# sangminwoo/SVOL

Measured on AMD Instinct MI355X. Metric: frames/sec (fwd+matcher+bwd), T=32·P=196·d=256, higher is better.
Workload: dtype bf16

## Files before the change

### include/svol_hip.h

```cpp
#ifndef SVOL_HIP_H
#define SVOL_HIP_H

#include <stdint.h>

#ifdef __cplusplus
extern "C" {
#endif

#define SVOL_F32 0
#define SVOL_BF16 1
#define SVOL_F16 2

#define SVOL_OK 0
#define SVOL_E_INVALID (-1)
#define SVOL_E_UNSUPPORTED (-2)
#define SVOL_E_LAUNCH (-3)

#define SVOL_ACT_NONE 0
#define SVOL_ACT_RELU 1
#define SVOL_ACT_GELU 2
#define SVOL_ACT_SIGMOID 3
#define SVOL_ACT_GELU_D 5
#define SVOL_ACT_RELU_RES 4

// ... 2 lines not shown

int svol_cast(const void* src, int dtype_src, void* dst, int dtype_dst, int64_t n, void* stream);
int svol_cast_transpose(const float* src, void* dst, void* dstT, int dtype, int64_t R, int64_t C, void* stream);
int svol_cast_transpose_multi(const void* descs, int32_t n_desc, int64_t total_tiles, int dtype, void* stream);
int svol_cast_split(const float* src, int64_t ld_src, void* dst_hilo, int64_t R, int64_t C, void* stream);

int svol_adamw_flat(float* p, const float* g, float* m, float* v, int64_t n, float lr, float beta1, float beta2, float eps,
                    float weight_decay, int64_t step, float grad_scale, void* stream);
int svol_adamw_flat_zero(float* p, float* g, float* m, float* v, int64_t n, float lr, float beta1, float beta2, float eps,
                         float weight_decay, int64_t step, float grad_scale, void* stream);
int svol_grad_finite(const float* g, int64_t n, float* scaler_state, void* stream);
int svol_adamw_flat_scaled(float* p, const float* g, float* m, float* v, int64_t n, float lr, float beta1, float beta2, float eps,
                           float weight_decay, float grad_mul, const float* scaler_state, void* stream);
int svol_loss_scaler_update(float* scaler_state, float growth_factor, float backoff_factor, int64_t growth_interval, float min_scale,
                            float max_scale, void* stream);
int svol_sgd_flat(float* p, const float* g, float* buf, int64_t n, float lr, float momentum, float weight_decay, float grad_scale,
                  void* stream);
int svol_sgd_flat_zero(float* p, float* g, float* buf, int64_t n, float lr, float momentum, float weight_decay, float grad_scale,
                       void* stream);
int svol_sgd_flat_scaled(float* p, const float* g, float* buf, int64_t n, float lr, float momentum, float weight_decay, float grad_mul,
                         const float* scaler_state, void* stream);
int svol_adam_flat(float* p, const float* g, float* m, float* v, int64_t n, float lr, float beta1, float beta2, float eps,
                   float weight_decay, int64_t step, float grad_scale, void* stream);
int svol_adam_flat_zero(float* p, float* g, float* m, float* v, int64_t n, float lr, float beta1, float beta2, float eps,
                        float weight_decay, int64_t step, float grad_scale, void* stream);
int svol_adam_flat_scaled(float* p, const float* g, float* m, float* v, int64_t n, float lr, float beta1, float beta2, float eps,
                          float weight_decay, float grad_mul, const float* scaler_state, void* stream);
int64_t svol_grad_sqnorm_ws_bytes(int64_t n);
int svol_grad_sqnorm(const float* g, int64_t n, float* ws, float* out, void* stream);
int svol_grad_clip_state(const float* sq, int32_t nb, float grad_mul, float max_norm, float loss_scale, int64_t steps_taken,
                         float* scaler_state, float* state_out, void* stream);
int svol_sgd_flat_grouped(float* p, float* g, float* buf, int64_t n, const int32_t* seg_end, const int32_t* seg_group, int32_t nseg,
                          const float* hyper, int32_t ngroups, const float* state, float grad_mul, int zero, void* stream);
int svol_adam_flat_grouped(float* p, float* g, float* m, float* v, int64_t n, const int32_t* seg_end, const int32_t* seg_group,
                           int32_t nseg, const float* hyper, int32_t ngroups, const float* state, const float* step_count,
                           float grad_mul, int zero, void* stream);
int svol_adamw_flat_grouped(float* p, float* g, float* m, float* v, int64_t n, const int32_t* seg_end, const int32_t* seg_group,
                            int32_t nseg, const float* hyper, int32_t ngroups, const float* state, const float* step_count,
                            float grad_mul, int zero, void* stream);
int svol_flat_step_advance(float* step_count, const float* state, void* stream);

int svol_gemm_nt(const void* A, int64_t lda, const void* A2, int64_t n_split, const void* B, int64_t ldb,
                 void* C, int64_t ldc, const float* bias, const float* colscale, int act, void* pre_act_out,
                 int64_t ldp, const void* residual, int64_t ldr, int out_f32, int64_t M, int64_t N, int64_t K,
                 int dtype, void* stream);
int svol_gemm_nt_split(const void* A, int64_t lda, const void* W_hilo, int64_t ldw, void* C, int64_t ldc, const float* bias,
                       int64_t M, int64_t N, int64_t K, void* stream);
int svol_gemm_nt_dgelu(const void* A, int64_t lda, const void* B, int64_t ldb, void* C, int64_t ldc,
                       const void* pre, int64_t ldp, float* colsum, int64_t M, int64_t N, int64_t K, int dtype,
                       void* stream);
int svol_gemm_nt_dact(const void* A, int64_t lda, const void* B, int64_t ldb, void* C, int64_t ldc,
                      const void* aux, int64_t ldaux, int act, float* colsum, int64_t M, int64_t N, int64_t K,
                      int dtype, void* stream);

int svol_gemm_tn(const void* A, int64_t lda, const void* B, int64_t ldb, float* C, int64_t ldc, float* colsum,
                 int64_t Mc, int64_t N, int64_t K, int dtype, void* stream);
#define SVOL_TN_GROUP_MAX 6
typedef struct svol_tn_problem {
    const void* A; int64_t lda;
    const void* B; int64_t ldb;
    float* C; int64_t ldc;
    float* colsum;
    int64_t Mc, N, K;
} svol_tn_problem;
int svol_gemm_tn_grouped(const svol_tn_problem* problems, int32_t n, int dtype, void* stream);
int svol_colsum(const void* X, int64_t ldx, float* out, int64_t M, int64_t N, int dtype, void* stream);
int svol_act_bwd(const void* dy, const void* aux, void* dpre, int act, int64_t n, int dtype, void* stream);

int svol_layernorm_fwd(const void* x, int x_f32, const float* gamma, const float* beta, float* y32, void* y,
                       void* ypos, const void* pos, int64_t pos_rows, float* mean, float* rstd, int64_t M, int64_t D,
                       float dropout_p, uint64_t seed, const int64_t* seed_offset_dev, int dtype, void* stream);
int svol_layernorm_bwd(const float* dy32, const void* dy, const void* dy2, const void* x, int x_f32,
                       const float* gamma, const float* mean, const float* rstd, float* dx32, void* dx,
                       float* dgamma, float* dbeta, float* dx_colsum, int64_t M, int64_t D, float dropout_p,
                       uint64_t seed, const int64_t* seed_offset_dev, int dtype, void* stream);

int svol_dropout(const void* x, void* y, int64_t n, int64_t row_len, float p, uint64_t seed, int dtype, void* stream);
int svol_dropout_add(const float* t32, const float* res32, float* out32, int64_t n, int64_t row_len, float p, uint64_t seed, void* stream);

int svol_posenc_sine(const float* mask, void* pos, int64_t B, int64_t L, int64_t D, int dtype, void* stream);

int64_t svol_attn_ws_bytes(int64_t B, int64_t H, int64_t Lq, int64_t Lk, int64_t dh);
int svol_attn_fwd(const void* q, int64_t ldq, const void* k, int64_t ldk, const void* v, int64_t ldv, void* o,
                  int64_t ldo, float* lse2, const float* kbias, int64_t B, int64_t H, int64_t Lq, int64_t Lk,
                  int64_t dh, float scale, float q_premul, void* ws, int64_t ws_bytes, int dtype, void* stream);
int svol_attn_bwd(const void* q, int64_t ldq, const void* k, int64_t ldk, const void* v, int64_t ldv, const void* o,
                  int64_t ldo, const void* d_o, int64_t lddo, const float* lse2, float* delta, const float* kbias,
                  void* dq, int64_t lddq, void* dk, int64_t lddk, void* dv, int64_t lddv, int64_t B, int64_t H,
                  int64_t Lq, int64_t Lk, int64_t dh, float scale, float q_premul, void* ws, int64_t ws_bytes,
                  int dtype, void* stream);

#define SVOL_ATTN_DQ_PREZEROED 1
int64_t svol_attn_bwd_sp_image_bytes(int64_t B, int64_t H, int64_t Lq, int64_t Lk, int64_t dh, int64_t ws_bytes, int dtype);
int svol_attn_bwd_zero_ws(void* ws, int64_t ws_bytes, int64_t B, int64_t H, int64_t Lq, int64_t Lk, int64_t dh, int dtype, void* stream);
int svol_attn_bwd_ex(const void* q, int64_t ldq, const void* k, int64_t ldk, const void* v, int64_t ldv, const void* o,
                     int64_t ldo, const void* d_o, int64_t lddo, const float* lse2, float* delta, const float* kbias,
                     void* dq, int64_t lddq, void* dk, int64_t lddk, void* dv, int64_t lddv, int64_t B, int64_t H,
                     int64_t Lq, int64_t Lk, int64_t dh, float scale, float q_premul, void* ws, int64_t ws_bytes,
                     int dtype, int flags, void* ev_prep, void* stream);

int svol_attn_fwd_dropout(const void* q, int64_t ldq, const void* k, int64_t ldk, const void* v, int64_t ldv, void* o,
                          int64_t ldo, float* lse2, const float* kbias, int64_t B, int64_t H, int64_t Lq, int64_t Lk,
                          int64_t dh, float scale, float q_premul, void* ws, int64_t ws_bytes, float dropout_p, uint64_t seed,
                          int dtype, void* stream);
int svol_attn_bwd_dropout(const void* q, int64_t ldq, const void* k, int64_t ldk, const void* v, int64_t ldv, const void* o,
                          int64_t ldo, const void* d_o, int64_t lddo, const float* lse2, float* delta, const float* kbias,
                          void* dq, int64_t lddq, void* dk, int64_t lddk, void* dv, int64_t lddv, int64_t B, int64_t H,
                          int64_t Lq, int64_t Lk, int64_t dh, float scale, float q_premul, void* ws, int64_t ws_bytes,
                          float dropout_p, uint64_t seed, int dtype, void* stream);

int svol_gate_fwd(const float* x32, const void* pos, const float* u, const float* gamma, const float* beta,
                  float* y32, void* y, void* ypos, float* a, float* mean, float* rstd, float* ws, int64_t B,
                  int64_t L, int64_t D, int64_t H, int dtype, void* stream);
int svol_gate_bwd(const float* dy32, const void* dy, const void* dy2, const float* x32, const void* pos,
                  const float* u, const float* gamma, const float* a, const float* mean, const float* rstd,
                  const float* ws, float* ws2, float* dx32, float* du, float* dgamma, float* dbeta, int64_t B,
                  int64_t L, int64_t D, int64_t H, int dtype, void* stream);

int svol_layernorm_gate_scores_fwd(const float* x32, const float* gamma, const float* beta, float* y32, void* y, void* ypos,
                                   const void* pos, float* mean, float* rstd, const float* u_next, float* scores_next,
                                   int64_t B, int64_t L, int64_t D, int64_t H, int dtype, void* stream);
int svol_gate_fwd_scored(const float* x32, const void* pos, const float* u, const float* gamma, const float* beta,
                         float* y32, void* y, void* ypos, float* a, float* mean, float* rstd, float* ws, int64_t B,
                         int64_t L, int64_t D, int64_t H, int dtype, void* stream);

int svol_gate_vectors_fwd(const float* skch, const float* W_in, const float* b_in, float* q_out, float* u_out, int64_t B, int64_t D,
                          int64_t H, void* stream);
int svol_gate_vectors_bwd(const float* du, const float* skch, const float* W_in, const float* q, float* dq_ws, float* dskch,
                          float* dW_in, float* db_in, int64_t B, int64_t D, int64_t H, void* stream);
#define SVOL_GATE_VEC_MAX_LAYERS 8
int svol_gate_vectors_fwd_multi(const float* skch, const float* const* W_in, const float* const* b_in, float* const* q_out,
                                float* const* u_out, int64_t n_layers, int64_t B, int64_t D, int64_t H, void* stream);
int svol_gate_vectors_bwd_multi(const float* const* du, const float* skch, const float* const* W_in, const float* const* q,
                                float* const* dq_ws, float* const* dskch, float* const* dW_in, float* const* db_in, int64_t n_layers,
                                int64_t B, int64_t D, int64_t H, void* stream);

int svol_match_cost(const float* logits, const float* boxes, const float* tgt_boxes, const int32_t* pred_off,
                    const int32_t* pred_cnt, const int32_t* tgt_off, const int32_t* tgt_cnt,
                    const int64_t* cost_off, float* cost, int32_t n_problems, float w_bbox, float w_giou,
                    float w_class, int32_t* box_status, void* stream);
int svol_lsap_batched(const float* cost, const int64_t* cost_off, const int32_t* pred_off, const int32_t* pred_cnt,
                      const int32_t* tgt_off, const int32_t* tgt_cnt, int32_t* match, int32_t* status,
                      int32_t n_problems, int32_t max_dim, void* stream);
int svol_heads_fwd(const float* hs, const float* Wc, const float* bc, const float* W0, const float* b0, const float* W1, const float* b1,
                   const float* W2, const float* b2, float* logits, float* h1, float* h2, float* boxes, int64_t R, int64_t D, void* stream);
// ... 46 lines not shown
int svol_conv_weight_unpack_add(const float* dwp, float* grad, int64_t Cout, int64_t Cin, int64_t kh, int64_t kw, int64_t Kp, void* stream);
int svol_conv_wgrad_nhwc(const void* dz, const void* x, float* dwp, int64_t N, int64_t H, int64_t W, int64_t C, int64_t Cout, int64_t kh, int64_t kw,
                         int64_t stride, int64_t pad, int64_t Kp, int dtype, void* stream);
int svol_bn_apply(const void* z, const float* scale, const float* shift, const void* residual, int relu, void* y, int64_t M, int64_t C,
                  int dtype, void* stream);
int svol_bn_bwd_reduce(const void* dy, const void* y, const void* z, const float* mean, const float* rstd, float* sum_g, float* sum_gx,
                       int64_t M, int64_t C, int dtype, void* stream);
int svol_bn_bwd_apply(const void* dy, const void* y, const void* z, const float* mean, const float* rstd, const float* gamma,
                      const float* sum_g, const float* sum_gx, void* dz, void* dres, int64_t M, int64_t C, int dtype, void* stream);
int svol_col2im_nhwc(const void* dcols, int64_t ldcols, void* dx, int64_t N, int64_t H, int64_t W, int64_t C, int64_t kh, int64_t kw,
                     int64_t stride, int64_t pad, int dtype, void* stream);
int svol_maxpool_idx_nhwc(const void* x, void* y, uint8_t* idx, int64_t N, int64_t H, int64_t W, int64_t C, int64_t k, int64_t stride,
                          int64_t pad, int dtype, void* stream);
int svol_maxpool_bwd_nhwc(const void* dy, const uint8_t* idx, void* dx, int64_t N, int64_t H, int64_t W, int64_t C, int64_t k,
                          int64_t stride, int64_t pad, int dtype, void* stream);
int svol_attn_weights_mean(const void* q, int64_t ldq, const void* k, int64_t ldk, const float* lse2, const float* kbias,
                           float* att, int64_t B, int64_t H, int64_t Lq, int64_t Lk, int64_t dh, float scale,
                           float q_premul, int dtype, void* stream);
int svol_attn_small_fwd(const void* q, int64_t ldq, const void* k, int64_t ldk, const void* v, int64_t ldv, void* o, int64_t ldo,
                        int64_t n_seq, int64_t H, int64_t L, int64_t dh, float scale, int dtype, void* stream);
int svol_attn_small_fwd_lse(const void* q, int64_t ldq, const void* k, int64_t ldk, const void* v, int64_t ldv, void* o, int64_t ldo,
                            float* lse2, int64_t n_seq, int64_t H, int64_t L, int64_t dh, float scale, int dtype, void* stream);
int svol_attn_small_bwd(const void* q, int64_t ldq, const void* k, int64_t ldk, const void* v, int64_t ldv, const void* o, int64_t ldo,
                        const void* dout, int64_t lddo, const float* lse2, void* dq, int64_t lddq, void* dk, int64_t lddk, void* dv,
                        int64_t lddv, int64_t n_seq, int64_t H, int64_t L, int64_t dh, float scale, int dtype, void* stream);


#define SVOL_DIM_B 0
#define SVOL_DIM_L 1
#define SVOL_DIM_N 2
#define SVOL_DIM_D 3
#define SVOL_DIM_H 4
#define SVOL_DIM_F 5
#define SVOL_DIM_DTYPE 6
#define SVOL_DIM_QDTYPE 7
#define SVOL_DIM_ATTN_WS_BYTES 8
#define SVOL_DIM_COUNT 9

#define SVOL_BLK_VIDEO_HALF 0
#define SVOL_BLK_QUERY_SELF 1
#define SVOL_BLK_QUERY_CROSS 2
const char* svol_block_slot_names(int block);
int svol_block_trace_dump(char* buf, int64_t cap);
int svol_clock_probe(uint64_t* samples, int32_t* count, int32_t max_samples, const int32_t* stop, int64_t period_us,
                     int64_t max_ms, int32_t* wall_khz, void* stream);


#define SVOL_VH_SLOTS(X) \
    X(X32) X(POS) X(U) X(G1) X(BT1) X(G2) X(BT2) X(G3) X(BT3) X(B_IN) X(B_O) X(B_FC1) X(B_FC2) X(QSCALE) \
    X(W_IN) X(WV_HILO) X(W_O) X(W_FC1) X(W_FC2) X(W_IN_T) X(W_O_T) X(W_FC1_T) X(W_FC2_T) \
    X(Y1) X(Y1POS) X(A) X(MEAN1) X(RSTD1) X(GATE_WS) X(GATE_PRE) X(U_NEXT) X(GATE_WS_NEXT) \
    X(QKV) X(O) X(LSE) X(S2) X(Y2) X(MEAN2) X(RSTD2) X(PRE) X(HID) X(S3) \
    X(MEAN3) X(RSTD3) X(M32) X(M) X(MPOS) X(Y1_32) X(Y2_32) X(ATTN_WS) \
    X(DM32) X(DM) X(DMPOS) X(DS32_3) X(DS3) X(DPRE) X(DY2) X(DS32_2) X(G2D) X(DO) X(DQKV) X(DELTA) X(DXQP) X(DXQ) X(GATE_WS2) \
    X(DX32) X(DU) \
    X(DG1) X(DBT1) X(DG2) X(DBT2) X(DG3) X(DBT3) X(DW_IN) X(DB_IN) X(DW_O) X(DB_O) X(DW_FC1) X(DB_FC1) X(DW_FC2) X(DB_FC2) \
    X(EV_A0) X(EV_A1) X(EV_CLEAN_IN) X(EV_PREP) X(ATTN_WS_NEXT) X(ZERO_STREAM) X(EV_CLEAN_OUT)
#define SVOL_QS_SLOTS(X) \
    X(O32) X(O) X(OPOS) X(QPOS) X(B_IN) X(B_O) X(G4) X(BT4) X(QSCALE) X(W_IN) X(WV_HILO) X(W_O) X(W_IN_T) X(W_O_T) \
    X(QKV) X(OA) X(LSE) X(S4) X(MEAN4) X(RSTD4) X(Y32) X(Y) X(YPOS) X(ATTN_WS) \
    X(DY32) X(DY) X(DYPOS) X(G) X(DOA) X(DQKV) X(DELTA) X(DO32) X(DXQ) X(DXQP) X(DQPOS) \
    X(DW_IN) X(DB_IN) X(DW_O) X(DB_O) X(DG4) X(DBT4)
#define SVOL_QC_SLOTS(X) \
    X(O32) X(O) X(OPOS) X(MV) X(MPOS) X(KBIAS) X(QPOS) X(B_IN) X(B_O) X(G5) X(BT5) X(B_FC1) X(B_FC2) X(G6) X(BT6) X(QSCALE) \
    X(W_INQ) X(W_INQ_T) X(W_KV) X(W_KV_T) X(WV_HILO) X(W_O) X(W_O_T) X(W_FC1) X(W_FC1_T) X(W_FC2) X(W_FC2_T) \
    X(Q) X(QC) X(KV) X(OA) X(OAQ) X(LSE) X(S5) X(Y5_32) X(Y5) X(MEAN5) X(RSTD5) X(PRE) X(HID) X(S6) X(MEAN6) X(RSTD6) \
    X(Y32) X(Y) X(YPOS) X(ATTN_WS) \
    X(DY32) X(DY) X(DYPOS) X(DS32_6) X(DS6) X(DPRE) X(DY5) X(DS32_5) X(G5D) X(DOAQ) X(DOA) X(DQC) X(DQ) X(DKV) X(DELTA) \
    X(DO32) X(DXQP) X(DMPOS) X(DMV) X(DQPOS) \
    X(DW_IN) X(DB_IN) X(DW_O) X(DB_O) X(DG5) X(DBT5) X(DW_FC1) X(DB_FC1) X(DW_FC2) X(DB_FC2) X(DG6) X(DBT6)
#define SVOL_SLOT_ENUM_VH(n) SVOL_VH_##n,
#define SVOL_SLOT_ENUM_QS(n) SVOL_QS_##n,
#define SVOL_SLOT_ENUM_QC(n) SVOL_QC_##n,
enum { SVOL_VH_SLOTS(SVOL_SLOT_ENUM_VH) SVOL_VH_COUNT };
enum { SVOL_QS_SLOTS(SVOL_SLOT_ENUM_QS) SVOL_QS_COUNT };
enum { SVOL_QC_SLOTS(SVOL_SLOT_ENUM_QC) SVOL_QC_COUNT };

int svol_video_half_fwd(const int64_t* dims, void* const* slots, void* stream);
int svol_video_half_bwd(const int64_t* dims, void* const* slots, int phase, void* stream);
int svol_video_half_wgrad(const int64_t* dims, void* const* slots, void* stream);
int svol_video_half_wgrad_part(const int64_t* dims, void* const* slots, int part, void* stream);
int svol_query_self_fwd(const int64_t* dims, void* const* slots, void* stream);
int svol_query_self_bwd(const int64_t* dims, void* const* slots, void* stream);
int svol_query_self_wgrad(const int64_t* dims, void* const* slots, void* stream);
int svol_query_cross_fwd(const int64_t* dims, void* const* slots, void* stream);
int svol_query_cross_bwd(const int64_t* dims, void* const* slots, void* stream);
int svol_query_cross_wgrad(const int64_t* dims, void* const* slots, void* stream);

#ifdef __cplusplus
}
#endif
#endif
```

### svol_amd/_lib.py

```python
from __future__ import annotations

import ctypes
import os

_HERE = os.path.dirname(os.path.abspath(__file__))
LIB_PATH = os.path.join(_HERE, 'libsvol_hip.so')

_p = ctypes.c_void_p
_i64 = ctypes.c_int64
_i32 = ctypes.c_int32
_int = ctypes.c_int
_f32 = ctypes.c_float
_u64 = ctypes.c_uint64

SIGNATURES = {
    'svol_block_trace_dump': [ctypes.c_char_p, _i64],
    'svol_lsap_solve': [_p, _i64, _i64, _p, _p],
    'svol_heads_fwd': [_p] * 13 + [_i64, _i64, _p],
    'svol_heads_bwd': [_p] * 17 + [_i64, _i64, _p],
    'svol_set_loss_bwd': [_p] * 6 + [_i64, _i64, _p],
    'svol_weighted_total': [_p, _p, _i64, _p, _p],
    'svol_weighted_total_bwd': [_p, _p, _i64, _p, _p],
    'svol_cast': [_p, _int, _p, _int, _i64, _p],
    'svol_cast_transpose': [_p, _p, _p, _int, _i64, _i64, _p],
    'svol_cast_split': [_p, _i64, _p, _i64, _i64, _p],
    'svol_gemm_nt_split': [_p, _i64, _p, _i64, _p, _i64, _p, _i64, _i64, _i64, _p],
    'svol_gemm_nt': [_p, _i64, _p, _i64, _p, _i64, _p, _i64, _p, _p, _int, _p, _i64, _p, _i64, _int, _i64, _i64, _i64,
                     _int, _p],
    'svol_gemm_nt_dgelu': [_p, _i64, _p, _i64, _p, _i64, _p, _i64, _p, _i64, _i64, _i64, _int, _p],
    'svol_gemm_nt_dact': [_p, _i64, _p, _i64, _p, _i64, _p, _i64, _int, _p, _i64, _i64, _i64, _int, _p],
    'svol_gemm_tn': [_p, _i64, _p, _i64, _p, _i64, _p, _i64, _i64, _i64, _int, _p],
    'svol_gemm_tn_grouped': [_p, _i32, _int, _p],
    'svol_colsum': [_p, _i64, _p, _i64, _i64, _int, _p],
    'svol_act_bwd': [_p, _p, _p, _int, _i64, _int, _p],
    'svol_layernorm_fwd': [_p, _int, _p, _p, _p, _p, _p, _p, _i64, _p, _p, _i64, _i64, _f32, _u64, _p, _int, _p],
    'svol_layernorm_bwd': [_p, _p, _p, _p, _int, _p, _p, _p, _p, _p, _p, _p, _p, _i64, _i64, _f32, _u64, _p, _int, _p],
    'svol_cast_transpose_multi': [_p, _int, _i64, _int, _p],
    'svol_postprocess': [_p, _p, _p, _i64, _i64, _i64, _p],
    'svol_eval_max_iou': [_p, _p, _p, _p, _p, _p, _i64, _int, _p],
    'svol_eval_ap': [_p, _p, _p, _p, _p, _p, _p, _p, _int, _p, _p, _p, _p, _i64, _i64, _i64, _p],
    'svol_patchify': [_p, _p, _i64, _i64, _i64, _i64, _i64, _int, _p],
    'svol_vit_embed': [_p, _p, _p, _p, _p, _i64, _i64, _i64, _int, _p],
    'svol_ingest_resize': [_p, _i64, _i64, _i64, _i64, _i64, _i64, _p, _i64, _p, _i64, _p, _p, _p, _i64, _i64, _i64, _i64, _i64, _i64, _int, _p],
    'svol_adamw_flat': [_p, _p, _p, _p, _i64, _f32, _f32, _f32, _f32, _f32, _i64, _f32, _p],
    'svol_adamw_flat_zero': [_p, _p, _p, _p, _i64, _f32, _f32, _f32, _f32, _f32, _i64, _f32, _p],
    'svol_grad_finite': [_p, _i64, _p, _p],
    'svol_adamw_flat_scaled': [_p, _p, _p, _p, _i64, _f32, _f32, _f32, _f32, _f32, _f32, _p, _p],
    'svol_loss_scaler_update': [_p, _f32, _f32, _i64, _f32, _f32, _p],
    'svol_sgd_flat': [_p, _p, _p, _i64, _f32, _f32, _f32, _f32, _p],
    'svol_sgd_flat_zero': [_p, _p, _p, _i64, _f32, _f32, _f32, _f32, _p],
    'svol_sgd_flat_scaled': [_p, _p, _p, _i64, _f32, _f32, _f32, _f32, _p, _p],
    'svol_adam_flat': [_p, _p, _p, _p, _i64, _f32, _f32, _f32, _f32, _f32, _i64, _f32, _p],
    'svol_adam_flat_zero': [_p, _p, _p, _p, _i64, _f32, _f32, _f32, _f32, _f32, _i64, _f32, _p],
    'svol_adam_flat_scaled': [_p, _p, _p, _p, _i64, _f32, _f32, _f32, _f32, _f32, _f32, _p, _p],
    'svol_grad_sqnorm_ws_bytes': [_i64],
    'svol_grad_sqnorm': [_p, _i64, _p, _p, _p],
    'svol_grad_clip_state': [_p, _i32, _f32, _f32, _f32, _i64, _p, _p, _p],
    'svol_sgd_flat_grouped': [_p, _p, _p, _i64, _p, _p, _i32, _p, _i32, _p, _f32, _int, _p],
    'svol_adam_flat_grouped': [_p, _p, _p, _p, _i64, _p, _p, _i32, _p, _i32, _p, _p, _f32, _int, _p],
    'svol_adamw_flat_grouped': [_p, _p, _p, _p, _i64, _p, _p, _i32, _p, _i32, _p, _p, _f32, _int, _p],
    'svol_flat_step_advance': [_p, _p, _p],
    'svol_conv_nhwc': [_p, _p, _i64, _p, _p, _int, _p, _i64, _i64, _i64, _i64, _i64, _i64, _i64, _i64, _i64, _int, _p],
    'svol_im2col': [_p, _i64, _i64, _i64, _i64, _int, _p, _i64, _i64, _i64, _i64, _i64, _i64, _i64, _i64, _i64, _int, _p],
    'svol_maxpool_nhwc': [_p, _p, _i64, _i64, _i64, _i64, _i64, _i64, _i64, _int, _p],
    'svol_avgpool_nhwc': [_p, _p, _i64, _i64, _i64, _int, _p],
    'svol_bn_colstats': [_p, _p, _f32, _p, _p, _i64, _i64, _int, _p],
    'svol_bn_finalize': [_p, _p, _p, _p, _p, _p, _p, _f32, _f32, _i64, _i64, _p, _p, _p, _p, _p],
    'svol_conv_weight_pack': [_p, _p, _i64, _i64, _i64, _i64, _i64, _int, _int, _p],
    'svol_conv_weight_unpack_add': [_p, _p, _i64, _i64, _i64, _i64, _i64, _p],
    'svol_conv_wgrad_nhwc': [_p, _p, _p, _i64, _i64, _i64, _i64, _i64, _i64, _i64, _i64, _i64, _i64, _int, _p],
    'svol_bn_apply': [_p, _p, _p, _p, _int, _p, _i64, _i64, _int, _p],
    'svol_bn_bwd_reduce': [_p, _p, _p, _p, _p, _p, _p, _i64, _i64, _int, _p],
    'svol_bn_bwd_apply': [_p, _p, _p, _p, _p, _p, _p, _p, _p, _p, _i64, _i64, _int, _p],
    'svol_col2im_nhwc': [_p, _i64, _p, _i64, _i64, _i64, _i64, _i64, _i64, _i64, _i64, _int, _p],
    'svol_maxpool_idx_nhwc': [_p, _p, _p, _i64, _i64, _i64, _i64, _i64, _i64, _i64, _int, _p],
    'svol_maxpool_bwd_nhwc': [_p, _p, _p, _i64, _i64, _i64, _i64, _i64, _i64, _i64, _int, _p],
    'svol_attn_weights_mean': [_p, _i64, _p, _i64, _p, _p, _p, _i64, _i64, _i64, _i64, _i64, _f32, _f32, _int, _p],
    'svol_attn_small_fwd': [_p, _i64, _p, _i64, _p, _i64, _p, _i64, _i64, _i64, _i64, _i64, _f32, _int, _p],
    'svol_attn_small_fwd_lse': [_p, _i64, _p, _i64, _p, _i64, _p, _i64, _p, _i64, _i64, _i64, _i64, _f32, _int, _p],
    'svol_attn_small_bwd': [_p, _i64, _p, _i64, _p, _i64, _p, _i64, _p, _i64, _p, _p, _i64, _p, _i64, _p, _i64, _i64, _i64, _i64,
                            _i64, _f32, _int, _p],
    'svol_posenc_sine': [_p, _p, _i64, _i64, _i64, _int, _p],
    'svol_attn_ws_bytes': [_i64, _i64, _i64, _i64, _i64],
# ... 83 lines not shown
```

### svol_amd/blocks.py

```python
from __future__ import annotations

import ctypes
import math
import os
import weakref

import torch

from . import _lib, ops

WGRAD_SPLIT = os.environ.get('SVOL_WGRAD_SPLIT') is not None
ENABLED = os.environ.get('SVOL_NO_BLOCKS') is None
GATE_SCORES_FUSE = os.environ.get('SVOL_GATE_SCORES_FUSE') is not None
VH, QS, QC = 0, 1, 2
_F32, _BF16 = 0, 1
_ESZ = {torch.float32: 4, torch.bfloat16: 2, torch.float16: 2}
_SLOTS = {}


def _slots(block):
    m = _SLOTS.get(block)
    if m is None:
        names = _lib.lib().svol_block_slot_names(block).decode().rstrip(',').split(',')
        m = _SLOTS[block] = {n: i for i, n in enumerate(names)}
# ... 293 lines not shown
    e0, e1 = torch.cuda.Event(enable_timing=True), torch.cuda.Event(enable_timing=True)
    e0.record()
    e1.record()
    tm.records.setdefault((name, meta), []).append((e0, e1))
    return e0, e1


DQ_PREZERO = os.environ.get('SVOL_DQ_PREZERO') is not None and os.environ.get('SVOL_NO_DQ_PREZERO') is None
_DQ_PREZERO = {}


class _DqPrezero:
    __slots__ = ('bufs', 'side', 'ev_prep', 'clean_ev', 'clean', 'nxt')

    def __init__(self, dev, wsb):
        self.bufs = [torch.empty((_align(wsb, 1 << 20),), dtype=torch.uint8, device=dev) for _ in range(2)]
        self.side = torch.cuda.Stream(device=dev)
        self.ev_prep = torch.cuda.Event()
        self.clean_ev = [torch.cuda.Event(), torch.cuda.Event()]
        for e_ in [self.ev_prep] + self.clean_ev:
            e_.record()
        self.clean = [False, False]
        self.nxt = 0

    def bind(self, tbl):
        i = self.nxt
        tbl.set('ATTN_WS', self.bufs[i].data_ptr())
        tbl.set('EV_CLEAN_IN', self.clean_ev[i].cuda_event if self.clean[i] else None)
        tbl.set('EV_PREP', self.ev_prep.cuda_event)
        tbl.set('ATTN_WS_NEXT', self.bufs[1 - i].data_ptr())
        tbl.set('ZERO_STREAM', self.side.cuda_stream)
        tbl.set('EV_CLEAN_OUT', self.clean_ev[1 - i].cuda_event)
        self.clean[i] = False

    def advance(self, tbl):
        i = self.nxt
        self.clean[1 - i] = True
        self.nxt = 1 - i
        for n_ in ('EV_CLEAN_IN', 'EV_PREP', 'ATTN_WS_NEXT', 'ZERO_STREAM', 'EV_CLEAN_OUT'):
            tbl.set(n_, None)


def _dq_prezero(dev, B, H, L, dh, dt, wsb):
    if not DQ_PREZERO or dt == torch.float32 or torch.cuda.is_current_stream_capturing():
        return None
    key = (dev, ops._stream(), B, H, L, dh, dt, wsb)
    st = _DQ_PREZERO.get(key)
    if st is None:
        img = _lib.lib().svol_attn_bwd_sp_image_bytes(B, H, L, L, dh, wsb, ops._DT[dt])
        st = _DQ_PREZERO[key] = _DqPrezero(dev, wsb) if img > 0 else False
    return st or None


def _vh_fwd_layout(B, L, D, H, F, e):
    M = B * L
    return [('Y1', M * D * e), ('Y1POS', M * D * e), ('A', M * 4), ('MEAN1', M * 4), ('RSTD1', M * 4), ('GATE_WS', B * H * (L + 2) * 4),
            ('QKV', M * 3 * D * e), ('O', M * D * e), ('LSE', B * H * L * 4), ('S2', M * D * 4), ('Y2', M * D * e), ('MEAN2', M * 4),
            ('RSTD2', M * 4), ('PRE', M * F * e), ('HID', M * F * e), ('S3', M * D * 4), ('MEAN3', M * 4), ('RSTD3', M * 4),
            ('M32', M * D * 4), ('M', M * D * e), ('MPOS', M * D * e)]


def _vh_bwd_layout(B, L, D, H, F, e):
    M = B * L
    return [('DS32_3', M * D * 4), ('DS3', M * D * e), ('DPRE', M * F * e), ('DY2', M * D * e), ('DS32_2', M * D * 4), ('G2D', M * D * e),
            ('DO', M * D * e), ('DQKV', M * 3 * D * e), ('DELTA', 3 * B * H * L * 4), ('DXQP', M * D * e), ('DXQ', M * D * e),
            ('GATE_WS2', (B * L + B * H) * 4), ('DX32', M * D * 4)]


class VideoHalfFn(torch.autograd.Function):

    @staticmethod
    def forward(ctx, pl, x32, pos, u, u_next, sc_in, *params):
        ctx.set_materialize_grads(False)
        B, L, D = x32.shape
        layer = pl.layer()
        H, F = layer.nhead, layer.mlp1.fc1.weight.shape[0]
        dt = pl.dt
        e = _ESZ[dt]
        dev = x32.device
        M = B * L
        x2 = x32.reshape(M, D)
        x2 = x2 if x2.is_contiguous() else x2.contiguous()
        pos2 = pos.reshape(M, D)
        pos2 = pos2 if pos2.is_contiguous() else pos2.contiguous()
        u = u.contiguous()
        assert x2.dtype == torch.float32 and pos2.dtype == dt and u.dtype == torch.float32
        wsb = _attn_ws_bytes(B, H, L, L, D // H, dt)
        key = (VH, B, L, D, H, F, dt)
        lay = _layout(('f',) + key, lambda: _vh_fwd_layout(B, L, D, H, F, e))
        slay = _layout(('s',) + key, lambda: [('Y1_32', M * D * 4), ('Y2_32', M * D * 4), ('ATTN_WS', max(wsb, 16))])
        arena = torch.empty((lay.total,), dtype=torch.uint8, device=dev)
        scr = _scratch(dev, slay.total)
        tbl = _Table(VH, pl.tpl)
        lay.fill(tbl, arena.data_ptr())
        slay.fill(tbl, scr.data_ptr())
        tbl.set('X32', x2.data_ptr())
        tbl.set('POS', pos2.data_ptr())
        tbl.set('U', u.data_ptr())
        if sc_in is not None:
            assert sc_in.dtype == torch.float32 and sc_in.numel() == B * H * (L + 2) and sc_in.is_contiguous()
            tbl.set('GATE_WS', sc_in.data_ptr())
            tbl.set('GATE_PRE', sc_in.data_ptr())
        if u_next is not None:
            u_next = u_next.contiguous()
            assert u_next.dtype == torch.float32 and u_next.shape == u.shape and L % 4 == 0
            sc_next = torch.empty((B * H * (L + 2),), dtype=torch.float32, device=dev)
            tbl.set('U_NEXT', u_next.data_ptr())
            tbl.set('GATE_WS_NEXT', sc_next.data_ptr())
        else:
            sc_next = torch.empty((0,), dtype=torch.float32, device=dev)
        dims = _dims(B, L, 0, D, H, F, dt, dt, wsb)
        big = B * H * L * L >= ops._WGRAD_FLUSH_MIN_SCORES
        if big:
            ops._BIG_ATTN['left'] += 1
        ev = _maybe_events('attn_fwd', (B, H, L, L, D // H))
        if ev:
            tbl.set('EV_A0', ev[0].cuda_event)
            tbl.set('EV_A1', ev[1].cuda_event)
# ... 2 lines not shown
        tbl.set('EV_A1', None)
        tbl.set('U_NEXT', None)
        tbl.set('GATE_WS_NEXT', None)
        ctx.pl, ctx.tbl, ctx.dims, ctx.arena, ctx.shape, ctx.big = pl, tbl, dims, arena, (B, L, D, H, F), big
        ctx.n_par = len(params)
        ctx.sc_in = sc_in
        ctx.save_for_backward(x2, pos2, u)
        ctx.mark_non_differentiable(sc_next)
        return (lay.view(arena, 'M32', torch.float32, (B, L, D)), lay.view(arena, 'M', dt, (B, L, D)),
                lay.view(arena, 'MPOS', dt, (B, L, D)), sc_next)

    @staticmethod
    def backward(ctx, dm32, dm, dmpos, _dsc=None):
        pl, tbl, dims = ctx.pl, ctx.tbl, ctx.dims
        B, L, D, H, F = ctx.shape
        x2, pos2, u = ctx.saved_tensors
        n_par = ctx.n_par
        if dm32 is None and dm is None and dmpos is None:
            pl.done(n_par > 0)
            return (None,) * (6 + n_par)
        dt = pl.dt
        e = _ESZ[dt]
        dev = x2.device
        M = B * L
        cont = lambda t_: None if t_ is None else (t_.reshape(M, D) if t_.is_contiguous() else t_.reshape(M, D).contiguous())
        dm32, dm, dmpos = cont(dm32), cont(dm), cont(dmpos)
        lay = _layout(('b', VH, B, L, D, H, F, dt), lambda: _vh_bwd_layout(B, L, D, H, F, e))
        tmp = torch.empty((lay.total,), dtype=torch.uint8, device=dev)
        lay.fill(tbl, tmp.data_ptr())
        du = torch.zeros((B, H, D), dtype=torch.float32, device=dev)
        tbl.set('DU', du.data_ptr())
        tbl.set_t('DM32', dm32)
        tbl.set_t('DM', dm)
        tbl.set_t('DMPOS', dmpos)
        slay = _layout(('s', VH, B, L, D, H, F, dt), None)
        scr = _scratch(dev, slay.total)
        slay.fill(tbl, scr.data_ptr())
        bufs = pl.grad_buffers(tbl, dev)
        L_ = _lib.lib()
        s = ops._stream()
        _lib.check(L_.svol_video_half_bwd(dims, tbl.arr, 1, s), 'svol_video_half_bwd')
        keep = [t_ for t_ in (ctx.arena, tmp, dm32, dm, dmpos) if t_ is not None]
        split = bufs is None and ctx.big and WGRAD_SPLIT
        if ctx.big:
            ops._BIG_ATTN['left'] -= 1
            if split:
                _issue_wgrad('svol_video_half_wgrad_part', dims, tbl, keep, dev, part=1)
            ops.flush_wgrad(gate=True)
        ev = _maybe_events('attn_bwd', (B, H, L, L, D // H))
        if ev:
            tbl.set('EV_A0', ev[0].cuda_event)
            tbl.set('EV_A1', ev[1].cuda_event)
        pz = _dq_prezero(dev, B, H, L, D // H, dt, dims[8]) if ctx.big else None
        if pz is not None:
            pz.bind(tbl)
        _lib.check(L_.svol_video_half_bwd(dims, tbl.arr, 2, s), 'svol_video_half_bwd')
        if pz is not None:
            pz.advance(tbl)
        tbl.set('EV_A0', None)
        tbl.set('EV_A1', None)
        if split:
            _issue_wgrad('svol_video_half_wgrad_part', dims, tbl, keep, dev, part=2)
        elif bufs is None:
            _issue_wgrad('svol_video_half_wgrad', dims, tbl, keep, dev)
        else:
            _lib.check(L_.svol_video_half_wgrad(dims, tbl.arr, s), 'svol_video_half_wgrad')
        pl.done(n_par > 0)
        dx32 = lay.view(tmp, 'DX32', torch.float32, (B, L, D))
        needs = ctx.needs_input_grad
        return (None, dx32, None, du if needs[3] else None, None, None) + tuple(pl.grads_out(bufs, needs[6:], n_par > 0))


def gate_scores_fusable(L, D, H):
    return GATE_SCORES_FUSE and L % 4 == 0 and D % 4 == 0 and D <= 256 and H <= 8


def video_half(layer, x32, pos, u, dt, u_next=None, sc_in=None):
    pl = plan(layer, VH, dt, dt)
    if u_next is not None and not gate_scores_fusable(x32.shape[1], x32.shape[2], layer.nhead):
        u_next = None
    m32, m, mpos, sc = VideoHalfFn.apply(pl, x32, pos, u, u_next, sc_in, *pl.inputs(x32, u))
    return m32, m, mpos, (sc if u_next is not None else None)


def _qpos_target(pl, qpos, tbl, dev, N, D):
    if not qpos.requires_grad:
        tbl.set('DQPOS', None)
        return None, False
    s = ops._claim(qpos, True) if (qpos.is_leaf and qpos.dtype == torch.float32) else None
    if s is not None:
        tbl.set_t('DQPOS', s.view)
        return None, True
    g = torch.zeros((N, D), dtype=torch.float32, device=dev)
    tbl.set('DQPOS', g.data_ptr())
    return g, False


class QuerySelfFn(torch.autograd.Function):

    @staticmethod
    def forward(ctx, pl, o32, o, opos, qpos, *params):
        ctx.set_materialize_grads(False)
        B, N, D = o.shape
        layer = pl.layer()
        H = layer.nhead
        qdt = pl.qdt
        e = _ESZ[qdt]
        dev = o.device
        R = B * N
        c = lambda t_: t_ if t_.is_contiguous() else t_.contiguous()
        o32_, o_, opos_, qpos_ = c(o32), c(o), c(opos), c(qpos)
# ... 30 lines not shown
            pl.done(n_par > 0)
            return (None,) * (5 + n_par)
        qdt = pl.qdt
        e = _ESZ[qdt]
        dev = o_.device
        R = B * N
        cont = lambda t_: None if t_ is None else (t_ if t_.is_contiguous() else t_.contiguous())
        dy32, dy, dypos = cont(dy32), cont(dy), cont(dypos)
        lay = _layout(('b', QS, B, N, D, H, qdt), lambda: [('G', R * D * e), ('DOA', R * D * e), ('DQKV', R * 3 * D * e),
                                                            ('DELTA', 3 * B * H * N * 4), ('DO32', R * D * 4), ('DXQ', R * D * e),
                                                            ('DXQP', R * D * e)])
        tmp = torch.empty((lay.total,), dtype=torch.uint8, device=dev)
        lay.fill(tbl, tmp.data_ptr())
        tbl.set_t('DY32', dy32)
        tbl.set_t('DY', dy)
        tbl.set_t('DYPOS', dypos)
        slay = _layout(('s', QS, B, N, D, H, qdt), None)
        scr = _scratch(dev, slay.total)
        slay.fill(tbl, scr.data_ptr())
        needs = ctx.needs_input_grad
        gq, _ = _qpos_target(pl, qpos, tbl, dev, N, D) if needs[4] else (None, False)
        if not needs[4]:
            tbl.set('DQPOS', None)
        bufs = pl.grad_buffers(tbl, dev)
        L_ = _lib.lib()
        s = ops._stream()
        _lib.check(L_.svol_query_self_bwd(dims, tbl.arr, s), 'svol_query_self_bwd')
        keep = (ctx.arena, tmp, o_, opos_)
        if bufs is None:
            _issue_wgrad('svol_query_self_wgrad', dims, tbl, list(keep), dev)
        else:
            _lib.check(L_.svol_query_self_wgrad(dims, tbl.arr, s), 'svol_query_self_wgrad')
        pl.done(n_par > 0)
        if gq is not None and qdt != torch.float32:
            gq = ops.cast(gq, qdt)
        v = lambda n_, dt_: lay.view(tmp, n_, dt_, (B, N, D))
        return (None, v('DO32', torch.float32), v('DXQ', qdt), v('DXQP', qdt), gq) + tuple(pl.grads_out(bufs, needs[5:], n_par > 0))


def query_self(layer, out, qpos, dt, qdt):
    pl = plan(layer, QS, dt, qdt)
    o32, o, opos = out
    return QuerySelfFn.apply(pl, o32, o, opos, qpos, *pl.inputs(o32, o, opos))


def _qc_fwd_layout(B, N, L, D, H, F, e, qe):
    R, M = B * N, B * L
    return [('Q', R * D * qe), ('QC', R * D * e), ('KV', M * 2 * D * e), ('OA', R * D * e), ('OAQ', R * D * qe), ('LSE', B * H * N * 4),
            ('S5', R * D * 4), ('Y5_32', R * D * 4), ('Y5', R * D * qe), ('MEAN5', R * 4), ('RSTD5', R * 4), ('PRE', R * F * qe),
            ('HID', R * F * qe), ('S6', R * D * 4), ('MEAN6', R * 4), ('RSTD6', R * 4), ('Y32', R * D * 4), ('Y', R * D * qe),
            ('YPOS', R * D * qe)]


def _qc_bwd_layout(B, N, L, D, H, F, e, qe):
    R, M = B * N, B * L
    return [('DS32_6', R * D * 4), ('DS6', R * D * qe), ('DPRE', R * F * qe), ('DY5', R * D * qe), ('G5D', R * D * qe), ('DOAQ', R * D * qe),
            ('DOA', R * D * e), ('DQC', R * D * e), ('DQ', R * D * qe), ('DKV', M * 2 * D * e), ('DELTA', 3 * B * H * N * 4),
            ('DO32', R * D * 4), ('DXQP', R * D * qe), ('DMPOS', M * D * e), ('DMV', M * D * e)]


class QueryCrossFn(torch.autograd.Function):

    @staticmethod
    def forward(ctx, pl, o32, o, opos, mv, mpos, kbias, qpos, *params):
        ctx.set_materialize_grads(False)
        B, N, D = o.shape
        L = mv.shape[1]
        layer = pl.layer()
        H, F = layer.nhead, layer.mlp2.fc1.weight.shape[0]
        dt, qdt = pl.dt, pl.qdt
        e, qe = _ESZ[dt], _ESZ[qdt]
        dev = o.device
        c = lambda t_: t_ if t_.is_contiguous() else t_.contiguous()
        o32_, o_, opos_, mv_, mpos_, kb_, qpos_ = c(o32), c(o), c(opos), c(mv), c(mpos), c(kbias), c(qpos)
        assert o32_.dtype == torch.float32 and o_.dtype == qdt and opos_.dtype == qdt and qpos_.dtype == qdt
        assert mv_.dtype == dt and mpos_.dtype == dt and kb_.dtype == torch.float32
        wsb = _attn_ws_bytes(B, H, N, L, D // H, dt)
        key = (QC, B, N, L, D, H, F, dt, qdt)
        lay = _layout(('f',) + key, lambda: _qc_fwd_layout(B, N, L, D, H, F, e, qe))
        slay = _layout(('s',) + key, lambda: [('ATTN_WS', max(wsb, 16))])
        arena = torch.empty((lay.total,), dtype=torch.uint8, device=dev)
        scr = _scratch(dev, slay.total)
        tbl = _Table(QC, pl.tpl)
        lay.fill(tbl, arena.data_ptr())
        slay.fill(tbl, scr.data_ptr())
        for n_, t_ in (('O32', o32_), ('O', o_), ('OPOS', opos_), ('MV', mv_), ('MPOS', mpos_), ('KBIAS', kb_), ('QPOS', qpos_)):
            tbl.set(n_, t_.data_ptr())
        dims = _dims(B, L, N, D, H, F, dt, qdt, wsb)
        _lib.check(_lib.lib().svol_query_cross_fwd(dims, tbl.arr, ops._stream()), 'svol_query_cross_fwd')
        ctx.pl, ctx.tbl, ctx.dims, ctx.arena, ctx.shape = pl, tbl, dims, arena, (B, N, L, D, H, F)
        ctx.n_par = len(params)
        ctx.save_for_backward(o32_, o_, opos_, mv_, mpos_, kb_, qpos)
        return (lay.view(arena, 'Y32', torch.float32, (B, N, D)), lay.view(arena, 'Y', qdt, (B, N, D)),
                lay.view(arena, 'YPOS', qdt, (B, N, D)))

    @staticmethod
    def backward(ctx, dy32, dy, dypos):
        pl, tbl, dims = ctx.pl, ctx.tbl, ctx.dims
        B, N, L, D, H, F = ctx.shape
        o32_, o_, opos_, mv_, mpos_, kb_, qpos = ctx.saved_tensors
        n_par = ctx.n_par
        if dy32 is None and dy is None and dypos is None:
            pl.done(n_par > 0)
            return (None,) * (8 + n_par)
        dt, qdt = pl.dt, pl.qdt
        e, qe = _ESZ[dt], _ESZ[qdt]
        dev = o_.device
        cont = lambda t_: None if t_ is None else (t_ if t_.is_contiguous() else t_.contiguous())
        dy32, dy, dypos = cont(dy32), cont(dy), cont(dypos)
        lay = _layout(('b', QC, B, N, L, D, H, F, dt, qdt), lambda: _qc_bwd_layout(B, N, L, D, H, F, e, qe))
        tmp = torch.empty((lay.total,), dtype=torch.uint8, device=dev)
        lay.fill(tbl, tmp.data_ptr())
        tbl.set_t('DY32', dy32)
        tbl.set_t('DY', dy)
        tbl.set_t('DYPOS', dypos)
        slay = _layout(('s', QC, B, N, L, D, H, F, dt, qdt), None)
        scr = _scratch(dev, slay.total)
        slay.fill(tbl, scr.data_ptr())
        needs = ctx.needs_input_grad
        gq = None
        if needs[7]:
            gq, _ = _qpos_target(pl, qpos, tbl, dev, N, D)
        else:
            tbl.set('DQPOS', None)
        bufs = pl.grad_buffers(tbl, dev)
        L_ = _lib.lib()
        s = ops._stream()
        _lib.check(L_.svol_query_cross_bwd(dims, tbl.arr, s), 'svol_query_cross_bwd')
        keep = (ctx.arena, tmp, opos_, mv_, mpos_)
        if bufs is None:
            _issue_wgrad('svol_query_cross_wgrad', dims, tbl, list(keep), dev)
        else:
            _lib.check(L_.svol_query_cross_wgrad(dims, tbl.arr, s), 'svol_query_cross_wgrad')
        pl.done(n_par > 0)
        if gq is not None and qdt != torch.float32:
            gq = ops.cast(gq, qdt)
        vq = lambda n_, dt_: lay.view(tmp, n_, dt_, (B, N, D))
        vm = lambda n_: lay.view(tmp, n_, dt, (B, L, D))
        return (None, vq('DO32', torch.float32), None, vq('DXQP', qdt), vm('DMV'), vm('DMPOS'), None, gq) + \
            tuple(pl.grads_out(bufs, needs[8:], n_par > 0))


def query_cross(layer, out, mv, mpos, kbias, qpos, dt, qdt):
    pl = plan(layer, QC, dt, qdt)
    o32, o, opos = out
    return QueryCrossFn.apply(pl, o32, o, opos, mv, mpos, kbias, qpos, *pl.inputs(o32, opos, mv, mpos))


def trace_dump() -> str:
    buf = ctypes.create_string_buffer(1 << 20)
    _lib.check(_lib.lib().svol_block_trace_dump(buf, len(buf)), 'svol_block_trace_dump')
    return buf.value.decode()
```

### svol_amd/csrc/attention.hip

```cpp
#include "attn_call.h"

namespace {

constexpr float LOG2E = 1.4426950408889634f;

template <typename T> struct AT;
template <> struct AT<float> {
    static constexpr int EPC = 4, NA = 4, CPR = 8, NAT_ROW = 128, TR_STRIDE = 64 * 4 + 16;
};

template <typename T>
__device__ __forceinline__ int nat_off(int row, int ch) {
    if constexpr (sizeof(T) == 2) return row * 64 + ((ch ^ ((row >> 2) & 3)) << 4);
    else return row * 128 + ((ch ^ (row & 7)) << 4);
}

template <typename T>
__device__ __forceinline__ void stage_tile(char* nat, char* tr, const T* g, int64_t ld, int row0, int limit, int dh,
                                           int tid) {
    constexpr int EPC = AT<T>::EPC, CPR = AT<T>::CPR, ST = AT<T>::TR_STRIDE;
    for (int c = tid; c < 64 * CPR; c += 256) {
        const int row = c / CPR, ch = c % CPR;
        const int d0 = ch * EPC;
        uint4 v = make_uint4(0, 0, 0, 0);
// ... 462 lines not shown
    AttnArgs p{};
    attn_fill(p, c);
    dim3 grid((unsigned)((Lq + 127) / 128), (unsigned)H, (unsigned)B);
    hipLaunchKernelGGL(attn_fwd_kernel<float>, grid, dim3(256), 0, c.stream, p);
    SVOL_CHECK_LAUNCH();
    return SVOL_OK;
}
int svol_attn_fwd(const void* q, int64_t ldq, const void* k, int64_t ldk, const void* v, int64_t ldv, void* o,
                  int64_t ldo, float* lse2, const float* kbias, int64_t B, int64_t H, int64_t Lq, int64_t Lk, int64_t dh,
                  float scale, float q_premul, void* ws, int64_t ws_bytes, int dtype, void* stream) {
    return svol_attn_fwd_dropout(q, ldq, k, ldk, v, ldv, o, ldo, lse2, kbias, B, H, Lq, Lk, dh, scale, q_premul, ws, ws_bytes, 0.f, 0,
                                 dtype, stream);
}

static int attn_bwd_impl(const void* q, int64_t ldq, const void* k, int64_t ldk, const void* v, int64_t ldv, const void* o,
                         int64_t ldo, const void* d_o, int64_t lddo, const float* lse2, float* delta, const float* kbias, void* dq,
                         int64_t lddq, void* dk, int64_t lddk, void* dv, int64_t lddv, int64_t B, int64_t H, int64_t Lq, int64_t Lk,
                         int64_t dh, float scale, float q_premul, void* ws, int64_t ws_bytes, float drop_p, uint64_t drop_seed,
                         int dtype, void* stream, int flags = 0, void* ev_prep = nullptr) {
    AttnCall c{};
    c.q = q; c.k = k; c.v = v; c.o = o; c.d_o = d_o; c.lse2 = const_cast<float*>(lse2); c.delta = delta; c.kbias = kbias;
    c.dq = dq; c.dk = dk; c.dv = dv;
    c.ldq = ldq; c.ldk = ldk; c.ldv = ldv; c.ldo = ldo; c.lddo = lddo; c.lddq = lddq; c.lddk = lddk; c.lddv = lddv;
    c.scale = scale; c.premul = q_premul; c.ws = static_cast<float*>(ws); c.ws_bytes = ws_bytes;
    c.drop_p = drop_p; c.drop_seed = drop_seed; c.flags = flags; c.ev_prep = ev_prep; c.stream = reinterpret_cast<hipStream_t>(stream);
    if (const int rc = check_call(c, true, B, H, Lq, Lk, dh, dtype)) return rc;
    if (svol_is16(dtype)) return (dtype == SVOL_BF16 ? svol_attn_bwd_bf16_launch : svol_attn_bwd_f16_launch)(c);
    AttnArgs p{};
    attn_fill(p, c);
    const int64_t total = B * Lq * H;
    dim3 gd((unsigned)((total + 255) / 256));
    dim3 gq((unsigned)((Lq + 127) / 128), (unsigned)H, (unsigned)B);
    dim3 gk((unsigned)((Lk + 127) / 128), (unsigned)H, (unsigned)B);
    hipLaunchKernelGGL(attn_delta_kernel<float>, gd, dim3(256), 0, c.stream, p);
    hipLaunchKernelGGL(attn_bwd_dq_kernel<float>, gq, dim3(256), 0, c.stream, p);
    hipLaunchKernelGGL(attn_bwd_dkdv_kernel<float>, gk, dim3(256), 0, c.stream, p);
    if (ev_prep) (void)hipEventRecord(static_cast<hipEvent_t>(ev_prep), c.stream);
    SVOL_CHECK_LAUNCH();
    return SVOL_OK;
}

int svol_attn_bwd(const void* q, int64_t ldq, const void* k, int64_t ldk, const void* v, int64_t ldv, const void* o,
                  int64_t ldo, const void* d_o, int64_t lddo, const float* lse2, float* delta, const float* kbias, void* dq,
                  int64_t lddq, void* dk, int64_t lddk, void* dv, int64_t lddv, int64_t B, int64_t H, int64_t Lq, int64_t Lk,
                  int64_t dh, float scale, float q_premul, void* ws, int64_t ws_bytes, int dtype, void* stream) {
    return attn_bwd_impl(q, ldq, k, ldk, v, ldv, o, ldo, d_o, lddo, lse2, delta, kbias, dq, lddq, dk, lddk, dv, lddv, B, H, Lq, Lk, dh,
                         scale, q_premul, ws, ws_bytes, 0.f, 0, dtype, stream);
}
int svol_attn_bwd_ex(const void* q, int64_t ldq, const void* k, int64_t ldk, const void* v, int64_t ldv, const void* o,
                     int64_t ldo, const void* d_o, int64_t lddo, const float* lse2, float* delta, const float* kbias, void* dq,
                     int64_t lddq, void* dk, int64_t lddk, void* dv, int64_t lddv, int64_t B, int64_t H, int64_t Lq, int64_t Lk,
                     int64_t dh, float scale, float q_premul, void* ws, int64_t ws_bytes, int dtype, int flags, void* ev_prep,
                     void* stream) {
    if (flags & ~SVOL_ATTN_DQ_PREZEROED) return SVOL_E_INVALID;
    return attn_bwd_impl(q, ldq, k, ldk, v, ldv, o, ldo, d_o, lddo, lse2, delta, kbias, dq, lddq, dk, lddk, dv, lddv, B, H, Lq, Lk, dh,
                         scale, q_premul, ws, ws_bytes, 0.f, 0, dtype, stream, flags, ev_prep);
}
int64_t svol_attn_bwd_sp_image_bytes(int64_t B, int64_t H, int64_t Lq, int64_t Lk, int64_t dh, int64_t ws_bytes, int dtype) {
    if (!svol_is16(dtype) || check_common(B, H, Lq, Lk, dh, dtype)) return 0;
    return (dtype == SVOL_BF16 ? svol_attn_sp_image_bytes_bf16 : svol_attn_sp_image_bytes_f16)((int)B, (int)H, (int)Lq, (int)Lk, (int)dh,
                                                                                              ws_bytes);
}
int svol_attn_bwd_zero_ws(void* ws, int64_t ws_bytes, int64_t B, int64_t H, int64_t Lq, int64_t Lk, int64_t dh, int dtype, void* stream) {
    if (!ws || !aligned16(ws)) return SVOL_E_INVALID;
    if (!svol_is16(dtype)) return SVOL_E_UNSUPPORTED;
    const int rc = check_common(B, H, Lq, Lk, dh, dtype);
    if (rc) return rc;
    return (dtype == SVOL_BF16 ? svol_attn_sp_zero_bf16_launch : svol_attn_sp_zero_f16_launch)(
        static_cast<float*>(ws), ws_bytes, (int)B, (int)H, (int)Lq, (int)Lk, (int)dh, reinterpret_cast<hipStream_t>(stream));
}
int svol_attn_bwd_dropout(const void* q, int64_t ldq, const void* k, int64_t ldk, const void* v, int64_t ldv, const void* o,
                          int64_t ldo, const void* d_o, int64_t lddo, const float* lse2, float* delta, const float* kbias, void* dq,
                          int64_t lddq, void* dk, int64_t lddk, void* dv, int64_t lddv, int64_t B, int64_t H, int64_t Lq, int64_t Lk,
                          int64_t dh, float scale, float q_premul, void* ws, int64_t ws_bytes, float dropout_p, uint64_t seed,
                          int dtype, void* stream) {
    return attn_bwd_impl(q, ldq, k, ldk, v, ldv, o, ldo, d_o, lddo, lse2, delta, kbias, dq, lddq, dk, lddk, dv, lddv, B, H, Lq, Lk, dh,
                         scale, q_premul, ws, ws_bytes, dropout_p, seed, dtype, stream);
}

}
```

### svol_amd/csrc/attention_bf16.hip

```cpp
#include <cstdint>
#include <cstdlib>

#include "attn_call.h"

namespace {

constexpr float LOG2E = 1.4426950408889634f;
constexpr int KT = 128;
constexpr int IMG = KT * 64;
constexpr float LAZY_THR = 4.0f;

struct Args {
    const void *q, *k, *v, *o, *d_o;
    void *out_o, *dq, *dk, *dv;
    const float* kbias;
    float *lse2, *delta;
    int64_t ldq, ldk, ldv, ldo, lddo, lddq, lddk, lddv;
    int B, H, Lq, Lk, dh;
    float scale;
    float premul;
    int ksplit, tiles_per_split;
    float *ws_o, *ws_ml, *ws_dq;
    const int* tile_flags;
    int head_xcd, nxt;
// ... 1502 lines not shown
        {
            const int row = tid >> 3, d0 = (tid & 7) * 4;
            f32x4 v = *reinterpret_cast<const f32x4*>(sRed + row * 32 + d0);
#pragma unroll
            for (int w = 1; w < 4; ++w) {
                const f32x4 u = *reinterpret_cast<const f32x4*>(sRed + (w * 32 + row) * 32 + d0);
#pragma unroll
                for (int e = 0; e < 4; ++e) v[e] += u[e];
            }
            const int q = sub * 32 + row;
            if (q < p.Lq) {
                float* z = p.ws_dq + ((int64_t)b * p.Lq + q) * (p.H * 32) + hh * 32 + d0;
#pragma unroll
                for (int e = 0; e < 4; ++e) unsafeAtomicAdd(z + e, v[e]);
            }
        }
        __syncthreads();
    }
}

template <bool ZERO>
__global__ __launch_bounds__(256) void attn_bwd_sp_prep_bf16(Args p) {
    __shared__ float s_lse[8][33], s_dl[8][33];
    const int tid = threadIdx.x;
    const int64_t row0 = (int64_t)blockIdx.x * 32;
    const int b = (int)(row0 / p.Lq), q0 = (int)(row0 % p.Lq);
    {
        const int hh = tid >> 5, rl = tid & 31;
        if (hh < p.H) s_lse[hh][rl] = p.lse2[((int64_t)b * p.H + hh) * p.Lq + q0 + rl];
    }
    const int rl = tid >> 3, hh = tid & 7;
    float dl = 0.f;
    if (hh < p.H) {
        const int64_t row = row0 + rl;
        const h16_t* o = reinterpret_cast<const h16_t*>(p.o) + row * p.ldo + hh * 32;
        const h16_t* d = reinterpret_cast<const h16_t*>(p.d_o) + row * p.lddo + hh * 32;
#pragma unroll
        for (int i = 0; i < 32; i += 8) {
            const h16x8 a = *reinterpret_cast<const h16x8*>(o + i), c = *reinterpret_cast<const h16x8*>(d + i);
#pragma unroll
            for (int e = 0; e < 8; ++e) dl += (float)a[e] * (float)c[e];
        }
        if constexpr (ZERO) {
            float* z = p.ws_dq + row * (p.H * 32) + hh * 32;
#pragma unroll
            for (int i = 0; i < 32; i += 4) *reinterpret_cast<f32x4*>(z + i) = f32x4{0.f, 0.f, 0.f, 0.f};
        }
        s_dl[hh][rl] = dl;
    }
    __syncthreads();
    {
        const int h2 = tid >> 5, r2 = tid & 31;
        if (h2 < p.H) {
            const int64_t si = ((int64_t)b * p.H + h2) * p.Lq + q0 + r2;
            reinterpret_cast<float*>(p.nl2)[si] = -s_lse[h2][r2];
            reinterpret_cast<float*>(p.nd2)[si] = -s_dl[h2][r2];
            p.delta[si] = s_dl[h2][r2];
        }
    }
}
__global__ __launch_bounds__(256) void attn_dq_round_bf16(Args p) {
    const int64_t i = ((int64_t)blockIdx.x * blockDim.x + threadIdx.x) * 8;
    const int64_t W = (int64_t)p.H * 32, total = (int64_t)p.B * p.Lq * W;
    if (i >= total) {
        const int tk = p.Lk % (4 * 128);
        const int64_t j = i - ((total + 2047) / 2048) * 2048;
        if (tk == 0 || j < 0 || j >= (int64_t)p.B * p.H * 2 * tk * 32) return;
        const int64_t per = (int64_t)2 * tk * 32;
        const int bh = (int)(j / per), rem = (int)(j % per), kv = rem / (tk * 32), key = (rem / 32) % tk, d0 = rem % 32;
        const float* src = p.ws_dq + total + (int64_t)bh * 4 * per + rem;
        f32x4 a = {0.f, 0.f, 0.f, 0.f}, c = a;
#pragma unroll
        for (int part = 0; part < 4; ++part) { a += *reinterpret_cast<const f32x4*>(src + part * per); c += *reinterpret_cast<const f32x4*>(src + part * per + 4); }
        const float mul = kv == 0 ? p.scale / p.premul : 1.f;
        h16x8 v;
#pragma unroll
        for (int e = 0; e < 4; ++e) { v[e] = (h16_t)(a[e] * mul); v[4 + e] = (h16_t)(c[e] * mul); }
        const int b_ = bh / p.H, hh_ = bh % p.H;
        const int64_t row = (int64_t)b_ * p.Lk + (p.Lk - tk) + key;
        h16_t* o = kv == 0 ? reinterpret_cast<h16_t*>(p.dk) + row * p.lddk : reinterpret_cast<h16_t*>(p.dv) + row * p.lddv;
        *reinterpret_cast<h16x8*>(o + hh_ * 32 + d0) = v;
        return;
    }
    const int64_t row = i / W, c = i % W;
    const f32x4 a = *reinterpret_cast<const f32x4*>(p.ws_dq + i), b = *reinterpret_cast<const f32x4*>(p.ws_dq + i + 4);
    h16x8 v;
#pragma unroll
    for (int e = 0; e < 4; ++e) { v[e] = (h16_t)(a[e] * p.scale); v[4 + e] = (h16_t)(b[e] * p.scale); }
    *reinterpret_cast<h16x8*>(reinterpret_cast<h16_t*>(p.dq) + row * p.lddq + c) = v;
}

__global__ __launch_bounds__(256) void attn_sp_zero_image(float* __restrict__ z, int64_t n4) {
    const int64_t stride = (int64_t)gridDim.x * 256;
    for (int64_t i = (int64_t)blockIdx.x * 256 + threadIdx.x; i < n4; i += stride)
        reinterpret_cast<f32x4*>(z)[i] = f32x4{0.f, 0.f, 0.f, 0.f};
}

typedef __attribute__((ext_vector_type(4))) unsigned u32x4;
__device__ __forceinline__ u32x4 to_acc(u32x4 r) {
    asm volatile("; operand -> AGPR" : "+a"(r));
    return r;
}
__device__ __forceinline__ u32x4 as_u32x4(const uint4& v) { return u32x4{v.x, v.y, v.z, v.w}; }
#define SP_FENCE() __builtin_amdgcn_sched_barrier(0)
__device__ __forceinline__ void sp_mfma_c(f32x16& d, const uint4& a, const u32x4& b, const f32x16& c) {
    asm volatile("v_mfma_f32_32x32x16_" SVOL_H16_ASM " %0, %1, %2, %3" : "=&v"(d) : "v"(as_u32x4(a)), "a"(b), "v"(c));
}
__device__ __forceinline__ void sp_mfma_z(f32x16& d, const uint4& a, const u32x4& b) {
    asm volatile("v_mfma_f32_32x32x16_" SVOL_H16_ASM " %0, %1, %2, 0" : "=&v"(d) : "v"(as_u32x4(a)), "a"(b));
}
__device__ __forceinline__ void sp_mfma_v(f32x16& d, const uint4& a, const u32x4& b) {
    asm volatile("v_mfma_f32_32x32x16_" SVOL_H16_ASM " %0, %1, %2, %0" : "+v"(d) : "v"(as_u32x4(a)), "a"(b));
}
__device__ __forceinline__ void sp_mfma_a(f32x16& acc, const uint4& a, const u32x4& b) {
    asm volatile("v_mfma_f32_32x32x16_" SVOL_H16_ASM " %0, %1, %2, %0" : "+a"(acc) : "v"(as_u32x4(a)), "v"(b));
}
__device__ __forceinline__ unsigned cvt_pk_u32(float a, float b) { return __builtin_bit_cast(unsigned, cvt_pk_h16(a, b)); }

struct SpStep {
    uint4 qa[2], doa[2];
    f32x16 Cl, Cd;
};
constexpr int SP_OFF_Q = 4 * KT * 4 + 512;
constexpr int SP_OFF_T = SP_OFF_Q + 4 * IMG;
constexpr int SP_OFF_P = SP_OFF_Q + 8 * IMG;

template <int NKB>
__device__ __forceinline__ void attn_bwd_sp_body(const Args& p, char* smem, int hh, int b, int kbase, int t_begin, int t_end, float* tail_out) {
    float* sL = reinterpret_cast<float*>(smem);
    float* sD = sL + 2 * KT;
    float* sNeg = sL + 4 * KT;
    char* sQ = smem + SP_OFF_Q;
    char* sPart = smem + SP_OFF_P;
    const int tid = threadIdx.x, lane = tid & 63, wave = __builtin_amdgcn_readfirstlane(tid >> 6);
    const int r = lane & 31, h = lane >> 5;
    constexpr int dqw = 8 * 32;
    const h16_t* Q = reinterpret_cast<const h16_t*>(p.q) + (int64_t)b * p.Lq * p.ldq + hh * 32;
    const h16_t* dO = reinterpret_cast<const h16_t*>(p.d_o) + (int64_t)b * p.Lq * p.lddo + hh * 32;
// ... 820 lines not shown
constexpr int SP_ZERO_WGS = 64;
int svol_attn_sp_zero_bf16_launch(float* ws, int64_t ws_bytes, int B, int H, int Lq, int Lk, int dh, hipStream_t s) {
    if (!sp_planned(B, H, Lq, Lk, dh, ws != nullptr, ws_bytes)) return SVOL_E_UNSUPPORTED;
    const int64_t n4 = (int64_t)B * Lq * H * 32 / 4;
    const int64_t want = (n4 + 255) / 256;
    hipLaunchKernelGGL(attn_sp_zero_image, dim3((unsigned)(want < SP_ZERO_WGS ? want : SP_ZERO_WGS)), dim3(256), 0, s, ws, n4);
    return hipGetLastError() == hipSuccess ? SVOL_OK : SVOL_E_LAUNCH;
}
static Args make_args(const AttnCall& c, int ksplit, int tiles_per_split, const Grid& g) {
    Args p{};
    attn_fill(p, c);
    p.ksplit = ksplit; p.tiles_per_split = tiles_per_split;
    if (ksplit > 1) {
        p.ws_o = c.ws;
        p.ws_ml = p.ws_o + (int64_t)p.ksplit * p.B * p.Lq * p.H * p.dh;
        p.ws_dq = p.ws_ml + (int64_t)p.ksplit * p.B * p.H * p.Lq * 2;
    }
    p.head_xcd = g.head_xcd; p.nxt = g.nxt; p.tail_last = g.tail_last;
    return p;
}

int svol_attn_fwd_bf16_launch(const AttnCall& c) {
    const Plan pl = attn_plan(c);
    Args p = make_args(c, pl.fwd_ksplit, pl.fwd_tps, pl.gf);
    const dim3 grid = pl.gf.dim, wg(256);
    hipStream_t s = c.stream;
    switch (pl.fwd) {
    case Fwd::pre_masked:
        p.tile_flags = reinterpret_cast<const int*>(c.ws);
        hipLaunchKernelGGL(attn_tile_flags_bf16, dim3((unsigned)pl.ntk, (unsigned)c.B), dim3(64), 0, s, c.kbias, c.Lk, pl.ntk, reinterpret_cast<int*>(c.ws));
        hipLaunchKernelGGL(attn_fwd_bf16_pre_masked, grid, wg, 0, s, p);
        break;
    case Fwd::fast2_redo:
        p.redo = reinterpret_cast<int*>(c.ws);
        hipLaunchKernelGGL(attn_fwd_bf16_fast2, grid, wg, 0, s, p);
        [[fallthrough]];
    case Fwd::pre_all: hipLaunchKernelGGL(attn_fwd_bf16_pre, grid, wg, 0, s, p); break;
    case Fwd::general_m:
    case Fwd::ksplit_m: hipLaunchKernelGGL(attn_fwd_bf16<true>, grid, wg, 0, s, p); break;
    case Fwd::general_u:
    case Fwd::ksplit_u: hipLaunchKernelGGL(attn_fwd_bf16<false>, grid, wg, 0, s, p); break;
    }
    const int64_t total = (int64_t)c.B * c.Lq * c.H;
    if (pl.fwd_ksplit > 1) hipLaunchKernelGGL(attn_combine_bf16, dim3((unsigned)((total + 127) / 128)), dim3(128), 0, s, p);
    return hipGetLastError() == hipSuccess ? SVOL_OK : SVOL_E_LAUNCH;
}

int svol_attn_bwd_bf16_launch(const AttnCall& c) {
    const Plan pl = attn_plan(c);
    Args pq = make_args(c, pl.bwd_ksplit, pl.bwd_tps, pl.gq), pk = make_args(c, pl.bwd_ksplit, pl.bwd_tps, pl.gk);
    const int64_t total = (int64_t)c.B * c.Lq * c.H;
    const dim3 gd((unsigned)((total + 255) / 256)), wg(256);
    hipStream_t s = c.stream;
    auto bind_rows = [&](Args& a) { a.nl2 = reinterpret_cast<unsigned*>(c.delta + total); a.nd2 = reinterpret_cast<unsigned*>(c.delta + 2 * total); };
    void (*dq)(Args) = nullptr, (*dkdv)(Args) = nullptr;
    if (!pl.pre) hipLaunchKernelGGL(attn_delta_bf16, gd, wg, 0, s, pq);
    switch (pl.bwd) {
    case Bwd::bwd_pre_masked:
        pq.tile_flags = pk.tile_flags = reinterpret_cast<const int*>(c.ws);
        hipLaunchKernelGGL(attn_tile_flags_bf16, dim3((unsigned)pl.ntk, (unsigned)c.B), dim3(64), 0, s, c.kbias, c.Lk, pl.ntk, reinterpret_cast<int*>(c.ws));
        dq = attn_bwd_dq_bf16_pre_masked, dkdv = attn_bwd_dkdv_bf16_pre_masked;
        break;
    case Bwd::bwd_sp:
        pq.ws_dq = c.ws;
        bind_rows(pq);
        hipLaunchKernelGGL((c.flags & SVOL_ATTN_DQ_PREZEROED) ? attn_bwd_sp_prep_bf16<false> : attn_bwd_sp_prep_bf16<true>,
                           dim3((unsigned)((int64_t)c.B * c.Lq / 32)), wg, 0, s, pq);
        break;
    case Bwd::bwd_rot_dma:
        bind_rows(pq), bind_rows(pk);
        dq = attn_bwd_dq_bf16_rot, dkdv = attn_bwd_dkdv_bf16_pre_dma;
        break;
    case Bwd::bwd_rot: dq = attn_bwd_dq_bf16_rot, dkdv = attn_bwd_dkdv_bf16_pre; break;
    case Bwd::bwd_pre: dq = attn_bwd_dq_bf16_pre, dkdv = attn_bwd_dkdv_bf16_pre; break;
    case Bwd::fq_m:
    case Bwd::fq_u: {
        Args pf = pq;
        pf.tiles_per_split = pl.fq_tps;
        hipLaunchKernelGGL(pl.bwd == Bwd::fq_m ? attn_bwd_fq_bf16<true> : attn_bwd_fq_bf16<false>, pl.fq_grid, wg, 0, s, pf);
        hipLaunchKernelGGL(attn_dq_finish_bf16, gd, wg, 0, s, pq);
        break;
    }
    case Bwd::two_pass_m: dq = attn_bwd_dq_bf16<true>, dkdv = attn_bwd_dkdv_bf16<true>; break;
    case Bwd::two_pass_u: dq = attn_bwd_dq_bf16<false>, dkdv = attn_bwd_dkdv_bf16<false>; break;
    }
    if (dq) {
        hipLaunchKernelGGL(dq, pl.gq.dim, wg, 0, s, pq);
        if (pl.bwd_ksplit > 1) hipLaunchKernelGGL(attn_dq_finish_bf16, gd, wg, 0, s, pq);
        hipLaunchKernelGGL(dkdv, pl.gk.dim, wg, 0, s, pk);
    }
    if (c.ev_prep) (void)hipEventRecord(static_cast<hipEvent_t>(c.ev_prep), s);
    if (pl.bwd == Bwd::bwd_sp) {
        hipLaunchKernelGGL(attn_bwd_sp_bf16, dim3(sp_grid(c.B, c.H, c.Lk)), wg, 0, s, pq);
        hipLaunchKernelGGL(attn_dq_round_bf16, dim3(sp_round_grid(c.B, c.H, c.Lq, c.Lk)), wg, 0, s, pq);
    }
    return hipGetLastError() == hipSuccess ? SVOL_OK : SVOL_E_LAUNCH;
}
```

### svol_amd/csrc/attn_call.h

```cpp
#pragma once
#include "common.h"

struct AttnCall {
    const void *q, *k, *v, *o, *d_o;
    void *out_o, *dq, *dk, *dv;
    const float* kbias;
    float *lse2, *delta;
    int64_t ldq, ldk, ldv, ldo, lddo, lddq, lddk, lddv;
    int B, H, Lq, Lk, dh;
    float scale, premul, drop_p;
    uint64_t drop_seed;
    float* ws;
    int64_t ws_bytes;
    int flags;
    void* ev_prep;
    hipStream_t stream;
};

template <typename A> static inline void attn_fill(A& p, const AttnCall& c) {
    p.q = c.q; p.k = c.k; p.v = c.v; p.o = c.o; p.d_o = c.d_o; p.out_o = c.out_o; p.dq = c.dq; p.dk = c.dk; p.dv = c.dv;
    p.kbias = c.kbias; p.lse2 = c.lse2; p.delta = c.delta;
    p.ldq = c.ldq; p.ldk = c.ldk; p.ldv = c.ldv; p.ldo = c.ldo; p.lddo = c.lddo; p.lddq = c.lddq; p.lddk = c.lddk; p.lddv = c.lddv;
    p.B = c.B; p.H = c.H; p.Lq = c.Lq; p.Lk = c.Lk; p.dh = c.dh; p.scale = c.scale; p.premul = c.premul;
    p.drop_p = c.drop_p; p.drop_inv = c.drop_p > 0.f ? 1.f / (1.f - c.drop_p) : 1.f; p.drop_seed = c.drop_seed;
}

#define SVOL_ATTN_H16_ENTRIES(T)                                                                                      \
    int svol_attn_fwd_##T##_launch(const AttnCall& c);                                                                \
    int svol_attn_bwd_##T##_launch(const AttnCall& c);                                                                \
    int64_t svol_attn_ws_floats_##T(int B, int H, int Lq, int Lk, int dh);                                            \
    int64_t svol_attn_sp_image_bytes_##T(int B, int H, int Lq, int Lk, int dh, int64_t ws_bytes);                     \
    int svol_attn_sp_zero_##T##_launch(float* ws, int64_t ws_bytes, int B, int H, int Lq, int Lk, int dh, hipStream_t s);
SVOL_ATTN_H16_ENTRIES(bf16)
SVOL_ATTN_H16_ENTRIES(f16)
#undef SVOL_ATTN_H16_ENTRIES
```

### svol_amd/csrc/blocks.hip

```cpp
#include <math.h>
#include <stdio.h>
#include <stdlib.h>
#include <string.h>

#include <map>
#include <mutex>
#include <string>
#include <vector>

#include "common.h"

namespace {

const bool kTrace = getenv("SVOL_BLOCK_TRACE") != nullptr;
struct TraceRec { const char* prog; const char* site; hipEvent_t e0, e1; };
std::mutex g_trace_mu;
std::vector<TraceRec> g_trace_log;
struct Trace {
    const char* prog;
    hipStream_t s;
    hipEvent_t last = nullptr;
    Trace* prev;
    static thread_local Trace* cur;
    Trace(const char* prog_, void* s_) : prog(prog_), s(static_cast<hipStream_t>(s_)), prev(cur) {
        cur = this;
        if (kTrace && hipEventCreate(&last) == hipSuccess) (void)hipEventRecord(last, s);
    }
    ~Trace() { cur = prev; }
    void mark(const char* site) {
        if (!kTrace || !last) return;
        hipEvent_t e;
        if (hipEventCreate(&e) != hipSuccess) return;
        (void)hipEventRecord(e, s);
        std::lock_guard<std::mutex> lk(g_trace_mu);
        g_trace_log.push_back({prog, site, last, e});
        last = e;
    }
};
thread_local Trace* Trace::cur = nullptr;

struct Dims {
    int64_t B, L, N, D, H, F, ws_bytes;
    int dt, qdt;
    explicit Dims(const int64_t* d)
        : B(d[SVOL_DIM_B]), L(d[SVOL_DIM_L]), N(d[SVOL_DIM_N]), D(d[SVOL_DIM_D]), H(d[SVOL_DIM_H]), F(d[SVOL_DIM_F]),
          ws_bytes(d[SVOL_DIM_ATTN_WS_BYTES]), dt((int)d[SVOL_DIM_DTYPE]), qdt((int)d[SVOL_DIM_QDTYPE]) {}
    bool ok() const {
        return B > 0 && D > 0 && H > 0 && D % H == 0 && (dt == SVOL_F32 || svol_is16(dt)) && (qdt == SVOL_F32 || svol_is16(qdt));
    }
};

inline int esz(int dtype) { return svol_is16(dtype) ? 2 : 4; }
inline void* at(void* p, int64_t elems, int dtype) { return p ? static_cast<char*>(p) + elems * esz(dtype) : nullptr; }
inline const void* at(const void* p, int64_t elems, int dtype) { return p ? static_cast<const char*>(p) + elems * esz(dtype) : nullptr; }
inline float* f32(void* p) { return static_cast<float*>(p); }

inline float attn_scale(int64_t dh) { return (float)(1.0 / sqrt((double)dh)); }
inline float attn_premul(int64_t dh, int dtype) { return svol_is16(dtype) ? (float)(1.4426950408889634 / sqrt((double)dh)) : 0.f; }

inline int nt(const void* A, int64_t lda, const void* W, int64_t ldw, void* C, int64_t ldc, const void* bias, const void* colscale,
              int64_t M, int64_t N, int64_t K, int dtype, void* s) {
    return svol_gemm_nt(A, lda, nullptr, 0, W, ldw, C, ldc, static_cast<const float*>(bias), static_cast<const float*>(colscale),
                        SVOL_ACT_NONE, nullptr, 0, nullptr, 0, 0, M, N, K, dtype, s);
}
inline int nt_res(const void* A, int64_t lda, const void* W, int64_t ldw, void* C32, const void* bias, const void* res32, int64_t M,
                  int64_t N, int64_t K, int dtype, void* s) {
    return svol_gemm_nt(A, lda, nullptr, 0, W, ldw, C32, N, static_cast<const float*>(bias), nullptr, SVOL_ACT_NONE, nullptr, 0, res32, N,
                        1, M, N, K, dtype, s);
}

#define RUN(expr)                                 \
    do {                                          \
        const int rc_ = (expr);                   \
        if (rc_) return rc_;                      \
        if (kTrace && Trace::cur) Trace::cur->mark(#expr); \
    } while (0)

#define SLOT_NAME(n) #n ","
const char* const kVhNames = SVOL_VH_SLOTS(SLOT_NAME);
const char* const kQsNames = SVOL_QS_SLOTS(SLOT_NAME);
const char* const kQcNames = SVOL_QC_SLOTS(SLOT_NAME);

inline void record(void* ev, void* stream) {
    if (ev) (void)hipEventRecord(static_cast<hipEvent_t>(ev), static_cast<hipStream_t>(stream));
}

}


extern "C" {

int svol_block_trace_dump(char* buf, int64_t cap) {
    if (!buf || cap <= 0) return SVOL_E_INVALID;
    buf[0] = 0;
    if (!kTrace) return SVOL_OK;
    if (hipDeviceSynchronize() != hipSuccess) return SVOL_E_LAUNCH;
    std::lock_guard<std::mutex> lk(g_trace_mu);
    static const bool timeline = getenv("SVOL_BLOCK_TRACE") && atoi(getenv("SVOL_BLOCK_TRACE")) == 2;
    if (timeline && !g_trace_log.empty()) {
        std::string out;
        char line[256];
        const hipEvent_t ref = g_trace_log.front().e0;
        for (const TraceRec& r : g_trace_log) {
            float t0 = 0.f, t1 = 0.f;
            if (hipEventElapsedTime(&t0, ref, r.e0) != hipSuccess || hipEventElapsedTime(&t1, ref, r.e1) != hipSuccess) continue;
            std::string site(r.site);
            const size_t c = site.find(',');
            if (c != std::string::npos) site.resize(c);
            snprintf(line, sizeof line, "%9.3f %9.3f  %-20s %s\n", t0, t1, r.prog, site.c_str());
            out += line;
        }
        std::map<hipEvent_t, int> seen_;
        for (const TraceRec& r : g_trace_log) { seen_[r.e0] = 1; seen_[r.e1] = 1; }
        for (auto& kv : seen_) (void)hipEventDestroy(kv.first);
        g_trace_log.clear();
        strncpy(buf, out.c_str(), (size_t)cap - 1);
        buf[cap - 1] = 0;
        return SVOL_OK;
    }
    std::map<std::string, std::pair<double, int>> acc;
    std::vector<std::string> order;
    std::map<hipEvent_t, int> seen;
    for (const TraceRec& r : g_trace_log) {
        float ms = 0.f;
        if (hipEventElapsedTime(&ms, r.e0, r.e1) != hipSuccess) continue;
        std::string site(r.site);
        const size_t c = site.find(',');
        if (c != std::string::npos) site.resize(c);
        const std::string key = std::string(r.prog) + " | " + site;
// ... 26 lines not shown
}

int svol_video_half_fwd(const int64_t* dims, void* const* p, void* s) {
    if (!dims || !p) return SVOL_E_INVALID;
    Trace tr_("video_half_fwd", s);
    const Dims d(dims);
    if (!d.ok() || d.L <= 0 || d.F <= 0) return SVOL_E_INVALID;
    const int64_t M = d.B * d.L, D = d.D, F = d.F, dh = D / d.H;
    const int dt = d.dt, xf = dt != SVOL_F32;
#define P(n) p[SVOL_VH_##n]
    if (P(GATE_PRE))
        RUN(svol_gate_fwd_scored(f32(P(X32)), P(POS), f32(P(U)), f32(P(G1)), f32(P(BT1)), f32(P(Y1_32)), P(Y1), P(Y1POS), f32(P(A)),
                                 f32(P(MEAN1)), f32(P(RSTD1)), f32(P(GATE_WS)), d.B, d.L, D, d.H, dt, s));
    else
        RUN(svol_gate_fwd(f32(P(X32)), P(POS), f32(P(U)), f32(P(G1)), f32(P(BT1)), f32(P(Y1_32)), P(Y1), P(Y1POS), f32(P(A)), f32(P(MEAN1)),
                          f32(P(RSTD1)), f32(P(GATE_WS)), d.B, d.L, D, d.H, dt, s));
    RUN(nt(P(Y1POS), D, P(W_IN), D, P(QKV), 3 * D, P(B_IN), P(QSCALE), M, 2 * D, D, dt, s));
    if (P(WV_HILO))
        RUN(svol_gemm_nt_split(P(Y1), D, P(WV_HILO), 2 * D, at(P(QKV), 2 * D, dt), 3 * D, f32(P(B_IN)) + 2 * D, M, D, D, s));
    else
        RUN(nt(P(Y1), D, at(P(W_IN), 2 * D * D, dt), D, at(P(QKV), 2 * D, dt), 3 * D, f32(P(B_IN)) + 2 * D, nullptr, M, D, D, dt, s));
    record(P(EV_A0), s);
    RUN(svol_attn_fwd(P(QKV), 3 * D, at(P(QKV), D, dt), 3 * D, at(P(QKV), 2 * D, dt), 3 * D, P(O), D, f32(P(LSE)), nullptr, d.B, d.H, d.L,
                      d.L, dh, attn_scale(dh), attn_premul(dh, dt), P(ATTN_WS), d.ws_bytes, dt, s));
    record(P(EV_A1), s);
    RUN(nt_res(P(O), D, P(W_O), D, P(S2), P(B_O), P(Y1_32), M, D, D, dt, s));
    RUN(svol_layernorm_fwd(P(S2), xf, f32(P(G2)), f32(P(BT2)), f32(P(Y2_32)), P(Y2), nullptr, nullptr, 0, f32(P(MEAN2)), f32(P(RSTD2)), M,
                           D, 0.f, 0, nullptr, dt, s));
    RUN(svol_gemm_nt(P(Y2), D, nullptr, 0, P(W_FC1), D, P(HID), F, f32(P(B_FC1)), nullptr, SVOL_ACT_GELU_D, P(PRE), F, nullptr, 0, 0, M, F, D, dt, s));
    RUN(nt_res(P(HID), F, P(W_FC2), F, P(S3), P(B_FC2), P(Y2_32), M, D, F, dt, s));
    if (P(U_NEXT) && P(GATE_WS_NEXT))
        RUN(svol_layernorm_gate_scores_fwd(f32(P(S3)), f32(P(G3)), f32(P(BT3)), f32(P(M32)), P(M), P(MPOS), P(POS), f32(P(MEAN3)),
                                           f32(P(RSTD3)), f32(P(U_NEXT)), f32(P(GATE_WS_NEXT)), d.B, d.L, D, d.H, dt, s));
    else
        RUN(svol_layernorm_fwd(P(S3), xf, f32(P(G3)), f32(P(BT3)), f32(P(M32)), P(M), P(MPOS), P(POS), M, f32(P(MEAN3)), f32(P(RSTD3)), M, D,
                               0.f, 0, nullptr, dt, s));
    return SVOL_OK;
}

int svol_video_half_bwd(const int64_t* dims, void* const* p, int phase, void* s) {
    if (!dims || !p || phase < 0 || phase > 2) return SVOL_E_INVALID;
    Trace tr_(phase == 2 ? "video_half_bwd.2" : "video_half_bwd.1", s);
    const Dims d(dims);
    if (!d.ok() || d.L <= 0 || d.F <= 0) return SVOL_E_INVALID;
    const int64_t M = d.B * d.L, D = d.D, F = d.F, dh = D / d.H;
    const int dt = d.dt, xf = dt != SVOL_F32;
    if (phase != 2) {
        RUN(svol_layernorm_bwd(f32(P(DM32)), P(DM), P(DMPOS), P(S3), xf, f32(P(G3)), f32(P(MEAN3)), f32(P(RSTD3)), f32(P(DS32_3)), P(DS3),
                               f32(P(DG3)), f32(P(DBT3)), f32(P(DB_FC2)), M, D, 0.f, 0, nullptr, dt, s));
        RUN(svol_gemm_nt_dact(P(DS3), D, P(W_FC2_T), D, P(DPRE), F, P(PRE), F, SVOL_ACT_GELU_D, f32(P(DB_FC1)), M, F, D, dt, s));
        RUN(nt(P(DPRE), F, P(W_FC1_T), F, P(DY2), D, nullptr, nullptr, M, D, F, dt, s));
        RUN(svol_layernorm_bwd(f32(P(DS32_3)), P(DY2), nullptr, P(S2), xf, f32(P(G2)), f32(P(MEAN2)), f32(P(RSTD2)), f32(P(DS32_2)), P(G2D),
                               f32(P(DG2)), f32(P(DBT2)), f32(P(DB_O)), M, D, 0.f, 0, nullptr, dt, s));
        RUN(nt(P(G2D), D, P(W_O_T), D, P(DO), D, nullptr, nullptr, M, D, D, dt, s));
    }
    if (phase != 1) {
        int aflags = 0;
        if (P(EV_CLEAN_IN)) {
            if (hipStreamWaitEvent(static_cast<hipStream_t>(s), static_cast<hipEvent_t>(P(EV_CLEAN_IN)), 0) != hipSuccess) return SVOL_E_LAUNCH;
            aflags = SVOL_ATTN_DQ_PREZEROED;
        }
        record(P(EV_A0), s);
        RUN(svol_attn_bwd_ex(P(QKV), 3 * D, at(P(QKV), D, dt), 3 * D, at(P(QKV), 2 * D, dt), 3 * D, P(O), D, P(DO), D, f32(P(LSE)),
                             f32(P(DELTA)), nullptr, P(DQKV), 3 * D, at(P(DQKV), D, dt), 3 * D, at(P(DQKV), 2 * D, dt), 3 * D, d.B, d.H, d.L,
                             d.L, dh, attn_scale(dh), attn_premul(dh, dt), P(ATTN_WS), d.ws_bytes, dt, aflags, P(EV_PREP), s));
        record(P(EV_A1), s);
        if (P(ATTN_WS_NEXT) && P(ZERO_STREAM) && P(EV_PREP) && P(EV_CLEAN_OUT)) {
            hipStream_t zs = static_cast<hipStream_t>(P(ZERO_STREAM));
            if (hipStreamWaitEvent(zs, static_cast<hipEvent_t>(P(EV_PREP)), 0) != hipSuccess) return SVOL_E_LAUNCH;
            const int zrc = svol_attn_bwd_zero_ws(P(ATTN_WS_NEXT), d.ws_bytes, d.B, d.H, d.L, d.L, dh, dt, zs);
            if (zrc) return zrc;
            record(P(EV_CLEAN_OUT), zs);
        }
        RUN(nt(P(DQKV), 3 * D, P(W_IN_T), 3 * D, P(DXQP), D, nullptr, nullptr, M, D, 2 * D, dt, s));
        RUN(nt(at(P(DQKV), 2 * D, dt), 3 * D, at(P(W_IN_T), 2 * D, dt), 3 * D, P(DXQ), D, nullptr, nullptr, M, D, D, dt, s));
        RUN(svol_gate_bwd(f32(P(DS32_2)), P(DXQ), P(DXQP), f32(P(X32)), P(POS), f32(P(U)), f32(P(G1)), f32(P(A)), f32(P(MEAN1)),
                          f32(P(RSTD1)), f32(P(GATE_WS)), f32(P(GATE_WS2)), f32(P(DX32)), f32(P(DU)), f32(P(DG1)), f32(P(DBT1)), d.B, d.L,
                          D, d.H, dt, s));
    }
    return SVOL_OK;
}

int svol_video_half_wgrad_part(const int64_t* dims, void* const* p, int part, void* s) {
    if (!dims || !p || part < 0 || part > 2) return SVOL_E_INVALID;
    Trace tr_(part == 1 ? "video_half_wgrad.1" : part == 2 ? "video_half_wgrad.2" : "video_half_wgrad", s);
    const Dims d(dims);
    if (!d.ok()) return SVOL_E_INVALID;
    const int64_t M = d.B * d.L, D = d.D, F = d.F;
    const int dt = d.dt;
    const svol_tn_problem pr[5] = {
        {P(DS3), D, P(HID), F, f32(P(DW_FC2)), F, nullptr, M, D, F},
        {P(DPRE), F, P(Y2), D, f32(P(DW_FC1)), D, nullptr, M, F, D},
        {P(G2D), D, P(O), D, f32(P(DW_O)), D, nullptr, M, D, D},
        {P(DQKV), 3 * D, P(Y1POS), D, f32(P(DW_IN)), D, f32(P(DB_IN)), M, 2 * D, D},
        {at(P(DQKV), 2 * D, dt), 3 * D, P(Y1), D, f32(P(DW_IN)) + 2 * D * D, D, f32(P(DB_IN)) + 2 * D, M, D, D}};
    if (part == 1) RUN(svol_gemm_tn_grouped(pr, 3, dt, s));
    else if (part == 2) RUN(svol_gemm_tn_grouped(pr + 3, 2, dt, s));
    else RUN(svol_gemm_tn_grouped(pr, 5, dt, s));
    return SVOL_OK;
}

int svol_video_half_wgrad(const int64_t* dims, void* const* p, void* s) { return svol_video_half_wgrad_part(dims, p, 0, s); }
#undef P

int svol_query_self_fwd(const int64_t* dims, void* const* p, void* s) {
    if (!dims || !p) return SVOL_E_INVALID;
    Trace tr_("query_self_fwd", s);
    const Dims d(dims);
    if (!d.ok() || d.N <= 0) return SVOL_E_INVALID;
    const int64_t R = d.B * d.N, D = d.D, dh = D / d.H;
    const int qdt = d.qdt, xf = qdt != SVOL_F32;
#define P(n) p[SVOL_QS_##n]
    RUN(nt(P(OPOS), D, P(W_IN), D, P(QKV), 3 * D, P(B_IN), P(QSCALE), R, 2 * D, D, qdt, s));
    if (P(WV_HILO))
        RUN(svol_gemm_nt_split(P(O), D, P(WV_HILO), 2 * D, at(P(QKV), 2 * D, qdt), 3 * D, f32(P(B_IN)) + 2 * D, R, D, D, s));
    else
        RUN(nt(P(O), D, at(P(W_IN), 2 * D * D, qdt), D, at(P(QKV), 2 * D, qdt), 3 * D, f32(P(B_IN)) + 2 * D, nullptr, R, D, D, qdt, s));
    RUN(svol_attn_fwd(P(QKV), 3 * D, at(P(QKV), D, qdt), 3 * D, at(P(QKV), 2 * D, qdt), 3 * D, P(OA), D, f32(P(LSE)), nullptr, d.B, d.H,
                      d.N, d.N, dh, attn_scale(dh), attn_premul(dh, qdt), P(ATTN_WS), d.ws_bytes, qdt, s));
    RUN(nt_res(P(OA), D, P(W_O), D, P(S4), P(B_O), P(O32), R, D, D, qdt, s));
    RUN(svol_layernorm_fwd(P(S4), xf, f32(P(G4)), f32(P(BT4)), f32(P(Y32)), P(Y), P(YPOS), P(QPOS), d.N, f32(P(MEAN4)), f32(P(RSTD4)), R, D,
                           0.f, 0, nullptr, qdt, s));
    return SVOL_OK;
}

int svol_query_self_bwd(const int64_t* dims, void* const* p, void* s) {
    if (!dims || !p) return SVOL_E_INVALID;
    Trace tr_("query_self_bwd", s);
    const Dims d(dims);
// ... 41 lines not shown
    if (mixed) {
        RUN(nt(P(OPOS), D, P(W_INQ), D, P(Q), D, P(B_IN), P(QSCALE), R, D, D, qdt, s));
        RUN(svol_cast(P(Q), qdt, P(QC), dt, R * D, s));
    } else {
        RUN(nt(P(OPOS), D, P(W_KV), D, P(QC), D, P(B_IN), P(QSCALE), R, D, D, dt, s));
    }
    RUN(nt(P(MPOS), D, at(P(W_KV), D * D, dt), D, P(KV), 2 * D, f32(P(B_IN)) + D, nullptr, M, D, D, dt, s));
    if (P(WV_HILO))
        RUN(svol_gemm_nt_split(P(MV), D, P(WV_HILO), 2 * D, at(P(KV), D, dt), 2 * D, f32(P(B_IN)) + 2 * D, M, D, D, s));
    else
        RUN(nt(P(MV), D, at(P(W_KV), 2 * D * D, dt), D, at(P(KV), D, dt), 2 * D, f32(P(B_IN)) + 2 * D, nullptr, M, D, D, dt, s));
    RUN(svol_attn_fwd(P(QC), D, P(KV), 2 * D, at(P(KV), D, dt), 2 * D, P(OA), D, f32(P(LSE)), f32(P(KBIAS)), d.B, d.H, d.N, d.L, dh,
                      attn_scale(dh), attn_premul(dh, dt), P(ATTN_WS), d.ws_bytes, dt, s));
    const void* oq = P(OA);
    if (mixed) {
        RUN(svol_cast(P(OA), dt, P(OAQ), qdt, R * D, s));
        oq = P(OAQ);
    }
    RUN(nt_res(oq, D, P(W_O), D, P(S5), P(B_O), P(O32), R, D, D, qdt, s));
    RUN(svol_layernorm_fwd(P(S5), xf, f32(P(G5)), f32(P(BT5)), f32(P(Y5_32)), P(Y5), nullptr, nullptr, 0, f32(P(MEAN5)), f32(P(RSTD5)), R,
                           D, 0.f, 0, nullptr, qdt, s));
    RUN(svol_gemm_nt(P(Y5), D, nullptr, 0, P(W_FC1), D, P(HID), F, f32(P(B_FC1)), nullptr, SVOL_ACT_GELU, P(PRE), F, nullptr, 0, 0, R, F, D,
                     qdt, s));
    RUN(nt_res(P(HID), F, P(W_FC2), F, P(S6), P(B_FC2), P(Y5_32), R, D, F, qdt, s));
    RUN(svol_layernorm_fwd(P(S6), xf, f32(P(G6)), f32(P(BT6)), f32(P(Y32)), P(Y), P(YPOS), P(QPOS), d.N, f32(P(MEAN6)), f32(P(RSTD6)), R, D,
                           0.f, 0, nullptr, qdt, s));
    return SVOL_OK;
}

int svol_query_cross_bwd(const int64_t* dims, void* const* p, void* s) {
    if (!dims || !p) return SVOL_E_INVALID;
    Trace tr_("query_cross_bwd", s);
    const Dims d(dims);
    if (!d.ok() || d.N <= 0 || d.L <= 0 || d.F <= 0) return SVOL_E_INVALID;
    const int64_t R = d.B * d.N, M = d.B * d.L, D = d.D, F = d.F, dh = D / d.H;
    const int dt = d.dt, qdt = d.qdt, xf = qdt != SVOL_F32;
    const bool mixed = qdt != dt;
    RUN(svol_layernorm_bwd(f32(P(DY32)), P(DY), P(DYPOS), P(S6), xf, f32(P(G6)), f32(P(MEAN6)), f32(P(RSTD6)), f32(P(DS32_6)), P(DS6),
                           f32(P(DG6)), f32(P(DBT6)), f32(P(DB_FC2)), R, D, 0.f, 0, nullptr, qdt, s));
    if (P(DQPOS) && P(DYPOS)) RUN(svol_colsum(P(DYPOS), d.N * D, f32(P(DQPOS)), d.B, d.N * D, qdt, s));
    RUN(svol_gemm_nt_dact(P(DS6), D, P(W_FC2_T), D, P(DPRE), F, P(PRE), F, SVOL_ACT_GELU, f32(P(DB_FC1)), R, F, D, qdt, s));
    RUN(nt(P(DPRE), F, P(W_FC1_T), F, P(DY5), D, nullptr, nullptr, R, D, F, qdt, s));
    RUN(svol_layernorm_bwd(f32(P(DS32_6)), P(DY5), nullptr, P(S5), xf, f32(P(G5)), f32(P(MEAN5)), f32(P(RSTD5)), f32(P(DO32)), P(G5D),
                           f32(P(DG5)), f32(P(DBT5)), f32(P(DB_O)), R, D, 0.f, 0, nullptr, qdt, s));
    RUN(nt(P(G5D), D, P(W_O_T), D, P(DOAQ), D, nullptr, nullptr, R, D, D, qdt, s));
    const void* d_o = P(DOAQ);
    if (mixed) {
        RUN(svol_cast(P(DOAQ), qdt, P(DOA), dt, R * D, s));
        d_o = P(DOA);
    }
    RUN(svol_attn_bwd(P(QC), D, P(KV), 2 * D, at(P(KV), D, dt), 2 * D, P(OA), D, d_o, D, f32(P(LSE)), f32(P(DELTA)), f32(P(KBIAS)), P(DQC), D,
                      P(DKV), 2 * D, at(P(DKV), D, dt), 2 * D, d.B, d.H, d.N, d.L, dh, attn_scale(dh), attn_premul(dh, dt), P(ATTN_WS),
                      d.ws_bytes, dt, s));
    RUN(nt(P(DKV), 2 * D, at(P(W_KV_T), D, dt), 3 * D, P(DMPOS), D, nullptr, nullptr, M, D, D, dt, s));
    RUN(nt(at(P(DKV), D, dt), 2 * D, at(P(W_KV_T), 2 * D, dt), 3 * D, P(DMV), D, nullptr, nullptr, M, D, D, dt, s));
    const void* dq = P(DQC);
    if (mixed) {
        RUN(svol_cast(P(DQC), dt, P(DQ), qdt, R * D, s));
        dq = P(DQ);
    }
    RUN(nt(dq, D, mixed ? P(W_INQ_T) : P(W_KV_T), 3 * D, P(DXQP), D, nullptr, nullptr, R, D, D, qdt, s));
    return SVOL_OK;
}

int svol_query_cross_wgrad(const int64_t* dims, void* const* p, void* s) {
    if (!dims || !p) return SVOL_E_INVALID;
    Trace tr_("query_cross_wgrad", s);
    const Dims d(dims);
    if (!d.ok()) return SVOL_E_INVALID;
    const int64_t R = d.B * d.N, M = d.B * d.L, D = d.D, F = d.F;
    const int dt = d.dt, qdt = d.qdt;
    const bool mixed = qdt != dt;
    const svol_tn_problem pv[2] = {
        {P(DKV), 2 * D, P(MPOS), D, f32(P(DW_IN)) + D * D, D, f32(P(DB_IN)) + D, M, D, D},
        {at(P(DKV), D, dt), 2 * D, P(MV), D, f32(P(DW_IN)) + 2 * D * D, D, f32(P(DB_IN)) + 2 * D, M, D, D}};
    RUN(svol_gemm_tn_grouped(pv, 2, dt, s));
    const svol_tn_problem pq[4] = {
        {P(DS6), D, P(HID), F, f32(P(DW_FC2)), F, nullptr, R, D, F},
        {P(DPRE), F, P(Y5), D, f32(P(DW_FC1)), D, nullptr, R, F, D},
        {P(G5D), D, mixed ? P(OAQ) : P(OA), D, f32(P(DW_O)), D, nullptr, R, D, D},
        {mixed ? P(DQ) : P(DQC), D, P(OPOS), D, f32(P(DW_IN)), D, f32(P(DB_IN)), R, D, D}};
    RUN(svol_gemm_tn_grouped(pq, 4, qdt, s));
    return SVOL_OK;
#undef P
}

}
```

### svol_amd/csrc/common.h

```cpp
#pragma once
#include <hip/hip_runtime.h>
#include <stdint.h>

#include "../../include/svol_hip.h"

typedef __bf16 bf16_t;
typedef __attribute__((ext_vector_type(8))) __bf16 bf16x8;
typedef __attribute__((ext_vector_type(4))) __bf16 bf16x4;
typedef __attribute__((ext_vector_type(2))) __bf16 bf16x2;
typedef _Float16 f16_t;
typedef __attribute__((ext_vector_type(8))) _Float16 f16x8;
typedef __attribute__((ext_vector_type(4))) _Float16 f16x4;
typedef __attribute__((ext_vector_type(2))) _Float16 f16x2;
typedef __attribute__((ext_vector_type(4))) float f32x4;
typedef __attribute__((ext_vector_type(16))) float f32x16;

#ifdef SVOL_H16_FP16
typedef f16_t h16_t;
typedef f16x8 h16x8;
typedef f16x4 h16x4;
typedef f16x2 h16x2;
#define SVOL_MFMA_16x16x32_H16 __builtin_amdgcn_mfma_f32_16x16x32_f16
#define SVOL_MFMA_32x32x16_H16 __builtin_amdgcn_mfma_f32_32x32x16_f16
#define SVOL_DS_READ_TR16_H16 svol_ds_read_tr16_f16
#define SVOL_H16_ASM "f16"
#define SVOL_H16_ONE2 0x3C003C00u
#define SVOL_H16_NINF_LO 0x0000FC00u
#define SVOL_H16_DTYPE SVOL_F16
#define SVOL_H16_NEG_BIG (-6.0e4f)
#define SVOL_H16_PSUM_MAX 6.5e4f
#define svol_gemm_nt_bf16_fast svol_gemm_nt_f16_fast
#define svol_gemm_tn_bf16_fast svol_gemm_tn_f16_fast
#define svol_gemm_tn_bf16_grouped svol_gemm_tn_f16_grouped
#define svol_conv_wgrad_bf16_fast svol_conv_wgrad_f16_fast
#define svol_gemm_ws_bf16 svol_gemm_ws_f16
#define svol_gemm_n256_bf16 svol_gemm_n256_f16
#define svol_attn_fwd_bf16_launch svol_attn_fwd_f16_launch
#define svol_attn_bwd_bf16_launch svol_attn_bwd_f16_launch
#define svol_attn_ws_floats_bf16 svol_attn_ws_floats_f16
#define svol_attn_sp_image_bytes_bf16 svol_attn_sp_image_bytes_f16
#define svol_attn_sp_zero_bf16_launch svol_attn_sp_zero_f16_launch
#else
typedef bf16_t h16_t;
typedef bf16x8 h16x8;
typedef bf16x4 h16x4;
typedef bf16x2 h16x2;
#define SVOL_MFMA_16x16x32_H16 __builtin_amdgcn_mfma_f32_16x16x32_bf16
#define SVOL_MFMA_32x32x16_H16 __builtin_amdgcn_mfma_f32_32x32x16_bf16
#define SVOL_DS_READ_TR16_H16 __builtin_amdgcn_ds_read_tr16_b64_v4bf16
#define SVOL_H16_ASM "bf16"
#define SVOL_H16_ONE2 0x3F803F80u
#define SVOL_H16_NINF_LO 0x0000FF80u
#define SVOL_H16_DTYPE SVOL_BF16
#define SVOL_H16_NEG_BIG (-3.0e38f)
#define SVOL_H16_PSUM_MAX 1.0e30f
#endif
typedef __attribute__((ext_vector_type(4))) short i16x4;
__device__ __forceinline__ f16x4 svol_ds_read_tr16_f16(__attribute__((address_space(3))) f16x4* p) {
    return __builtin_bit_cast(f16x4, __builtin_amdgcn_ds_read_tr16_b64_v4i16((__attribute__((address_space(3))) i16x4*)p));
}
typedef __attribute__((ext_vector_type(2))) float f32x2;
__device__ __forceinline__ h16x2 cvt_pk_h16(float a, float b) {
#ifdef SVOL_H16_FP16
    return __builtin_convertvector((f32x2){a, b}, f16x2);
#else
    return h16x2{(bf16_t)a, (bf16_t)b};
#endif
}
static inline bool svol_is16(int dtype) { return dtype == SVOL_BF16 || dtype == SVOL_F16; }

template <typename T> struct H16;
template <> struct H16<bf16_t> {
    typedef bf16x8 v8;
    typedef bf16x4 v4;
    typedef __attribute__((address_space(3))) bf16x4* lds_v4_ptr;
    static __device__ __forceinline__ f32x4 mfma16(v8 a, v8 b, f32x4 c) { return __builtin_amdgcn_mfma_f32_16x16x32_bf16(a, b, c, 0, 0, 0); }
    static __device__ __forceinline__ f32x16 mfma32(v8 a, v8 b, f32x16 c) { return __builtin_amdgcn_mfma_f32_32x32x16_bf16(a, b, c, 0, 0, 0); }
    static __device__ __forceinline__ v4 read_tr(lds_v4_ptr p) { return __builtin_amdgcn_ds_read_tr16_b64_v4bf16(p); }
};
template <> struct H16<f16_t> {
    typedef f16x8 v8;
    typedef f16x4 v4;
    typedef __attribute__((address_space(3))) f16x4* lds_v4_ptr;
    static __device__ __forceinline__ f32x4 mfma16(v8 a, v8 b, f32x4 c) { return __builtin_amdgcn_mfma_f32_16x16x32_f16(a, b, c, 0, 0, 0); }
    static __device__ __forceinline__ f32x16 mfma32(v8 a, v8 b, f32x16 c) { return __builtin_amdgcn_mfma_f32_32x32x16_f16(a, b, c, 0, 0, 0); }
    static __device__ __forceinline__ v4 read_tr(lds_v4_ptr p) { return svol_ds_read_tr16_f16(p); }
};

#define SVOL_CHECK_LAUNCH()                                   \
    do {                                                      \
        if (hipGetLastError() != hipSuccess) return SVOL_E_LAUNCH; \
    } while (0)

static inline bool aligned16(const void* p) { return (reinterpret_cast<uintptr_t>(p) & 15u) == 0; }
__device__ __forceinline__ bool nonfinite(float x) { return !(fabsf(x) <= 3.0e38f); }

#include <cstdlib>
static inline bool svol_deterministic() {
    static const bool det = getenv("SVOL_DETERMINISTIC") != nullptr;
    return det;
}

struct DetScratch {
    float* p = nullptr;
    hipStream_t s;
    DetScratch(size_t floats, hipStream_t s_, bool zero = false) : s(s_) {
        if (floats == 0) return;
        hipStreamCaptureStatus cap = hipStreamCaptureStatusNone;
        if (hipStreamIsCapturing(s, &cap) != hipSuccess || cap != hipStreamCaptureStatusNone) return;
        if (hipMallocAsync(reinterpret_cast<void**>(&p), floats * sizeof(float), s) != hipSuccess) p = nullptr;
        if (p && zero && hipMemsetAsync(p, 0, floats * sizeof(float), s) != hipSuccess) { (void)hipFreeAsync(p, s); p = nullptr; }
    }
    ~DetScratch() { if (p) (void)hipFreeAsync(p, s); }
    DetScratch(const DetScratch&) = delete;
    DetScratch& operator=(const DetScratch&) = delete;
};
#ifdef __HIPCC__
namespace {
__global__ __launch_bounds__(256) void det_fold_kernel(const float* __restrict__ part, int parts, int64_t pstride, float* __restrict__ dst,
                                                       int64_t n, int64_t bpart, int64_t bdst) {
    const int64_t j = (int64_t)blockIdx.x * 256 + threadIdx.x;
    if (j >= n) return;
// ... 148 lines not shown
```

### svol_amd/csrc/gemm.hip

```cpp
#include <cstdlib>

#include "common.h"

namespace {

template <typename T> struct Tr;
template <> struct Tr<bf16_t> { static constexpr int EPC = 8; };
template <> struct Tr<f16_t> { static constexpr int EPC = 8; };
template <> struct Tr<float> { static constexpr int EPC = 4; };

__device__ __forceinline__ void mma_chunk(f32x4& acc, const uint4& a, const uint4& b, bf16_t) {
    acc = __builtin_amdgcn_mfma_f32_16x16x32_bf16(__builtin_bit_cast(bf16x8, a), __builtin_bit_cast(bf16x8, b), acc,
                                                  0, 0, 0);
}
__device__ __forceinline__ void mma_chunk(f32x4& acc, const uint4& a, const uint4& b, f16_t) {
    acc = __builtin_amdgcn_mfma_f32_16x16x32_f16(__builtin_bit_cast(f16x8, a), __builtin_bit_cast(f16x8, b), acc, 0, 0, 0);
}
__device__ __forceinline__ void mma_chunk(f32x4& acc, const uint4& a, const uint4& b, float) {
    f32x4 af = __builtin_bit_cast(f32x4, a), bf = __builtin_bit_cast(f32x4, b);
#pragma unroll
    for (int e = 0; e < 4; ++e) acc = __builtin_amdgcn_mfma_f32_16x16x4f32(af[e], bf[e], acc, 0, 0, 0);
}

struct NtArgs {
// ... 473 lines not shown
        }
    } else {
        if (mv) {
            const f32x4 x = *reinterpret_cast<const f32x4*>(p.aux + (int64_t)m * p.ldaux + n0);
#pragma unroll
            for (int e = 0; e < 4; ++e) v[e] *= p.act == SVOL_ACT_RELU ? (x[e] > 0.f ? 1.f : 0.f) : (p.act == SVOL_ACT_GELU_D ? x[e] : dgelu_f(x[e]));
        } else {
            v = f32x4{0.f, 0.f, 0.f, 0.f};
        }
        if (p.colsum) {
            __syncthreads();
            *reinterpret_cast<f32x4*>(&red[0][row][c0]) = v;
            __syncthreads();
            if (tid < SKF_T) {
                float sacc = 0.f;
#pragma unroll 8
                for (int i = 0; i < SKF_T; ++i) sacc += red[0][i][tid];
                atomicAdd(p.colsum + bn + tid, sacc);
            }
        }
    }
    if (mv) *reinterpret_cast<f32x4*>(p.C + (int64_t)m * p.ldc + n0) = v;
}

inline bool skinny_f32_ok(int64_t M, int64_t N, int64_t K, int64_t lda, int64_t ldb, int64_t ldc, const void* A, const void* B,
                          const void* C) {
    constexpr int64_t max_m = 2048;
    return M <= max_m && K % 128 == 0 && N % 32 == 0 && lda % 4 == 0 && ldb % 4 == 0 && ldc % 4 == 0 && aligned16(A) &&
           aligned16(B) && aligned16(C) && (M + 31) / 32 <= 65535;
}

inline int grid_1d(int64_t n, int block) {
    int64_t g = (n + block - 1) / block;
    return (int)(g > 4096 ? 4096 : (g < 1 ? 1 : g));
}

}

int svol_gemm_tn_bf16_fast(const void* A, int64_t lda, const void* B, int64_t ldb, float* C, int64_t ldc, float* colsum,
                           int64_t Mc, int64_t N, int64_t K, hipStream_t s);
int svol_gemm_nt_bf16_fast(const void* A, int64_t lda, const void* B, int64_t ldb, void* C, int64_t ldc, const float* bias,
                           int act, void* pre, int64_t ldp, const void* res, int64_t ldr, int out_f32, const void* aux,
                           int64_t ldaux, float* colsum, int epi, const float* colscale, int64_t M, int64_t N, int64_t K,
                           int64_t kwrap, hipStream_t s);

int svol_gemm_tn_f16_fast(const void* A, int64_t lda, const void* B, int64_t ldb, float* C, int64_t ldc, float* colsum,
                          int64_t Mc, int64_t N, int64_t K, hipStream_t s);
int svol_gemm_tn_bf16_grouped(const svol_tn_problem* pr, int n, hipStream_t s);
int svol_gemm_tn_f16_grouped(const svol_tn_problem* pr, int n, hipStream_t s);
int svol_gemm_nt_f16_fast(const void* A, int64_t lda, const void* B, int64_t ldb, void* C, int64_t ldc, const float* bias,
                          int act, void* pre, int64_t ldp, const void* res, int64_t ldr, int out_f32, const void* aux,
                          int64_t ldaux, float* colsum, int epi, const float* colscale, int64_t M, int64_t N, int64_t K,
                          int64_t kwrap, hipStream_t s);

static int tn_generic_plan(const void* A, int64_t lda, const void* B, int64_t ldb, float* C, int64_t ldc, float* colsum, int64_t Mc,
                           int64_t N, int64_t K, int dtype, TnArgs& out, int64_t& wgs) {
    const int epc = svol_is16(dtype) ? 8 : 4;
    if (N % epc || K % epc || lda % epc || ldb % epc) return SVOL_E_UNSUPPORTED;
    if (!aligned16(A) || !aligned16(B)) return SVOL_E_INVALID;
    if (Mc > (1 << 30) || N > (1 << 30) || K > (1 << 30)) return SVOL_E_UNSUPPORTED;
    const int ct = svol_is16(dtype) ? 64 : 32;
    const int64_t tiles = ((N + 127) / 128) * ((K + 127) / 128);
    constexpr int small_wgs = 64;
    const int target_wgs = (dtype == SVOL_F32 && Mc <= 4096) ? small_wgs : (tiles <= 8 ? 256 : 512);
    int64_t want = (target_wgs + tiles - 1) / tiles;
    if (svol_deterministic()) want = 1;
    int64_t chunk = (Mc + want - 1) / want;
    chunk = ((chunk + ct - 1) / ct) * ct;
    const int64_t floor_rows = (dtype == SVOL_F32 && Mc <= 4096) ? ct : 4 * ct;
    if (chunk < floor_rows) chunk = floor_rows;
    int64_t splits = (Mc + chunk - 1) / chunk;
    if (splits > 8 && splits % 8) {
        const int64_t s8 = (splits + 7) / 8 * 8;
        int64_t c8 = (Mc + s8 - 1) / s8;
        c8 = ((c8 + ct - 1) / ct) * ct;
        if (c8 >= floor_rows && (Mc + c8 - 1) / c8 == s8) { chunk = c8; splits = s8; }
    }
    const int64_t ktiles = (K + 127) / 128;
    if (splits * tiles > (1ll << 30)) return SVOL_E_UNSUPPORTED;
    out = TnArgs{A, B, C, colsum, lda, ldb, ldc, (int)Mc, (int)N, (int)K, (int)chunk, (int)ktiles, (int)splits};
    wgs = splits * tiles;
    return SVOL_OK;
}

extern "C" {

int svol_abi_version(void) { return 7; }

const char* svol_strerror(int code) {
    switch (code) {
        case SVOL_OK: return "ok";
        case SVOL_E_INVALID: return "invalid argument (null pointer, bad size or misaligned buffer)";
        case SVOL_E_UNSUPPORTED: return "shape not supported by the gfx950 kernels";
        case SVOL_E_LAUNCH: return "kernel launch failed";
        default: return "unknown error";
    }
}

static int gemm_nt_impl(const void* A, int64_t lda, const void* A2, int64_t n_split, const void* B, int64_t ldb, void* C,
                        int64_t ldc, const float* bias, const float* colscale, int act, void* pre_act_out, int64_t ldp,
                        const void* residual, int64_t ldr, int out_f32, int64_t M, int64_t N, int64_t K, int64_t kwrap, int dtype,
                        void* stream) {
    if (!A || !B || !C || M < 0 || N < 0 || K <= 0) return SVOL_E_INVALID;
    if (act == SVOL_ACT_GELU_D && !pre_act_out) return SVOL_E_INVALID;
    if (M == 0 || N == 0) return SVOL_OK;
    const int epc = svol_is16(dtype) ? 8 : 4;
// ... 30 lines not shown
    } else if (small) {
        hipLaunchKernelGGL((gemm_nt_kernel<float, float, 64>), g64, dim3(256), 0, s, p);
    } else {
        hipLaunchKernelGGL((gemm_nt_kernel<float, float>), grid, dim3(256), 0, s, p);
    }
    SVOL_CHECK_LAUNCH();
    return SVOL_OK;
}

int svol_gemm_nt(const void* A, int64_t lda, const void* A2, int64_t n_split, const void* B, int64_t ldb, void* C,
                 int64_t ldc, const float* bias, const float* colscale, int act, void* pre_act_out, int64_t ldp,
                 const void* residual, int64_t ldr, int out_f32, int64_t M, int64_t N, int64_t K, int dtype, void* stream) {
    return gemm_nt_impl(A, lda, A2, n_split, B, ldb, C, ldc, bias, colscale, act, pre_act_out, ldp, residual, ldr, out_f32, M, N, K, K,
                        dtype, stream);
}

int svol_gemm_nt_split(const void* A, int64_t lda, const void* W_hilo, int64_t ldw, void* C, int64_t ldc, const float* bias,
                       int64_t M, int64_t N, int64_t K, void* stream) {
    if (K <= 0 || K % 8) return SVOL_E_UNSUPPORTED;
    return gemm_nt_impl(A, lda, nullptr, 0, W_hilo, ldw, C, ldc, bias, nullptr, SVOL_ACT_NONE, nullptr, 0, nullptr, 0, 0, M, N, 2 * K, K,
                        SVOL_BF16, stream);
}

int svol_gemm_nt_dact(const void* A, int64_t lda, const void* B, int64_t ldb, void* C, int64_t ldc, const void* aux,
                      int64_t ldaux, int act, float* colsum, int64_t M, int64_t N, int64_t K, int dtype, void* stream) {
    if (!A || !B || !C || !aux || M < 0 || N < 0 || K <= 0) return SVOL_E_INVALID;
    if (act != SVOL_ACT_GELU && act != SVOL_ACT_RELU && act != SVOL_ACT_GELU_D) return SVOL_E_INVALID;
    if (M == 0 || N == 0) return SVOL_OK;
    if (colsum && svol_deterministic()) {
        const int rc = svol_gemm_nt_dact(A, lda, B, ldb, C, ldc, aux, ldaux, act, nullptr, M, N, K, dtype, stream);
        return rc ? rc : svol_colsum(C, ldc, colsum, M, N, dtype, stream);
    }
    hipStream_t s = reinterpret_cast<hipStream_t>(stream);
    if (svol_is16(dtype)) {
        const int rc = (dtype == SVOL_BF16 ? svol_gemm_nt_bf16_fast : svol_gemm_nt_f16_fast)(
            A, lda, B, ldb, C, ldc, nullptr, act, nullptr, 0, nullptr, 0, 0, aux, ldaux, colsum, 1, nullptr, M, N, K, K, s);
        if (rc != SVOL_E_UNSUPPORTED) return rc;
    }
    if (dtype == SVOL_F32 && skinny_f32_ok(M, N, K, lda, ldb, ldc, A, B, C) && ldaux % 4 == 0 && aligned16(aux)) {
        SkArgs q{(const float*)A, (const float*)B, (float*)C, nullptr, nullptr, nullptr, nullptr, (const float*)aux, colsum,
                 lda, ldb, ldc, 0, 0, ldaux, (int)M, (int)N, (int)K, act, 1};
        hipLaunchKernelGGL(gemm_nt_f32_skinny, dim3((unsigned)(N / 32), (unsigned)((M + 31) / 32)), dim3(256), 0, s, q);
        SVOL_CHECK_LAUNCH();
        return SVOL_OK;
    }
    if (ldc != N || ldaux != N) return SVOL_E_UNSUPPORTED;
    int rc = svol_gemm_nt(A, lda, nullptr, 0, B, ldb, C, ldc, nullptr, nullptr, SVOL_ACT_NONE, nullptr, 0, nullptr, 0, 0, M, N, K,
                          dtype, stream);
    if (rc) return rc;
    rc = svol_act_bwd(C, aux, C, act, M * N, dtype, stream);
    if (rc) return rc;
    if (colsum) rc = svol_colsum(C, ldc, colsum, M, N, dtype, stream);
    return rc;
}

int svol_gemm_nt_dgelu(const void* A, int64_t lda, const void* B, int64_t ldb, void* C, int64_t ldc, const void* pre,
                       int64_t ldp, float* colsum, int64_t M, int64_t N, int64_t K, int dtype, void* stream) {
    return svol_gemm_nt_dact(A, lda, B, ldb, C, ldc, pre, ldp, SVOL_ACT_GELU, colsum, M, N, K, dtype, stream);
}

int svol_gemm_tn(const void* A, int64_t lda, const void* B, int64_t ldb, float* C, int64_t ldc, float* colsum, int64_t Mc,
                 int64_t N, int64_t K, int dtype, void* stream) {
    if (!A || !B || !C || Mc < 0 || N <= 0 || K <= 0) return SVOL_E_INVALID;
    if (Mc == 0) return SVOL_OK;
    if (!svol_is16(dtype) && dtype != SVOL_F32) return SVOL_E_INVALID;
    if (svol_is16(dtype)) {
        const int rc = (dtype == SVOL_BF16 ? svol_gemm_tn_bf16_fast : svol_gemm_tn_f16_fast)(A, lda, B, ldb, C, ldc, colsum, Mc, N, K,
                                                                                              reinterpret_cast<hipStream_t>(stream));
        if (rc != SVOL_E_UNSUPPORTED) return rc;
    }
    TnArgs p{};
    int64_t wgs = 0;
    const int prc = tn_generic_plan(A, lda, B, ldb, C, ldc, colsum, Mc, N, K, dtype, p, wgs);
    if (prc) return prc;
    const int64_t splits = 1, tiles = wgs;
    dim3 grid((unsigned)(splits * tiles));
    hipStream_t s = reinterpret_cast<hipStream_t>(stream);
    if (dtype == SVOL_BF16) hipLaunchKernelGGL(gemm_tn_kernel<bf16_t>, grid, dim3(256), 0, s, p);
    else if (dtype == SVOL_F16) hipLaunchKernelGGL(gemm_tn_kernel<f16_t>, grid, dim3(256), 0, s, p);
    else hipLaunchKernelGGL(gemm_tn_kernel<float>, grid, dim3(256), 0, s, p);
    SVOL_CHECK_LAUNCH();
    return SVOL_OK;
}

int svol_gemm_tn_grouped(const svol_tn_problem* pr, int32_t n, int dtype, void* stream) {
    if (!pr || n < 0) return SVOL_E_INVALID;
    if (!svol_is16(dtype) && dtype != SVOL_F32) return SVOL_E_INVALID;
    hipStream_t s = reinterpret_cast<hipStream_t>(stream);
    for (int32_t i0 = 0; i0 < n; i0 += SVOL_TN_GROUP_MAX) {
        const int m = (int)((n - i0 < SVOL_TN_GROUP_MAX) ? n - i0 : SVOL_TN_GROUP_MAX);
        int rc = SVOL_E_UNSUPPORTED;
        bool ok = m > 1;
        for (int i = 0; ok && i < m; ++i) ok = pr[i0 + i].A && pr[i0 + i].B && pr[i0 + i].C && pr[i0 + i].Mc > 0 && pr[i0 + i].N > 0 && pr[i0 + i].K > 0;
        if (ok && svol_is16(dtype)) {
            rc = (dtype == SVOL_BF16 ? svol_gemm_tn_bf16_grouped : svol_gemm_tn_f16_grouped)(pr + i0, m, s);
        } else if (ok) {
            TnGroupArgsG g{};
            g.n = m;
            int64_t tot = 0;
            rc = SVOL_OK;
            for (int i = 0; i < m && rc == SVOL_OK; ++i) {
                int64_t wgs = 0;
                const svol_tn_problem& q = pr[i0 + i];
                rc = tn_generic_plan(q.A, q.lda, q.B, q.ldb, q.C, q.ldc, q.colsum, q.Mc, q.N, q.K, dtype, g.a[i], wgs);
                g.begin[i] = (int)tot;
                tot += wgs;
// ... 135 lines not shown
```

### svol_amd/csrc/gemm_ws_bf16.hip

```cpp
#include <cstdlib>

#include "common.h"

namespace {

struct WsArgs {
    const h16_t* A; const h16_t* W; void* C;
    const float* bias; const float* colscale; h16_t* pre; const void* res; const h16_t* aux; float* colsum;
    int64_t lda, ldw, ldc, ldp, ldr, ldaux;
    int M, N, act, tiles_per_wg, nchunk;
};

typedef __attribute__((address_space(3))) void* lds_void_ptr;

constexpr int WS_K = 256;
constexpr int TR = 16;
constexpr int A_PLANE = TR * WS_K * 2;

typedef unsigned u32x4_t __attribute__((ext_vector_type(4)));

template <int N> __device__ __forceinline__ void ws_wait_vm() { asm volatile("s_waitcnt vmcnt(%0)" ::"n"(N) : "memory"); }
__device__ __forceinline__ void ws_wait_vm_dyn(int n) {
    switch (n) {
#define C_(x) case x: ws_wait_vm<x>(); break;
        C_(0) C_(1) C_(2) C_(3) C_(4) C_(5) C_(6) C_(7) C_(8) C_(9) C_(10) C_(11) C_(12) C_(13) C_(14) C_(15) C_(16)
        C_(17) C_(18) C_(19) C_(20) C_(21) C_(22) C_(23) C_(24) C_(25) C_(26) C_(27) C_(28) C_(29) C_(30) C_(31) C_(32)
#undef C_
        default: ws_wait_vm<32>(); break;
    }
}

__device__ __forceinline__ int ws_col(int t, int i) { return (t >> 1) * 32 + (i >> 2) * 8 + (t & 1) * 4 + (i & 3); }

template <int MODE> struct WsCfg;
template <> struct WsCfg<0> { static constexpr int SLOT = A_PLANE, STG = 4, ND = 2; };
template <> struct WsCfg<1> { static constexpr int SLOT = A_PLANE + TR * 256 * 4, STG = 3, ND = 6; };
template <> struct WsCfg<2> { static constexpr int SLOT = 2 * A_PLANE, STG = 4, ND = 4; };

template <int MODE>
__device__ __forceinline__ void gemm_ws_body(const WsArgs& p) {
    constexpr int SLOT = WsCfg<MODE>::SLOT, STG = WsCfg<MODE>::STG, ND = WsCfg<MODE>::ND;
    __shared__ __attribute__((aligned(1024))) char smem[STG * SLOT];
    const int tid = threadIdx.x, lane = tid & 63;
    const int wave = __builtin_amdgcn_readfirstlane(tid >> 6);
    const int fr = lane & 15, fq = lane >> 4;
    const int chunk_id = blockIdx.x % p.nchunk, cg = blockIdx.x / p.nchunk;
    const int cg0 = cg * 256;
    const int c0 = cg0 + wave * 64;
    const bool active = c0 < p.N;
    const int tile0 = chunk_id * p.tiles_per_wg;
    const int row_base = tile0 * TR;
    const int rows_here = min(p.tiles_per_wg * TR, p.M - row_base);
    const int ntile = (rows_here + TR - 1) / TR;
    const int ns = !active ? 0 : (MODE == 0 ? (p.pre ? 4 : 2) : (MODE == 1 ? 4 : 2));

    const __amdgpu_buffer_rsrc_t rA = __builtin_amdgcn_make_buffer_rsrc(
        (void*)(p.A + (int64_t)row_base * p.lda), 0, (int)((((int64_t)rows_here - 1) * p.lda + WS_K) * 2), 0x00020000);
    int voffA[2];
#pragma unroll
    for (int j = 0; j < 2; ++j) {
        const int row = (wave * 2 + j) * 2 + (lane >> 5), s = lane & 31;
        voffA[j] = (int)(((int64_t)row * p.lda + ((s ^ row) & 31) * 8) * 2);
    }
    __amdgpu_buffer_rsrc_t rX = rA;
    int voffX[4] = {0, 0, 0, 0};
    if constexpr (MODE == 1) {
        const float* R = reinterpret_cast<const float*>(p.res) + (int64_t)row_base * p.ldr + cg0;
        const int cols = min(256, p.N - cg0);
        rX = __builtin_amdgcn_make_buffer_rsrc((void*)R, 0, (int)((((int64_t)rows_here - 1) * p.ldr + cols) * 4), 0x00020000);
#pragma unroll
        for (int j = 0; j < 4; ++j) {
            const int row = wave * 4 + j, s = lane;
            voffX[j] = (int)(((int64_t)row * p.ldr + (((s & 48) | ((s ^ row) & 15))) * 4) * 4);
        }
    } else if constexpr (MODE == 2) {
        const h16_t* X = p.aux + (int64_t)row_base * p.ldaux + cg0;
        const int cols = min(256, p.N - cg0);
        rX = __builtin_amdgcn_make_buffer_rsrc((void*)X, 0, (int)((((int64_t)rows_here - 1) * p.ldaux + cols) * 2), 0x00020000);
#pragma unroll
        for (int j = 0; j < 2; ++j) {
            const int row = (wave * 2 + j) * 2 + (lane >> 5), s = lane & 31;
            voffX[j] = (int)(((int64_t)row * p.ldaux + ((s ^ row) & 31) * 8) * 2);
        }
    }
    auto issue = [&](int slot, int tile) {
        char* sl = smem + slot * SLOT;
        const int soA = (int)((int64_t)tile * TR * p.lda * 2);
#pragma unroll
        for (int j = 0; j < 2; ++j)
            __builtin_amdgcn_raw_ptr_buffer_load_lds(rA, (lds_void_ptr)(sl + (wave * 2 + j) * 1024), 16, voffA[j], soA, 0, 0);
// ... 146 lines not shown
                const unsigned xb = sl + A_PLANE + (unsigned)(fr * 512);
                const unsigned q0 = (unsigned)(((wave * 8 + fq) ^ fr) & 31), q1 = (unsigned)(((wave * 8 + 4 + fq) ^ fr) & 31);
                asm volatile(
                    "ds_read_b128 %0, %2\n\t"
                    "ds_read_b128 %1, %3\n\t"
                    "s_waitcnt lgkmcnt(0)"
                    : "=&v"(ax[0]), "=&v"(ax[1])
                    : "v"(xb + q0 * 16), "v"(xb + q1 * 16)
                    : "memory");
            }
            const bool ok = active && m < p.M;
#pragma unroll
            for (int hf = 0; hf < 2; ++hf) {
                const h16x8 a8 = __builtin_bit_cast(h16x8, ax[hf]);
                h16x8 o;
#pragma unroll
                for (int e = 0; e < 8; ++e) {
                    float d = v[hf][e] * dact_fast((float)a8[e], p.act);
                    d = ok ? d : 0.f;
                    csum[hf][e] += d;
                    o[e] = (h16_t)d;
                }
                if (ok) *reinterpret_cast<h16x8*>(reinterpret_cast<h16_t*>(p.C) + (int64_t)m * p.ldc + c0 + hf * 32 + fq * 8) = o;
            }
        }
    }
    if constexpr (MODE == 2) {
        if (p.colsum) {
#pragma unroll
            for (int hf = 0; hf < 2; ++hf)
#pragma unroll
                for (int e = 0; e < 8; ++e) {
                    float s = csum[hf][e];
                    s += __shfl_xor(s, 1, 64);
                    s += __shfl_xor(s, 2, 64);
                    s += __shfl_xor(s, 4, 64);
                    s += __shfl_xor(s, 8, 64);
                    if (fr == 0 && active) atomicAdd(p.colsum + c0 + hf * 32 + fq * 8 + e, s);
                }
        }
    }
}

__global__ __launch_bounds__(256, 2) void gemm_ws_bf16_m0(WsArgs p) { gemm_ws_body<0>(p); }
__global__ __launch_bounds__(256, 2) void gemm_ws_bf16_m1(WsArgs p) { gemm_ws_body<1>(p); }
__global__ __launch_bounds__(256, 2) void gemm_ws_bf16_m2(WsArgs p) { gemm_ws_body<2>(p); }


__device__ __forceinline__ void store_b128_guarded(u32x4_t v, __amdgpu_buffer_rsrc_t rsrc, int voffset, int soffset) {
    __builtin_amdgcn_raw_buffer_store_b128(v, rsrc, voffset, soffset, 0);
    asm volatile("s_nop 1" ::"v"(v));
}

template <int MODE, int ACT, bool PRE, bool SCALE, int VPM>
__device__ __forceinline__ void gemm_wsp_body(const WsArgs& p) {
    static_assert(MODE == 0 || MODE == 2, "bf16 outputs only");
    constexpr int SLOT = WsCfg<MODE>::SLOT, STG = 4, ND = WsCfg<MODE>::ND;
    constexpr int NS = MODE == 0 ? (PRE ? 4 : 2) : 2;
    __shared__ __attribute__((aligned(1024))) char smem[STG * SLOT];
    const int tid = threadIdx.x, lane = tid & 63;
    const int wave = __builtin_amdgcn_readfirstlane(tid >> 6);
    const int fr = lane & 15, fq = lane >> 4;
    const int chunk_id = blockIdx.x % p.nchunk, cg = blockIdx.x / p.nchunk;
    const int cg0 = cg * 256;
    const int c0 = cg0 + wave * 64;
    const bool active = c0 < p.N;
    const int tile0 = chunk_id * p.tiles_per_wg;
    const int row_base = tile0 * TR;
    const int rows_here = min(p.tiles_per_wg * TR, p.M - row_base);
    const int ntile = (rows_here + TR - 1) / TR;

    const __amdgpu_buffer_rsrc_t rA = __builtin_amdgcn_make_buffer_rsrc(
        (void*)(p.A + (int64_t)row_base * p.lda), 0, (int)((((int64_t)rows_here - 1) * p.lda + WS_K) * 2), 0x00020000);
    int voffA[2];
#pragma unroll
    for (int j = 0; j < 2; ++j) {
        const int row = (wave * 2 + j) * 2 + (lane >> 5), s = lane & 31;
        voffA[j] = (int)(((int64_t)row * p.lda + ((s ^ row) & 31) * 8) * 2);
    }
    __amdgpu_buffer_rsrc_t rX = rA;
    int voffX[2] = {0, 0};
    if constexpr (MODE == 2) {
        const h16_t* X = p.aux + (int64_t)row_base * p.ldaux + cg0;
        const int cols = min(256, p.N - cg0);
        rX = __builtin_amdgcn_make_buffer_rsrc((void*)X, 0, (int)((((int64_t)rows_here - 1) * p.ldaux + cols) * 2), 0x00020000);
#pragma unroll
        for (int j = 0; j < 2; ++j) {
            const int row = (wave * 2 + j) * 2 + (lane >> 5), s = lane & 31;
            voffX[j] = (int)(((int64_t)row * p.ldaux + ((s ^ row) & 31) * 8) * 2);
        }
    }
    auto issue = [&](int slot, int tile) {
        char* sl = smem + slot * SLOT;
        const int soA = (int)((int64_t)tile * TR * p.lda * 2);
#pragma unroll
        for (int j = 0; j < 2; ++j)
            __builtin_amdgcn_raw_ptr_buffer_load_lds(rA, (lds_void_ptr)(sl + (wave * 2 + j) * 1024), 16, voffA[j], soA, 0, 0);
        if constexpr (MODE == 2) {
            const int so = (int)((int64_t)tile * TR * p.ldaux * 2);
#pragma unroll
            for (int j = 0; j < 2; ++j)
                __builtin_amdgcn_raw_ptr_buffer_load_lds(rX, (lds_void_ptr)(sl + A_PLANE + (wave * 2 + j) * 1024), 16, voffX[j], so, 0, 0);
        }
    };

    uint4 wf[4][8];
#pragma unroll
    for (int t = 0; t < 4; ++t) {
        const h16_t* wrow = p.W + (int64_t)(c0 + ws_col(t, fr)) * p.ldw + fq * 8;
#pragma unroll
        for (int ks = 0; ks < 8; ++ks) wf[t][ks] = active ? *reinterpret_cast<const uint4*>(wrow + ks * 32) : make_uint4(0, 0, 0, 0);
    }
    float bias8[2][8], scale8[2][8];
#pragma unroll
    for (int hf = 0; hf < 2; ++hf)
#pragma unroll
        for (int e = 0; e < 8; ++e) {
            const int n = c0 + hf * 32 + fq * 8 + e;
            bias8[hf][e] = (MODE == 0 && active && p.bias) ? p.bias[n] : 0.f;
            scale8[hf][e] = (MODE == 0 && SCALE && active && p.colscale) ? p.colscale[n] : 1.f;
        }
    float csum[2][8];
#pragma unroll
    for (int hf = 0; hf < 2; ++hf)
#pragma unroll
        for (int e = 0; e < 8; ++e) csum[hf][e] = 0.f;

    const unsigned lds0 = (unsigned)(size_t)(lds_void_ptr)smem;
    const unsigned aoff = (unsigned)(fr * 512 + ((fq ^ fr) & 3) * 16);
    const unsigned ax_x = (unsigned)((fr & 12) * 16);
    const unsigned xq0 = (unsigned)(A_PLANE + fr * 512 + (((wave * 8 + fq) ^ fr) & 31) * 16);
    const unsigned xq1 = (unsigned)(A_PLANE + fr * 512 + (((wave * 8 + 4 + fq) ^ fr) & 31) * 16);
    const __amdgpu_buffer_rsrc_t rC = __builtin_amdgcn_make_buffer_rsrc(
        (void*)(reinterpret_cast<h16_t*>(p.C) + (int64_t)row_base * p.ldc), 0,
        active ? (int)((((int64_t)rows_here - 1) * p.ldc + p.N) * 2) : 0, 0x00020000);
    const __amdgpu_buffer_rsrc_t rP = __builtin_amdgcn_make_buffer_rsrc(
        (void*)(PRE ? p.pre + (int64_t)row_base * p.ldp : nullptr), 0,
        (PRE && active) ? (int)((((int64_t)rows_here - 1) * p.ldp + p.N) * 2) : 0, 0x00020000);
    const int voffC = (int)(((int64_t)fr * p.ldc + c0 + fq * 8) * 2), voffP = (int)(((int64_t)fr * p.ldp + c0 + fq * 8) * 2);
    const int cstep = (int)(TR * p.ldc * 2), pstep = (int)(TR * p.ldp * 2);

    u32x4_t af[8], ax[2] = {u32x4_t{0, 0, 0, 0}, u32x4_t{0, 0, 0, 0}};
    auto read_frags = [&](int slot) {
        const unsigned sl = lds0 + (unsigned)(slot * SLOT);
        const unsigned b = sl + aoff;
        asm volatile(
            "ds_read_b128 %0, %8\n\t"
            "ds_read_b128 %1, %9\n\t"
            "ds_read_b128 %2, %10\n\t"
            "ds_read_b128 %3, %11\n\t"
            "ds_read_b128 %4, %8 offset:256\n\t"
            "ds_read_b128 %5, %9 offset:256\n\t"
            "ds_read_b128 %6, %10 offset:256\n\t"
            "ds_read_b128 %7, %11 offset:256"
            : "=&v"(af[0]), "=&v"(af[1]), "=&v"(af[2]), "=&v"(af[3]), "=&v"(af[4]), "=&v"(af[5]), "=&v"(af[6]), "=&v"(af[7])
            : "v"(b + ((0u * 64) ^ ax_x)), "v"(b + ((1u * 64) ^ ax_x)), "v"(b + ((2u * 64) ^ ax_x)), "v"(b + ((3u * 64) ^ ax_x))
            : "memory");
        if constexpr (MODE == 2) {
            asm volatile(
                "ds_read_b128 %0, %2\n\t"
                "ds_read_b128 %1, %3"
                : "=&v"(ax[0]), "=&v"(ax[1])
                : "v"(sl + xq0), "v"(sl + xq1)
                : "memory");
        }
    };
    auto wait_frags = [&]() {
        asm volatile("s_waitcnt lgkmcnt(0)"
                     : "+v"(af[0]), "+v"(af[1]), "+v"(af[2]), "+v"(af[3]), "+v"(af[4]), "+v"(af[5]), "+v"(af[6]), "+v"(af[7]),
                       "+v"(ax[0]), "+v"(ax[1]));
    };
    auto mfma_slab = [&](f32x4 (&acc)[4]) {
#pragma unroll
        for (int t = 0; t < 4; ++t) acc[t] = f32x4{0.f, 0.f, 0.f, 0.f};
#pragma unroll
        for (int ks = 0; ks < 8; ++ks)
#pragma unroll
            for (int t = 0; t < 4; ++t)
                acc[t] = SVOL_MFMA_16x16x32_H16(__builtin_bit_cast(h16x8, wf[t][ks]),
                                                                 __builtin_bit_cast(h16x8, af[ks]), acc[t], 0, 0, 0);
    };
    auto epilogue = [&](int j, const f32x4 (&acc)[4], const u32x4_t (&axj)[2]) {
        float v[2][8];
#pragma unroll
        for (int hf = 0; hf < 2; ++hf)
#pragma unroll
            for (int e = 0; e < 8; ++e) v[hf][e] = acc[2 * hf + (e >> 2)][e & 3];
        if constexpr (MODE == 0) {
#pragma unroll
            for (int hf = 0; hf < 2; ++hf)
#pragma unroll
                for (int e = 0; e < 8; ++e) {
                    v[hf][e] += bias8[hf][e];
                    if constexpr (SCALE) v[hf][e] *= scale8[hf][e];
                }
            if constexpr (PRE) {
                h16x8 o[2];
#pragma unroll
                for (int hf = 0; hf < 2; ++hf)
#pragma unroll
                    for (int e = 0; e < 8; ++e) o[hf][e] = (h16_t)pre_save_fast(v[hf][e], ACT);
                store_b128_guarded(__builtin_bit_cast(u32x4_t, o[0]), rP, voffP, j * pstep);
                store_b128_guarded(__builtin_bit_cast(u32x4_t, o[1]), rP, voffP + 64, j * pstep);
            }
            h16x8 o[2];
#pragma unroll
            for (int hf = 0; hf < 2; ++hf)
#pragma unroll
                for (int e = 0; e < 8; ++e) {
                    float y = v[hf][e];
                    if constexpr (ACT == SVOL_ACT_GELU || ACT == SVOL_ACT_GELU_D) y = gelu_fast(y);
                    if constexpr (ACT == SVOL_ACT_RELU) y = fmaxf(y, 0.f);
                    o[hf][e] = (h16_t)y;
                }
            store_b128_guarded(__builtin_bit_cast(u32x4_t, o[0]), rC, voffC, j * cstep);
            store_b128_guarded(__builtin_bit_cast(u32x4_t, o[1]), rC, voffC + 64, j * cstep);
        } else {
            h16x8 o[2];
#pragma unroll
            for (int hf = 0; hf < 2; ++hf) {
                const h16x8 a8 = __builtin_bit_cast(h16x8, axj[hf]);
#pragma unroll
                for (int e = 0; e < 8; ++e) {
                    const float d = v[hf][e] * dact_fast((float)a8[e], ACT);
                    csum[hf][e] += d;
                    o[hf][e] = (h16_t)d;
                }
            }
            store_b128_guarded(__builtin_bit_cast(u32x4_t, o[0]), rC, voffC, j * cstep);
            store_b128_guarded(__builtin_bit_cast(u32x4_t, o[1]), rC, voffC + 64, j * cstep);
        }
    };

#pragma unroll
    for (int s = 0; s < STG; ++s)
        if (s < ntile) issue(s, s);
    ws_wait_vm_dyn(ND * min(STG - 1, ntile - 1));
    __builtin_amdgcn_s_barrier();
    read_frags(0);
    wait_frags();
    f32x4 acc[4];
    mfma_slab(acc);
    for (int j = 0; j + 1 < ntile; ++j) {
        const int nd = min(STG - 2, ntile - 2 - j), nst = min(j, STG - 1);
        if (nd == STG - 2 && nst == STG - 1) ws_wait_vm<ND * (STG - 2) + NS * (STG - 1)>();
        else ws_wait_vm_dyn(ND * nd + NS * nst);
        __builtin_amdgcn_s_barrier();
        if (j + STG < ntile) issue(j % STG, j + STG);
        f32x4 accp[4];
        u32x4_t axp[2];
#pragma unroll
        for (int t = 0; t < 4; ++t) accp[t] = acc[t];
        axp[0] = ax[0];
        axp[1] = ax[1];
        read_frags((j + 1) % STG);
        wait_frags();
        mfma_slab(acc);
        epilogue(j, accp, axp);
#pragma unroll
        for (int i = 0; i < 32; ++i) {
            __builtin_amdgcn_sched_group_barrier(0x008, 1, 0);
            __builtin_amdgcn_sched_group_barrier(0x002, VPM, 0);
        }
    }
    {
        u32x4_t axp[2] = {ax[0], ax[1]};
        epilogue(ntile - 1, acc, axp);
    }
    if constexpr (MODE == 2) {
        if (p.colsum) {
#pragma unroll
            for (int hf = 0; hf < 2; ++hf)
#pragma unroll
                for (int e = 0; e < 8; ++e) {
                    float s = csum[hf][e];
                    s += __shfl_xor(s, 1, 64);
                    s += __shfl_xor(s, 2, 64);
                    s += __shfl_xor(s, 4, 64);
                    s += __shfl_xor(s, 8, 64);
                    if (fr == 0 && active) atomicAdd(p.colsum + c0 + hf * 32 + fq * 8 + e, s);
                }
        }
    }
}

#define WSP_KERNEL(name, MODE, ACT, PRE, SCALE, VPM) \
    __global__ __launch_bounds__(256, 2) void name(WsArgs p) { gemm_wsp_body<MODE, ACT, PRE, SCALE, VPM>(p); }
WSP_KERNEL(gemm_wsp_bf16_none, 0, SVOL_ACT_NONE, false, false, 2)
WSP_KERNEL(gemm_wsp_bf16_none_scale, 0, SVOL_ACT_NONE, false, true, 2)
WSP_KERNEL(gemm_wsp_bf16_gelu, 0, SVOL_ACT_GELU, false, false, 7)
WSP_KERNEL(gemm_wsp_bf16_gelu_pre, 0, SVOL_ACT_GELU, true, false, 8)
WSP_KERNEL(gemm_wsp_bf16_gelu_dpre, 0, SVOL_ACT_GELU_D, true, false, 9)
WSP_KERNEL(gemm_wsp_bf16_relu, 0, SVOL_ACT_RELU, false, false, 2)
WSP_KERNEL(gemm_wsp_bf16_dgelu, 2, SVOL_ACT_GELU, false, false, 9)
WSP_KERNEL(gemm_wsp_bf16_dmul, 2, SVOL_ACT_GELU_D, false, false, 3)
WSP_KERNEL(gemm_wsp_bf16_drelu, 2, SVOL_ACT_RELU, false, false, 3)
#undef WSP_KERNEL

}

int svol_gemm_ws_bf16(const void* A, int64_t lda, const void* W, int64_t ldw, void* C, int64_t ldc, const float* bias, int act,
                      void* pre, int64_t ldp, const void* res, int64_t ldr, int out_f32, const void* aux, int64_t ldaux,
                      float* colsum, int epi, const float* colscale, int64_t M, int64_t N, int64_t K, hipStream_t s) {
    if (K != WS_K || N % 64 || M < 4096) return SVOL_E_UNSUPPORTED;
    int mode;
    if (epi == 1) {
        if (!aux || out_f32) return SVOL_E_UNSUPPORTED;
        mode = 2;
    } else if (out_f32) {
        if (!res || act != SVOL_ACT_NONE || pre || colscale) return SVOL_E_UNSUPPORTED;
        mode = 1;
    } else {
        if (res || (act != SVOL_ACT_NONE && act != SVOL_ACT_GELU && act != SVOL_ACT_RELU && act != SVOL_ACT_GELU_D)) return SVOL_E_UNSUPPORTED;
        if (act == SVOL_ACT_GELU_D && !pre) return SVOL_E_INVALID;
        mode = 0;
    }
    auto al16 = [](const void* p_) { return (reinterpret_cast<uintptr_t>(p_) & 15) == 0; };
    if (lda % 8 || ldw % 8 || !al16(A) || !al16(W) || !al16(C)) return SVOL_E_UNSUPPORTED;
    if (mode == 1 ? (ldc % 4 || ldr % 4 || !al16(res)) : (ldc % 8 != 0)) return SVOL_E_UNSUPPORTED;
    if (pre && (ldp % 8 || !al16(pre))) return SVOL_E_UNSUPPORTED;
    if (mode == 2 && (ldaux % 8 || !al16(aux))) return SVOL_E_UNSUPPORTED;
    const int64_t ntile = (M + TR - 1) / TR;
    const int64_t ncg = (N + 255) / 256;
    int64_t tpw = (ntile * ncg + (ncg <= 2 ? 255 : 511)) / (ncg <= 2 ? 256 : 512);
    if (tpw < 4) tpw = 4;
    if (tpw > 64) tpw = 64;
    const int64_t ldmax = lda > ldr * 2 ? lda : ldr * 2;
    int64_t ldbig = ldmax > ldaux ? ldmax : ldaux;
    if (ldc > ldbig) ldbig = ldc;
    if (pre && ldp > ldbig) ldbig = ldp;
    if (tpw * TR * ldbig * 2 >= (1ll << 31)) return SVOL_E_UNSUPPORTED;
    int64_t nchunk = (ntile + tpw - 1) / tpw;
    if (ncg > 1 && nchunk > 8 && nchunk % 8) {
        const int64_t n8 = (nchunk + 7) / 8 * 8;
        const int64_t t8 = (ntile + n8 - 1) / n8;
        if (t8 >= 1 && (ntile + t8 - 1) / t8 == n8) { tpw = t8; nchunk = n8; }
    }
    if (nchunk * ncg > (1ll << 30)) return SVOL_E_UNSUPPORTED;
    WsArgs p{(const h16_t*)A, (const h16_t*)W, C, bias, colscale, (h16_t*)pre, res, (const h16_t*)aux, colsum,
             lda, ldw, ldc, ldp, ldr, ldaux, (int)M, (int)N, act, (int)tpw, (int)nchunk};
    dim3 grid((unsigned)(ncg * nchunk));
    void (*kp)(WsArgs) = nullptr;
    if (mode == 0) {
        if (act == SVOL_ACT_NONE && !pre) kp = colscale ? gemm_wsp_bf16_none_scale : gemm_wsp_bf16_none;
        else if (act == SVOL_ACT_GELU && !colscale) kp = pre ? gemm_wsp_bf16_gelu_pre : gemm_wsp_bf16_gelu;
        else if (act == SVOL_ACT_GELU_D && !colscale) kp = gemm_wsp_bf16_gelu_dpre;
        else if (act == SVOL_ACT_RELU && !pre && !colscale) kp = gemm_wsp_bf16_relu;
    } else if (mode == 2) {
        kp = act == SVOL_ACT_RELU ? gemm_wsp_bf16_drelu : (act == SVOL_ACT_GELU_D ? gemm_wsp_bf16_dmul : gemm_wsp_bf16_dgelu);
    }
    if (kp) hipLaunchKernelGGL(kp, grid, dim3(256), 0, s, p);
    else if (mode == 0) hipLaunchKernelGGL(gemm_ws_bf16_m0, grid, dim3(256), 0, s, p);
    else if (mode == 1) hipLaunchKernelGGL(gemm_ws_bf16_m1, grid, dim3(256), 0, s, p);
    else hipLaunchKernelGGL(gemm_ws_bf16_m2, grid, dim3(256), 0, s, p);
    return hipGetLastError() == hipSuccess ? SVOL_OK : SVOL_E_LAUNCH;
}
```

### svol_amd/csrc/norm.hip

```cpp
#include "common.h"

namespace {

constexpr int LN_MAX_PASSES = 4;

template <typename T, typename TX, int NP>
__global__ __launch_bounds__(256) void ln_fwd_kernel(const TX* __restrict__ x, const float* __restrict__ gamma,
                                                     const float* __restrict__ beta, float* __restrict__ y32,
                                                     T* __restrict__ y, T* __restrict__ ypos, const T* __restrict__ pos,
                                                     int64_t pos_rows, float* __restrict__ mean, float* __restrict__ rstd,
                                                     int64_t M, int D, float p, float inv_keep, uint64_t seed0,
                                                     const int64_t* __restrict__ soff) {
    const uint64_t seed = seed0 + (soff ? ((uint64_t)soff[0] << 8) : 0ull);
    const int lane = threadIdx.x & 63;
    const int64_t row = (int64_t)blockIdx.x * 4 + (threadIdx.x >> 6);
    if (row >= M) return;
    const TX* xr = x + row * D;
    float v[NP][4];
    float s = 0.f;
    const T* pr = pos ? pos + (row % pos_rows) * D : nullptr;
    Vec4<TX> t[NP];
    Vec4<T> pv[NP];
    Vec4<float> gv[NP], bv[NP];
#pragma unroll
// ... 235 lines not shown
        int64_t r = i / row_len;
        int64_t k = i - r * row_len;
        uint32_t rm = drop_row(s0, (uint64_t)r);
#pragma unroll
        for (int e = 0; e < 4; ++e) {
            if (i + e >= n) break;
            out[i + e] = res[i + e] + t[i + e] * drop_scale_rk(rm, (uint32_t)k, p, inv_keep);
            if (++k == row_len) { k = 0; ++r; rm = drop_row(s0, (uint64_t)r); }
        }
    }
}
}

extern "C" {

int svol_layernorm_fwd(const void* x, int x_f32, const float* gamma, const float* beta, float* y32, void* y,
                       void* ypos, const void* pos, int64_t pos_rows, float* mean, float* rstd, int64_t M, int64_t D,
                       float dropout_p, uint64_t seed, const int64_t* seed_offset_dev, int dtype, void* stream) {
    if (!x || !gamma || !beta || (!y && !y32) || !mean || !rstd || M < 0 || D <= 0) return SVOL_E_INVALID;
    if (!aligned16(gamma) || !aligned16(beta)) return SVOL_E_INVALID;
    if ((ypos != nullptr) != (pos != nullptr)) return SVOL_E_INVALID;
    if (pos && pos_rows <= 0) return SVOL_E_INVALID;
    if (D % 4 || D > LN_MAX_PASSES * 256) return SVOL_E_UNSUPPORTED;
    if (dropout_p < 0.f || dropout_p >= 1.f) return SVOL_E_INVALID;
    if (!svol_is16(dtype) && dtype != SVOL_F32) return SVOL_E_INVALID;
    if (M == 0) return SVOL_OK;
    const float inv_keep = 1.f / (1.f - dropout_p);
    const unsigned grid = (unsigned)((M + 3) / 4);
    hipStream_t s = reinterpret_cast<hipStream_t>(stream);
#define SVOL_LNF(TT, TXX, NPP)                                                                                              \
    hipLaunchKernelGGL((ln_fwd_kernel<TT, TXX, NPP>), dim3(grid), dim3(256), 0, s, (const TXX*)x, gamma, beta, y32, (TT*)y,      \
                       (TT*)ypos, (const TT*)pos, pos_rows, mean, rstd, M, (int)D, dropout_p, inv_keep, seed, seed_offset_dev)
#define SVOL_LNF_NP(TT, TXX)                     \
    do {                                         \
        if (D <= 256) SVOL_LNF(TT, TXX, 1);      \
        else if (D <= 512) SVOL_LNF(TT, TXX, 2); \
        else SVOL_LNF(TT, TXX, 4);               \
    } while (0)
    if (dtype == SVOL_BF16 && x_f32) SVOL_LNF_NP(bf16_t, float);
    else if (dtype == SVOL_BF16) SVOL_LNF_NP(bf16_t, bf16_t);
    else if (dtype == SVOL_F16 && x_f32) SVOL_LNF_NP(f16_t, float);
    else if (dtype == SVOL_F16) SVOL_LNF_NP(f16_t, f16_t);
    else SVOL_LNF_NP(float, float);
#undef SVOL_LNF_NP
#undef SVOL_LNF
    SVOL_CHECK_LAUNCH();
    return SVOL_OK;
}

int svol_layernorm_bwd(const float* dy32, const void* dy, const void* dy2, const void* x, int x_f32, const float* gamma,
                       const float* mean, const float* rstd, float* dx32, void* dx, float* dgamma, float* dbeta,
                       float* dx_colsum, int64_t M, int64_t D, float dropout_p, uint64_t seed, const int64_t* seed_offset_dev,
                       int dtype, void* stream) {
    if ((!dy32 && !dy && !dy2) || !x || !gamma || !mean || !rstd || (!dx && !dx32) || !dgamma || !dbeta || M < 0 || D <= 0)
        return SVOL_E_INVALID;
    if (D % 4 || D > LN_MAX_PASSES * 256) return SVOL_E_UNSUPPORTED;
    if (dropout_p < 0.f || dropout_p >= 1.f) return SVOL_E_INVALID;
    if (!svol_is16(dtype) && dtype != SVOL_F32) return SVOL_E_INVALID;
    if (M == 0) return SVOL_OK;
    const float inv_keep = 1.f / (1.f - dropout_p);
    int64_t rpw = (M + 2047) / 2048;
    if (rpw < 1) rpw = 1;
    const int64_t waves = (M + rpw - 1) / rpw;
    const unsigned grid = (unsigned)((waves + 3) / 4);
    hipStream_t s = reinterpret_cast<hipStream_t>(stream);
    const bool det_mode = svol_deterministic();
    DetScratch det(det_mode ? (size_t)grid * 3 * (size_t)D : 0, s);
    if (det_mode && !det.p) return SVOL_E_LAUNCH;
#define SVOL_LNB(TT, TXX, NPP)                                                                                                      \
    hipLaunchKernelGGL((ln_bwd_kernel<TT, TXX, NPP>), dim3(grid), dim3(256), 0, s, dy32, (const TT*)dy, (const TT*)dy2, (const TXX*)x, \
                       gamma, mean, rstd, dx32, (TT*)dx, dgamma, dbeta, dx_colsum, M, (int)D, dropout_p, inv_keep, seed,              \
                       seed_offset_dev, (int)rpw, det.p)
#define SVOL_LNB_NP(TT, TXX)                  \
    do {                                      \
        if (D <= 256) SVOL_LNB(TT, TXX, 1);   \
        else if (D <= 512) SVOL_LNB(TT, TXX, 2); \
        else SVOL_LNB(TT, TXX, 4);            \
    } while (0)
    if (dtype == SVOL_BF16 && x_f32) SVOL_LNB_NP(bf16_t, float);
    else if (dtype == SVOL_BF16) SVOL_LNB_NP(bf16_t, bf16_t);
    else if (dtype == SVOL_F16 && x_f32) SVOL_LNB_NP(f16_t, float);
    else if (dtype == SVOL_F16) SVOL_LNB_NP(f16_t, f16_t);
    else SVOL_LNB_NP(float, float);
#undef SVOL_LNB_NP
#undef SVOL_LNB
    if (det_mode) {
        det_fold(det.p, (int)grid, 3 * D, dgamma, D, s);
        det_fold(det.p + D, (int)grid, 3 * D, dbeta, D, s);
        det_fold(det.p + 2 * D, (int)grid, 3 * D, dx_colsum, D, s);
    }
    SVOL_CHECK_LAUNCH();
    return SVOL_OK;
}

int svol_dropout(const void* x, void* y, int64_t n, int64_t row_len, float p, uint64_t seed, int dtype, void* stream) {
    if (!x || !y || n < 0 || row_len <= 0 || row_len > 0xffffffffll || !(p >= 0.f && p < 1.f)) return SVOL_E_INVALID;
    if (n == 0) return SVOL_OK;
    const float inv = 1.f / (1.f - p);
    int64_t g = (n + 1023) / 1024;
    if (g > 8192) g = 8192;
    hipStream_t s = reinterpret_cast<hipStream_t>(stream);
    if (dtype == SVOL_F32) hipLaunchKernelGGL(dropout_kernel<float>, dim3((unsigned)g), dim3(256), 0, s, (const float*)x, (float*)y, n, row_len, p, inv, seed);
    else if (dtype == SVOL_BF16) hipLaunchKernelGGL(dropout_kernel<bf16_t>, dim3((unsigned)g), dim3(256), 0, s, (const bf16_t*)x, (bf16_t*)y, n, row_len, p, inv, seed);
    else if (dtype == SVOL_F16) hipLaunchKernelGGL(dropout_kernel<f16_t>, dim3((unsigned)g), dim3(256), 0, s, (const f16_t*)x, (f16_t*)y, n, row_len, p, inv, seed);
    else return SVOL_E_INVALID;
    SVOL_CHECK_LAUNCH();
    return SVOL_OK;
// ... 32 lines not shown
```

### svol_amd/ops.py

```python
from __future__ import annotations

import ctypes
import math
import os
from typing import Optional

import torch

from . import _lib

ACT_NONE, ACT_RELU, ACT_GELU, ACT_SIGMOID, ACT_RELU_RES, ACT_GELU_D = 0, 1, 2, 3, 4, 5
_DT = {torch.float32: 0, torch.bfloat16: 1, torch.float16: 2}


def _dt(t: torch.Tensor) -> int:
    try:
        return _DT[t.dtype]
    except KeyError:
        raise _lib.SvolHipError(f'unsupported dtype {t.dtype}')


_RAW_STREAM = getattr(torch._C, '_cuda_getCurrentRawStream', None)
_CUR_DEVICE = getattr(torch._C, '_cuda_getDevice', None)

# ... 723 lines not shown
                st['table'] = None
            except TypeError:
                pass
        return e.ws


weights = _WeightCache()


class GradSink:
    __slots__ = ('view', 'owner', 'bucket')

    def __init__(self, view, owner=None, bucket=-1):
        self.view, self.owner, self.bucket = view, owner, bucket


def _claim(p, needed=True):
    s = getattr(p, '_svol_sink', None) if (needed and p is not None) else None
    g = p.grad if s is not None else None
    if g is None or g.data_ptr() != s.view.data_ptr():
        return None
    return s


def _tgt(sink, shape, device):
    return sink.view if sink is not None else torch.zeros(shape, dtype=torch.float32, device=device)


def _pos_grad(dypos, pos_shape, D):
    rows = 1
    for n in pos_shape[:-1]:
        rows *= n
    g = colsum(dypos.reshape(-1, rows * D).contiguous())
    return cast(g.view(pos_shape), dypos.dtype)


class LayerNormFn(torch.autograd.Function):

    @staticmethod
    def forward(ctx, x, gamma, beta, p, seed, seed_dev):
        shp = x.shape
        x2 = x.reshape(-1, shp[-1])
        _, y, _, mean, rstd = layernorm_fwd(x2, gamma, beta, x.dtype, None, p, seed, seed_dev=seed_dev)
        ctx.save_for_backward(x2, gamma, mean, rstd, seed_dev)
        ctx.p, ctx.seed, ctx.shp = p, seed, shp
        ctx.sinks = (_claim(gamma, ctx.needs_input_grad[1]), _claim(beta, ctx.needs_input_grad[2]))
        return y.view(shp)

    @staticmethod
    def backward(ctx, dy):
        x2, gamma, mean, rstd, seed_dev = ctx.saved_tensors
        sg, sb = ctx.sinks
        _, dx, dg, db = layernorm_bwd(None, dy, None, x2, gamma, mean, rstd, x2.dtype, ctx.p, ctx.seed, seed_dev=seed_dev,
                                      dg_out=sg.view if sg else None, db_out=sb.view if sb else None)
        return dx.view(ctx.shp), None if sg else dg, None if sb else db, None, None, None


def layer_norm(x, gamma, beta, p=0.0, seed=0, seed_dev=None):
    return LayerNormFn.apply(x, gamma, beta, p, seed, seed_dev)


class LinearFn(torch.autograd.Function):

    @staticmethod
    def forward(ctx, x, W, b, act, out_f32):
        if act == ACT_GELU:
            raise _lib.SvolHipError('LinearFn: GELU is only available fused in MLPLNFn')
        shp = x.shape
        x2 = x.reshape(-1, shp[-1])
        Wc, WcT = weights.get(W, x.dtype)
        y = gemm_nt(x2, Wc, b, act, out_f32=out_f32)
        ctx.save_for_backward(x2, y if act != ACT_NONE else None)
        ctx.WcT, ctx.act, ctx.shp, ctx.has_b = WcT, act, shp, b is not None
        ctx.need_dx = ctx.needs_input_grad[0]
        epc = 4 if x.dtype == torch.float32 else 8
        ok = W.shape[0] % epc == 0
        ctx.sinks = (_claim(W, ok and ctx.needs_input_grad[1]), _claim(b, ok and ctx.needs_input_grad[2]))
        return y.view(*shp[:-1], W.shape[0])

    @staticmethod
    def backward(ctx, dy):
        x2, y = ctx.saved_tensors
        N = dy.shape[-1]
        d = dy.reshape(-1, N)
        if not d.is_contiguous():
            d = d.contiguous()
        if d.dtype != x2.dtype:
            d = cast(d, x2.dtype)
        if ctx.act != ACT_NONE:
            d = act_bwd(d, y, ctx.act)
        epc = 4 if d.dtype == torch.float32 else 8
        WcT = ctx.WcT
        Np = (N + epc - 1) // epc * epc
        if N % epc:
            dp = torch.zeros((d.shape[0], Np), dtype=d.dtype, device=d.device)
            dp[:, :N] = d
            wp = torch.zeros((WcT.shape[0], Np), dtype=WcT.dtype, device=WcT.device)
            wp[:, :N] = WcT
            d, WcT = dp, wp
        K_ = x2.shape[1]
        sW, sb = ctx.sinks
        if sW is not None and (sb is not None or not ctx.has_b):
            gemm_tn_sink(d, x2, out=sW.view, colsum=sb.view if sb else None)
            dW = db = None
        else:
            buf = torch.zeros((Np * K_ + Np,), dtype=torch.float32, device=d.device)
            dWp, dbp = buf[:Np * K_].view(Np, K_), buf[Np * K_:]
            gemm_tn(d, x2, out=dWp, colsum=dbp if ctx.has_b else None)
# ... 583 lines not shown
```

Baseline: 14850.

## Fuse attention delta/row prep into out-proj GEMM and add several backward work cuts

Adds a GEMM variant that computes dO from the out-projection and, in its epilogue, writes the attention delta, negated LSE and negated delta row planes. This lets the sparse attention backward skip its separate prep kernel. It also keeps a persistent dQ workspace that the dQ-round kernel re-zeroes, which avoids a separate zeroing pass. In addition, it merges the query-cross DMPOS gradient with the video-half path and lets LayerNorm backward skip dx when it is not needed. Together these are several unrelated changes that trade extra code paths and shape gating for fewer kernels and less memory traffic.

```diff
diff --git a/include/svol_hip.h b/include/svol_hip.h
--- a/include/svol_hip.h
+++ b/include/svol_hip.h
@@ -78,6 +78,9 @@
 int svol_gemm_nt_dact(const void* A, int64_t lda, const void* B, int64_t ldb, void* C, int64_t ldc,
                       const void* aux, int64_t ldaux, int act, float* colsum, int64_t M, int64_t N, int64_t K,
                       int dtype, void* stream);
+int svol_gemm_nt_delta(const void* A, int64_t lda, const void* W, int64_t ldw, void* d_o, int64_t lddo, const void* o, int64_t ldo,
+                       const float* lse2, float* rows, int64_t B, int64_t H, int64_t Lq, int64_t N, int64_t K, int dtype,
+                       void* stream);
 
 int svol_gemm_tn(const void* A, int64_t lda, const void* B, int64_t ldb, float* C, int64_t ldc, float* colsum,
                  int64_t Mc, int64_t N, int64_t K, int dtype, void* stream);
@@ -117,6 +120,8 @@
                   int dtype, void* stream);
 
 #define SVOL_ATTN_DQ_PREZEROED 1
+#define SVOL_ATTN_ROWS_READY 4
+#define SVOL_ATTN_DQ_LEAVE_ZERO 8
 int64_t svol_attn_bwd_sp_image_bytes(int64_t B, int64_t H, int64_t Lq, int64_t Lk, int64_t dh, int64_t ws_bytes, int dtype);
 int svol_attn_bwd_zero_ws(void* ws, int64_t ws_bytes, int64_t B, int64_t H, int64_t Lq, int64_t Lk, int64_t dh, int dtype, void* stream);
 int svol_attn_bwd_ex(const void* q, int64_t ldq, const void* k, int64_t ldk, const void* v, int64_t ldv, const void* o,
@@ -269,10 +274,10 @@
     X(Y1) X(Y1POS) X(A) X(MEAN1) X(RSTD1) X(GATE_WS) X(GATE_PRE) X(U_NEXT) X(GATE_WS_NEXT) \
     X(QKV) X(O) X(LSE) X(S2) X(Y2) X(MEAN2) X(RSTD2) X(PRE) X(HID) X(S3) \
     X(MEAN3) X(RSTD3) X(M32) X(M) X(MPOS) X(Y1_32) X(Y2_32) X(ATTN_WS) \
-    X(DM32) X(DM) X(DMPOS) X(DS32_3) X(DS3) X(DPRE) X(DY2) X(DS32_2) X(G2D) X(DO) X(DQKV) X(DELTA) X(DXQP) X(DXQ) X(GATE_WS2) \
+    X(DM32) X(DM) X(DMPOS) X(DS32_3) X(DS3) X(DPRE) X(DY2) X(DS32_2) X(G2D) X(DO) X(DQKV) X(DELTA) X(DXQ) X(GATE_WS2) \
     X(DX32) X(DU) \
     X(DG1) X(DBT1) X(DG2) X(DBT2) X(DG3) X(DBT3) X(DW_IN) X(DB_IN) X(DW_O) X(DB_O) X(DW_FC1) X(DB_FC1) X(DW_FC2) X(DB_FC2) \
-    X(EV_A0) X(EV_A1) X(EV_CLEAN_IN) X(EV_PREP) X(ATTN_WS_NEXT) X(ZERO_STREAM) X(EV_CLEAN_OUT)
+    X(EV_A0) X(EV_A1) X(EV_CLEAN_IN) X(EV_PREP) X(ATTN_WS_NEXT) X(ZERO_STREAM) X(EV_CLEAN_OUT) X(DQ_KEEP) X(DQ_CLEAN)
 #define SVOL_QS_SLOTS(X) \
     X(O32) X(O) X(OPOS) X(QPOS) X(B_IN) X(B_O) X(G4) X(BT4) X(QSCALE) X(W_IN) X(WV_HILO) X(W_O) X(W_IN_T) X(W_O_T) \
     X(QKV) X(OA) X(LSE) X(S4) X(MEAN4) X(RSTD4) X(Y32) X(Y) X(YPOS) X(ATTN_WS) \
diff --git a/svol_amd/_lib.py b/svol_amd/_lib.py
--- a/svol_amd/_lib.py
+++ b/svol_amd/_lib.py
@@ -29,6 +29,7 @@
                      _int, _p],
     'svol_gemm_nt_dgelu': [_p, _i64, _p, _i64, _p, _i64, _p, _i64, _p, _i64, _i64, _i64, _int, _p],
     'svol_gemm_nt_dact': [_p, _i64, _p, _i64, _p, _i64, _p, _i64, _int, _p, _i64, _i64, _i64, _int, _p],
+    'svol_gemm_nt_delta': [_p, _i64, _p, _i64, _p, _i64, _p, _i64, _p, _p, _i64, _i64, _i64, _i64, _i64, _int, _p],
     'svol_gemm_tn': [_p, _i64, _p, _i64, _p, _i64, _p, _i64, _i64, _i64, _int, _p],
     'svol_gemm_tn_grouped': [_p, _i32, _int, _p],
     'svol_colsum': [_p, _i64, _p, _i64, _i64, _int, _p],
diff --git a/svol_amd/blocks.py b/svol_amd/blocks.py
--- a/svol_amd/blocks.py
+++ b/svol_amd/blocks.py
@@ -369,6 +369,39 @@
     return st or None
 
 
+_DQ_KEEP = {}
+
+
+class _DqKeep:
+    __slots__ = ('buf', 'clean')
+
+    def __init__(self, dev, wsb):
+        self.buf = torch.zeros((_align(wsb, 1 << 20),), dtype=torch.uint8, device=dev)
+        self.clean = True
+
+    def bind(self, tbl):
+        tbl.set('ATTN_WS', self.buf.data_ptr())
+        tbl.set('DQ_KEEP', 1)
+        tbl.set('DQ_CLEAN', 1 if self.clean else None)
+        self.clean = False
+
+    def done(self, tbl):
+        self.clean = True
+        tbl.set('DQ_KEEP', None)
+        tbl.set('DQ_CLEAN', None)
+
+
+def _dq_keep(dev, B, H, L, dh, dt, wsb):
+    if dt == torch.float32 or torch.cuda.is_current_stream_capturing():
+        return None
+    key = (dev, ops._stream(), B, H, L, dh, dt, wsb)
+    st = _DQ_KEEP.get(key)
+    if st is None:
+        img = _lib.lib().svol_attn_bwd_sp_image_bytes(B, H, L, L, dh, wsb, ops._DT[dt])
+        st = _DQ_KEEP[key] = _DqKeep(dev, wsb) if img > 0 else False
+    return st or None
+
+
 def _vh_fwd_layout(B, L, D, H, F, e):
     M = B * L
     return [('Y1', M * D * e), ('Y1POS', M * D * e), ('A', M * 4), ('MEAN1', M * 4), ('RSTD1', M * 4), ('GATE_WS', B * H * (L + 2) * 4),
@@ -380,7 +413,7 @@
 def _vh_bwd_layout(B, L, D, H, F, e):
     M = B * L
     return [('DS32_3', M * D * 4), ('DS3', M * D * e), ('DPRE', M * F * e), ('DY2', M * D * e), ('DS32_2', M * D * 4), ('G2D', M * D * e),
-            ('DO', M * D * e), ('DQKV', M * 3 * D * e), ('DELTA', 3 * B * H * L * 4), ('DXQP', M * D * e), ('DXQ', M * D * e),
+            ('DO', M * D * e), ('DQKV', M * 3 * D * e), ('DELTA', 3 * B * H * L * 4), ('DXQ', M * D * e),
             ('GATE_WS2', (B * L + B * H) * 4), ('DX32', M * D * 4)]
 
 
@@ -489,11 +522,16 @@
             tbl.set('EV_A0', ev[0].cuda_event)
             tbl.set('EV_A1', ev[1].cuda_event)
         pz = _dq_prezero(dev, B, H, L, D // H, dt, dims[8]) if ctx.big else None
+        keep_ws = _dq_keep(dev, B, H, L, D // H, dt, dims[8]) if pz is None else None
         if pz is not None:
             pz.bind(tbl)
+        elif keep_ws is not None:
+            keep_ws.bind(tbl)
         _lib.check(L_.svol_video_half_bwd(dims, tbl.arr, 2, s), 'svol_video_half_bwd')
         if pz is not None:
             pz.advance(tbl)
+        elif keep_ws is not None:
+            keep_ws.done(tbl)
         tbl.set('EV_A0', None)
         tbl.set('EV_A1', None)
         if split:
@@ -630,17 +668,18 @@
             ('YPOS', R * D * qe)]
 
 
-def _qc_bwd_layout(B, N, L, D, H, F, e, qe):
+def _qc_bwd_layout(B, N, L, D, H, F, e, qe, merged):
     R, M = B * N, B * L
-    return [('DS32_6', R * D * 4), ('DS6', R * D * qe), ('DPRE', R * F * qe), ('DY5', R * D * qe), ('G5D', R * D * qe), ('DOAQ', R * D * qe),
+    lay = [('DS32_6', R * D * 4), ('DS6', R * D * qe), ('DPRE', R * F * qe), ('DY5', R * D * qe), ('G5D', R * D * qe), ('DOAQ', R * D * qe),
             ('DOA', R * D * e), ('DQC', R * D * e), ('DQ', R * D * qe), ('DKV', M * 2 * D * e), ('DELTA', 3 * B * H * N * 4),
-            ('DO32', R * D * 4), ('DXQP', R * D * qe), ('DMPOS', M * D * e), ('DMV', M * D * e)]
+            ('DO32', R * D * 4), ('DXQP', R * D * qe), ('DMV', M * D * e)]
+    return lay if merged else lay + [('DMPOS', M * D * e)]
 
 
 class QueryCrossFn(torch.autograd.Function):
 
     @staticmethod
-    def forward(ctx, pl, o32, o, opos, mv, mpos, kbias, qpos, *params):
+    def forward(ctx, pl, merged, o32, o, opos, mv, mpos, kbias, qpos, *params):
         ctx.set_materialize_grads(False)
         B, N, D = o.shape
         L = mv.shape[1]
@@ -667,7 +706,7 @@
         dims = _dims(B, L, N, D, H, F, dt, qdt, wsb)
         _lib.check(_lib.lib().svol_query_cross_fwd(dims, tbl.arr, ops._stream()), 'svol_query_cross_fwd')
         ctx.pl, ctx.tbl, ctx.dims, ctx.arena, ctx.shape = pl, tbl, dims, arena, (B, N, L, D, H, F)
-        ctx.n_par = len(params)
+        ctx.n_par, ctx.merged = len(params), bool(merged)
         ctx.save_for_backward(o32_, o_, opos_, mv_, mpos_, kb_, qpos)
         return (lay.view(arena, 'Y32', torch.float32, (B, N, D)), lay.view(arena, 'Y', qdt, (B, N, D)),
                 lay.view(arena, 'YPOS', qdt, (B, N, D)))
@@ -680,15 +719,18 @@
         n_par = ctx.n_par
         if dy32 is None and dy is None and dypos is None:
             pl.done(n_par > 0)
-            return (None,) * (8 + n_par)
+            return (None,) * (9 + n_par)
         dt, qdt = pl.dt, pl.qdt
         e, qe = _ESZ[dt], _ESZ[qdt]
         dev = o_.device
         cont = lambda t_: None if t_ is None else (t_ if t_.is_contiguous() else t_.contiguous())
         dy32, dy, dypos = cont(dy32), cont(dy), cont(dypos)
-        lay = _layout(('b', QC, B, N, L, D, H, F, dt, qdt), lambda: _qc_bwd_layout(B, N, L, D, H, F, e, qe))
+        merged = ctx.merged
+        lay = _layout(('b', QC, B, N, L, D, H, F, dt, qdt, merged), lambda: _qc_bwd_layout(B, N, L, D, H, F, e, qe, merged))
         tmp = torch.empty((lay.total,), dtype=torch.uint8, device=dev)
         lay.fill(tbl, tmp.data_ptr())
+        if merged:
+            tbl.set('DMPOS', None)
         tbl.set_t('DY32', dy32)
         tbl.set_t('DY', dy)
         tbl.set_t('DYPOS', dypos)
@@ -697,7 +739,7 @@
         slay.fill(tbl, scr.data_ptr())
         needs = ctx.needs_input_grad
         gq = None
-        if needs[7]:
+        if needs[8]:
             gq, _ = _qpos_target(pl, qpos, tbl, dev, N, D)
         else:
             tbl.set('DQPOS', None)
@@ -715,14 +757,16 @@
             gq = ops.cast(gq, qdt)
         vq = lambda n_, dt_: lay.view(tmp, n_, dt_, (B, N, D))
         vm = lambda n_: lay.view(tmp, n_, dt, (B, L, D))
-        return (None, vq('DO32', torch.float32), None, vq('DXQP', qdt), vm('DMV'), vm('DMPOS'), None, gq) + \
-            tuple(pl.grads_out(bufs, needs[8:], n_par > 0))
+        return (None, None, vq('DO32', torch.float32), None, vq('DXQP', qdt), vm('DMV'), None if merged else vm('DMPOS'), None, gq) + \
+            tuple(pl.grads_out(bufs, needs[9:], n_par > 0))
 
 
 def query_cross(layer, out, mv, mpos, kbias, qpos, dt, qdt):
     pl = plan(layer, QC, dt, qdt)
     o32, o, opos = out
-    return QueryCrossFn.apply(pl, o32, o, opos, mv, mpos, kbias, qpos, *pl.inputs(o32, opos, mv, mpos))
+    f = mv.grad_fn
+    merged = f is not None and f is mpos.grad_fn and isinstance(f, VideoHalfFn._backward_cls)
+    return QueryCrossFn.apply(pl, merged, o32, o, opos, mv, mpos, kbias, qpos, *pl.inputs(o32, opos, mv, mpos))
 
 
 def trace_dump() -> str:
diff --git a/svol_amd/csrc/attention.hip b/svol_amd/csrc/attention.hip
--- a/svol_amd/csrc/attention.hip
+++ b/svol_amd/csrc/attention.hip
@@ -538,7 +538,7 @@
                      int64_t lddq, void* dk, int64_t lddk, void* dv, int64_t lddv, int64_t B, int64_t H, int64_t Lq, int64_t Lk,
                      int64_t dh, float scale, float q_premul, void* ws, int64_t ws_bytes, int dtype, int flags, void* ev_prep,
                      void* stream) {
-    if (flags & ~SVOL_ATTN_DQ_PREZEROED) return SVOL_E_INVALID;
+    if (flags & ~(SVOL_ATTN_DQ_PREZEROED | SVOL_ATTN_ROWS_READY | SVOL_ATTN_DQ_LEAVE_ZERO)) return SVOL_E_INVALID;
     return attn_bwd_impl(q, ldq, k, ldk, v, ldv, o, ldo, d_o, lddo, lse2, delta, kbias, dq, lddq, dk, lddk, dv, lddv, B, H, Lq, Lk, dh,
                          scale, q_premul, ws, ws_bytes, 0.f, 0, dtype, stream, flags, ev_prep);
 }
diff --git a/svol_amd/csrc/attention_bf16.hip b/svol_amd/csrc/attention_bf16.hip
--- a/svol_amd/csrc/attention_bf16.hip
+++ b/svol_amd/csrc/attention_bf16.hip
@@ -1578,13 +1578,14 @@
     {
         const int h2 = tid >> 5, r2 = tid & 31;
         if (h2 < p.H) {
-            const int64_t si = ((int64_t)b * p.H + h2) * p.Lq + q0 + r2;
+            const int64_t si = attn_rows_index(b, h2, q0 + r2, p.H, p.Lq);
             reinterpret_cast<float*>(p.nl2)[si] = -s_lse[h2][r2];
             reinterpret_cast<float*>(p.nd2)[si] = -s_dl[h2][r2];
             p.delta[si] = s_dl[h2][r2];
         }
     }
 }
+template <bool REZERO>
 __global__ __launch_bounds__(256) void attn_dq_round_bf16(Args p) {
     const int64_t i = ((int64_t)blockIdx.x * blockDim.x + threadIdx.x) * 8;
     const int64_t W = (int64_t)p.H * 32, total = (int64_t)p.B * p.Lq * W;
@@ -1610,6 +1611,10 @@
     }
     const int64_t row = i / W, c = i % W;
     const f32x4 a = *reinterpret_cast<const f32x4*>(p.ws_dq + i), b = *reinterpret_cast<const f32x4*>(p.ws_dq + i + 4);
+    if constexpr (REZERO) {
+        *reinterpret_cast<f32x4*>(p.ws_dq + i) = f32x4{0.f, 0.f, 0.f, 0.f};
+        *reinterpret_cast<f32x4*>(p.ws_dq + i + 4) = f32x4{0.f, 0.f, 0.f, 0.f};
+    }
     h16x8 v;
 #pragma unroll
     for (int e = 0; e < 4; ++e) { v[e] = (h16_t)(a[e] * p.scale); v[4 + e] = (h16_t)(b[e] * p.scale); }
@@ -2536,7 +2541,10 @@
     const int64_t total = (int64_t)c.B * c.Lq * c.H;
     const dim3 gd((unsigned)((total + 255) / 256)), wg(256);
     hipStream_t s = c.stream;
-    auto bind_rows = [&](Args& a) { a.nl2 = reinterpret_cast<unsigned*>(c.delta + total); a.nd2 = reinterpret_cast<unsigned*>(c.delta + 2 * total); };
+    auto bind_rows = [&](Args& a) {
+        a.nl2 = reinterpret_cast<unsigned*>(c.delta + ATTN_ROWS_NL * attn_rows_total(c.B, c.H, c.Lq));
+        a.nd2 = reinterpret_cast<unsigned*>(c.delta + ATTN_ROWS_ND * attn_rows_total(c.B, c.H, c.Lq));
+    };
     void (*dq)(Args) = nullptr, (*dkdv)(Args) = nullptr;
     if (!pl.pre) hipLaunchKernelGGL(attn_delta_bf16, gd, wg, 0, s, pq);
     switch (pl.bwd) {
@@ -2548,8 +2556,13 @@
     case Bwd::bwd_sp:
         pq.ws_dq = c.ws;
         bind_rows(pq);
-        hipLaunchKernelGGL((c.flags & SVOL_ATTN_DQ_PREZEROED) ? attn_bwd_sp_prep_bf16<false> : attn_bwd_sp_prep_bf16<true>,
-                           dim3((unsigned)((int64_t)c.B * c.Lq / 32)), wg, 0, s, pq);
+        if (!(c.flags & SVOL_ATTN_ROWS_READY))
+            hipLaunchKernelGGL((c.flags & SVOL_ATTN_DQ_PREZEROED) ? attn_bwd_sp_prep_bf16<false> : attn_bwd_sp_prep_bf16<true>,
+                               dim3((unsigned)((int64_t)c.B * c.Lq / 32)), wg, 0, s, pq);
+        else if (!(c.flags & SVOL_ATTN_DQ_PREZEROED)) {
+            const int64_t n4 = (int64_t)c.B * c.Lq * c.H * 32 / 4;
+            hipLaunchKernelGGL(attn_sp_zero_image, dim3((unsigned)min((n4 + 255) / 256, (int64_t)2048)), wg, 0, s, c.ws, n4);
+        }
         break;
     case Bwd::bwd_rot_dma:
         bind_rows(pq), bind_rows(pk);
@@ -2576,7 +2589,8 @@
     if (c.ev_prep) (void)hipEventRecord(static_cast<hipEvent_t>(c.ev_prep), s);
     if (pl.bwd == Bwd::bwd_sp) {
         hipLaunchKernelGGL(attn_bwd_sp_bf16, dim3(sp_grid(c.B, c.H, c.Lk)), wg, 0, s, pq);
-        hipLaunchKernelGGL(attn_dq_round_bf16, dim3(sp_round_grid(c.B, c.H, c.Lq, c.Lk)), wg, 0, s, pq);
+        hipLaunchKernelGGL((c.flags & SVOL_ATTN_DQ_LEAVE_ZERO) ? attn_dq_round_bf16<true> : attn_dq_round_bf16<false>,
+                           dim3(sp_round_grid(c.B, c.H, c.Lq, c.Lk)), wg, 0, s, pq);
     }
     return hipGetLastError() == hipSuccess ? SVOL_OK : SVOL_E_LAUNCH;
 }
diff --git a/svol_amd/csrc/attn_call.h b/svol_amd/csrc/attn_call.h
--- a/svol_amd/csrc/attn_call.h
+++ b/svol_amd/csrc/attn_call.h
@@ -17,6 +17,10 @@
     hipStream_t stream;
 };
 
+enum { ATTN_ROWS_DELTA = 0, ATTN_ROWS_NL = 1, ATTN_ROWS_ND = 2, ATTN_ROWS_PLANES = 3 };
+static inline int64_t attn_rows_total(int64_t B, int64_t H, int64_t Lq) { return B * H * Lq; }
+__host__ __device__ static inline int64_t attn_rows_index(int64_t b, int64_t h, int64_t q, int64_t H, int64_t Lq) { return (b * H + h) * Lq + q; }
+
 template <typename A> static inline void attn_fill(A& p, const AttnCall& c) {
     p.q = c.q; p.k = c.k; p.v = c.v; p.o = c.o; p.d_o = c.d_o; p.out_o = c.out_o; p.dq = c.dq; p.dk = c.dk; p.dv = c.dv;
     p.kbias = c.kbias; p.lse2 = c.lse2; p.delta = c.delta;
diff --git a/svol_amd/csrc/blocks.hip b/svol_amd/csrc/blocks.hip
--- a/svol_amd/csrc/blocks.hip
+++ b/svol_amd/csrc/blocks.hip
@@ -75,6 +75,11 @@
         if (rc_) return rc_;                      \
         if (kTrace && Trace::cur) Trace::cur->mark(#expr); \
     } while (0)
+
+inline bool vh_rows_from_gemm(const Dims& d) {
+    return svol_is16(d.dt) && svol_attn_bwd_sp_image_bytes(d.B, d.H, d.L, d.L, d.D / d.H, d.ws_bytes, d.dt) > 0 &&
+           svol_gemm_nt_delta_shape_ok(d.B, d.H, d.L, d.D, d.D);
+}
 
 #define SLOT_NAME(n) #n ","
 const char* const kVhNames = SVOL_VH_SLOTS(SLOT_NAME);
@@ -207,7 +212,10 @@
         RUN(nt(P(DPRE), F, P(W_FC1_T), F, P(DY2), D, nullptr, nullptr, M, D, F, dt, s));
         RUN(svol_layernorm_bwd(f32(P(DS32_3)), P(DY2), nullptr, P(S2), xf, f32(P(G2)), f32(P(MEAN2)), f32(P(RSTD2)), f32(P(DS32_2)), P(G2D),
                                f32(P(DG2)), f32(P(DBT2)), f32(P(DB_O)), M, D, 0.f, 0, nullptr, dt, s));
-        RUN(nt(P(G2D), D, P(W_O_T), D, P(DO), D, nullptr, nullptr, M, D, D, dt, s));
+        if (vh_rows_from_gemm(d))
+            RUN(svol_gemm_nt_delta(P(G2D), D, P(W_O_T), D, P(DO), D, P(O), D, f32(P(LSE)), f32(P(DELTA)), d.B, d.H, d.L, D, D, dt, s));
+        else
+            RUN(nt(P(G2D), D, P(W_O_T), D, P(DO), D, nullptr, nullptr, M, D, D, dt, s));
     }
     if (phase != 1) {
         int aflags = 0;
@@ -215,6 +223,8 @@
             if (hipStreamWaitEvent(static_cast<hipStream_t>(s), static_cast<hipEvent_t>(P(EV_CLEAN_IN)), 0) != hipSuccess) return SVOL_E_LAUNCH;
             aflags = SVOL_ATTN_DQ_PREZEROED;
         }
+        if (vh_rows_from_gemm(d)) aflags |= SVOL_ATTN_ROWS_READY;
+        if (P(DQ_KEEP)) aflags |= SVOL_ATTN_DQ_LEAVE_ZERO | (P(DQ_CLEAN) ? SVOL_ATTN_DQ_PREZEROED : 0);
         record(P(EV_A0), s);
         RUN(svol_attn_bwd_ex(P(QKV), 3 * D, at(P(QKV), D, dt), 3 * D, at(P(QKV), 2 * D, dt), 3 * D, P(O), D, P(DO), D, f32(P(LSE)),
                              f32(P(DELTA)), nullptr, P(DQKV), 3 * D, at(P(DQKV), D, dt), 3 * D, at(P(DQKV), 2 * D, dt), 3 * D, d.B, d.H, d.L,
@@ -227,9 +237,8 @@
             if (zrc) return zrc;
             record(P(EV_CLEAN_OUT), zs);
         }
-        RUN(nt(P(DQKV), 3 * D, P(W_IN_T), 3 * D, P(DXQP), D, nullptr, nullptr, M, D, 2 * D, dt, s));
-        RUN(nt(at(P(DQKV), 2 * D, dt), 3 * D, at(P(W_IN_T), 2 * D, dt), 3 * D, P(DXQ), D, nullptr, nullptr, M, D, D, dt, s));
-        RUN(svol_gate_bwd(f32(P(DS32_2)), P(DXQ), P(DXQP), f32(P(X32)), P(POS), f32(P(U)), f32(P(G1)), f32(P(A)), f32(P(MEAN1)),
+        RUN(nt(P(DQKV), 3 * D, P(W_IN_T), 3 * D, P(DXQ), D, nullptr, nullptr, M, D, 3 * D, dt, s));
+        RUN(svol_gate_bwd(f32(P(DS32_2)), P(DXQ), nullptr, f32(P(X32)), P(POS), f32(P(U)), f32(P(G1)), f32(P(A)), f32(P(MEAN1)),
                           f32(P(RSTD1)), f32(P(GATE_WS)), f32(P(GATE_WS2)), f32(P(DX32)), f32(P(DU)), f32(P(DG1)), f32(P(DBT1)), d.B, d.L,
                           D, d.H, dt, s));
     }
@@ -377,8 +386,12 @@
     RUN(svol_attn_bwd(P(QC), D, P(KV), 2 * D, at(P(KV), D, dt), 2 * D, P(OA), D, d_o, D, f32(P(LSE)), f32(P(DELTA)), f32(P(KBIAS)), P(DQC), D,
                       P(DKV), 2 * D, at(P(DKV), D, dt), 2 * D, d.B, d.H, d.N, d.L, dh, attn_scale(dh), attn_premul(dh, dt), P(ATTN_WS),
                       d.ws_bytes, dt, s));
-    RUN(nt(P(DKV), 2 * D, at(P(W_KV_T), D, dt), 3 * D, P(DMPOS), D, nullptr, nullptr, M, D, D, dt, s));
-    RUN(nt(at(P(DKV), D, dt), 2 * D, at(P(W_KV_T), 2 * D, dt), 3 * D, P(DMV), D, nullptr, nullptr, M, D, D, dt, s));
+    if (P(DMPOS)) {
+        RUN(nt(P(DKV), 2 * D, at(P(W_KV_T), D, dt), 3 * D, P(DMPOS), D, nullptr, nullptr, M, D, D, dt, s));
+        RUN(nt(at(P(DKV), D, dt), 2 * D, at(P(W_KV_T), 2 * D, dt), 3 * D, P(DMV), D, nullptr, nullptr, M, D, D, dt, s));
+    } else {
+        RUN(nt(P(DKV), 2 * D, at(P(W_KV_T), D, dt), 3 * D, P(DMV), D, nullptr, nullptr, M, D, 2 * D, dt, s));
+    }
     const void* dq = P(DQC);
     if (mixed) {
         RUN(svol_cast(P(DQC), dt, P(DQ), qdt, R * D, s));
diff --git a/svol_amd/csrc/common.h b/svol_amd/csrc/common.h
--- a/svol_amd/csrc/common.h
+++ b/svol_amd/csrc/common.h
@@ -34,6 +34,7 @@
 #define svol_gemm_tn_bf16_grouped svol_gemm_tn_f16_grouped
 #define svol_conv_wgrad_bf16_fast svol_conv_wgrad_f16_fast
 #define svol_gemm_ws_bf16 svol_gemm_ws_f16
+#define svol_gemm_ws_delta_bf16 svol_gemm_ws_delta_f16
 #define svol_gemm_n256_bf16 svol_gemm_n256_f16
 #define svol_attn_fwd_bf16_launch svol_attn_fwd_f16_launch
 #define svol_attn_bwd_bf16_launch svol_attn_bwd_f16_launch
@@ -68,6 +69,7 @@
 #endif
 }
 static inline bool svol_is16(int dtype) { return dtype == SVOL_BF16 || dtype == SVOL_F16; }
+bool svol_gemm_nt_delta_shape_ok(int64_t B, int64_t H, int64_t Lq, int64_t N, int64_t K);
 
 template <typename T> struct H16;
 template <> struct H16<bf16_t> {
diff --git a/svol_amd/csrc/gemm.hip b/svol_amd/csrc/gemm.hip
--- a/svol_amd/csrc/gemm.hip
+++ b/svol_amd/csrc/gemm.hip
@@ -549,6 +549,17 @@
                           int act, void* pre, int64_t ldp, const void* res, int64_t ldr, int out_f32, const void* aux,
                           int64_t ldaux, float* colsum, int epi, const float* colscale, int64_t M, int64_t N, int64_t K,
                           int64_t kwrap, hipStream_t s);
+
+int svol_gemm_ws_delta_bf16(const void* A, int64_t lda, const void* W, int64_t ldw, void* C, int64_t ldc, const float* bias,
+                            const void* O, int64_t ldo, const float* lse2, float* rows, int64_t B, int64_t H, int64_t Lq, int64_t N,
+                            int64_t K, hipStream_t s);
+int svol_gemm_ws_delta_f16(const void* A, int64_t lda, const void* W, int64_t ldw, void* C, int64_t ldc, const float* bias,
+                           const void* O, int64_t ldo, const float* lse2, float* rows, int64_t B, int64_t H, int64_t Lq, int64_t N,
+                           int64_t K, hipStream_t s);
+
+bool svol_gemm_nt_delta_shape_ok(int64_t B, int64_t H, int64_t Lq, int64_t N, int64_t K) {
+    return K == 256 && N == H * 32 && N <= 256 && N % 64 == 0 && B * Lq >= 4096 && Lq >= 16;
+}
 
 static int tn_generic_plan(const void* A, int64_t lda, const void* B, int64_t ldb, float* C, int64_t ldc, float* colsum, int64_t Mc,
                            int64_t N, int64_t K, int dtype, TnArgs& out, int64_t& wgs) {
@@ -685,6 +696,14 @@
     if (rc) return rc;
     if (colsum) rc = svol_colsum(C, ldc, colsum, M, N, dtype, stream);
     return rc;
+}
+
+int svol_gemm_nt_delta(const void* A, int64_t lda, const void* W, int64_t ldw, void* d_o, int64_t lddo, const void* o, int64_t ldo,
+                       const float* lse2, float* rows, int64_t B, int64_t H, int64_t Lq, int64_t N, int64_t K, int dtype, void* stream) {
+    if (!A || !W || !d_o || !o || !lse2 || !rows || B <= 0 || H <= 0 || Lq <= 0 || N <= 0 || K <= 0) return SVOL_E_INVALID;
+    if (!svol_is16(dtype)) return dtype == SVOL_F32 ? SVOL_E_UNSUPPORTED : SVOL_E_INVALID;
+    return (dtype == SVOL_BF16 ? svol_gemm_ws_delta_bf16 : svol_gemm_ws_delta_f16)(A, lda, W, ldw, d_o, lddo, nullptr, o, ldo, lse2, rows, B,
+                                                                                   H, Lq, N, K, reinterpret_cast<hipStream_t>(stream));
 }
 
 int svol_gemm_nt_dgelu(const void* A, int64_t lda, const void* B, int64_t ldb, void* C, int64_t ldc, const void* pre,
diff --git a/svol_amd/csrc/gemm_ws_bf16.hip b/svol_amd/csrc/gemm_ws_bf16.hip
--- a/svol_amd/csrc/gemm_ws_bf16.hip
+++ b/svol_amd/csrc/gemm_ws_bf16.hip
@@ -1,5 +1,6 @@
 #include <cstdlib>
 
+#include "attn_call.h"
 #include "common.h"
 
 namespace {
@@ -9,6 +10,8 @@
     const float* bias; const float* colscale; h16_t* pre; const void* res; const h16_t* aux; float* colsum;
     int64_t lda, ldw, ldc, ldp, ldr, ldaux;
     int M, N, act, tiles_per_wg, nchunk;
+    const float* lse; float* rows;
+    int Lq, row_wrap, head_step, batch_step, rows_total;
 };
 
 typedef __attribute__((address_space(3))) void* lds_void_ptr;
@@ -36,6 +39,7 @@
 template <> struct WsCfg<0> { static constexpr int SLOT = A_PLANE, STG = 4, ND = 2; };
 template <> struct WsCfg<1> { static constexpr int SLOT = A_PLANE + TR * 256 * 4, STG = 3, ND = 6; };
 template <> struct WsCfg<2> { static constexpr int SLOT = 2 * A_PLANE, STG = 4, ND = 4; };
+template <> struct WsCfg<3> { static constexpr int SLOT = 2 * A_PLANE + 1024, ND = 5; };
 
 template <int MODE>
 __device__ __forceinline__ void gemm_ws_body(const WsArgs& p) {
@@ -288,11 +292,14 @@
     asm volatile("s_nop 1" ::"v"(v));
 }
 
-template <int MODE, int ACT, bool PRE, bool SCALE, int VPM>
+template <int MODE, int ACT, bool PRE, bool SCALE, int VPM, bool DELTA = false>
 __device__ __forceinline__ void gemm_wsp_body(const WsArgs& p) {
     static_assert(MODE == 0 || MODE == 2, "bf16 outputs only");
-    constexpr int SLOT = WsCfg<MODE>::SLOT, STG = 4, ND = WsCfg<MODE>::ND;
-    constexpr int NS = MODE == 0 ? (PRE ? 4 : 2) : 2;
+    static_assert(!DELTA || MODE == 2, "the delta epilogue reads the aux plane");
+    constexpr int CFG = DELTA ? 3 : MODE;
+    constexpr int SLOT = WsCfg<CFG>::SLOT, STG = 4, ND = WsCfg<CFG>::ND;
+    constexpr int NS = DELTA ? 5 : (MODE == 0 ? (PRE ? 4 : 2) : 2);
+    constexpr unsigned OOB = 0x7ffffff0u;
     __shared__ __attribute__((aligned(1024))) char smem[STG * SLOT];
     const int tid = threadIdx.x, lane = tid & 63;
     const int wave = __builtin_amdgcn_readfirstlane(tid >> 6);
@@ -326,6 +333,16 @@
             voffX[j] = (int)(((int64_t)row * p.ldaux + ((s ^ row) & 31) * 8) * 2);
         }
     }
+    const bool rows_lane = DELTA && active && lane < 32;
+    int ld_m = row_base + fr, ld_q = 0, ld_si = 0, st_m = ld_m, st_q = 0, st_si = 0;
+    __amdgpu_buffer_rsrc_t rL = rA, rR = rA;
+    if constexpr (DELTA) {
+        const int b0 = ld_m / p.Lq;
+        ld_q = st_q = ld_m - b0 * p.Lq;
+        ld_si = st_si = b0 * p.batch_step + (c0 / 32 + ((lane >> 4) & 1)) * p.head_step + ld_q;
+        rL = __builtin_amdgcn_make_buffer_rsrc((void*)p.lse, 0, p.rows_total * 4, 0x00020000);
+        rR = __builtin_amdgcn_make_buffer_rsrc((void*)p.rows, 0, ATTN_ROWS_PLANES * p.rows_total * 4, 0x00020000);
+    }
     auto issue = [&](int slot, int tile) {
         char* sl = smem + slot * SLOT;
         const int soA = (int)((int64_t)tile * TR * p.lda * 2);
@@ -338,6 +355,12 @@
             for (int j = 0; j < 2; ++j)
                 __builtin_amdgcn_raw_ptr_buffer_load_lds(rX, (lds_void_ptr)(sl + A_PLANE + (wave * 2 + j) * 1024), 16, voffX[j], so, 0, 0);
         }
+        if constexpr (DELTA) {
+            const unsigned vo = (rows_lane && ld_m < p.M) ? (unsigned)ld_si * 4u : OOB;
+            __builtin_amdgcn_raw_ptr_buffer_load_lds(rL, (lds_void_ptr)(sl + 2 * A_PLANE + wave * 256), 4, (int)vo, 0, 0, 0);
+            ld_m += TR; ld_q += TR; ld_si += TR;
+            if (ld_q >= p.Lq) { ld_q -= p.Lq; ld_si += p.row_wrap; }
+        }
     };
 
     uint4 wf[4][8];
@@ -353,7 +376,7 @@
 #pragma unroll
         for (int e = 0; e < 8; ++e) {
             const int n = c0 + hf * 32 + fq * 8 + e;
-            bias8[hf][e] = (MODE == 0 && active && p.bias) ? p.bias[n] : 0.f;
+            bias8[hf][e] = ((MODE == 0 || DELTA) && active && p.bias) ? p.bias[n] : 0.f;
             scale8[hf][e] = (MODE == 0 && SCALE && active && p.colscale) ? p.colscale[n] : 1.f;
         }
     float csum[2][8];
@@ -367,6 +390,7 @@
     const unsigned ax_x = (unsigned)((fr & 12) * 16);
     const unsigned xq0 = (unsigned)(A_PLANE + fr * 512 + (((wave * 8 + fq) ^ fr) & 31) * 16);
     const unsigned xq1 = (unsigned)(A_PLANE + fr * 512 + (((wave * 8 + 4 + fq) ^ fr) & 31) * 16);
+    const unsigned xl = (unsigned)(2 * A_PLANE + wave * 256 + (lane & 31) * 4);
     const __amdgpu_buffer_rsrc_t rC = __builtin_amdgcn_make_buffer_rsrc(
         (void*)(reinterpret_cast<h16_t*>(p.C) + (int64_t)row_base * p.ldc), 0,
         active ? (int)((((int64_t)rows_here - 1) * p.ldc + p.N) * 2) : 0, 0x00020000);
@@ -377,6 +401,7 @@
     const int cstep = (int)(TR * p.ldc * 2), pstep = (int)(TR * p.ldp * 2);
 
     u32x4_t af[8], ax[2] = {u32x4_t{0, 0, 0, 0}, u32x4_t{0, 0, 0, 0}};
+    float lsev = 0.f;
     auto read_frags = [&](int slot) {
         const unsigned sl = lds0 + (unsigned)(slot * SLOT);
         const unsigned b = sl + aoff;
@@ -400,11 +425,12 @@
                 : "v"(sl + xq0), "v"(sl + xq1)
                 : "memory");
         }
+        if constexpr (DELTA) asm volatile("ds_read_b32 %0, %1" : "=&v"(lsev) : "v"(sl + xl) : "memory");
     };
     auto wait_frags = [&]() {
         asm volatile("s_waitcnt lgkmcnt(0)"
                      : "+v"(af[0]), "+v"(af[1]), "+v"(af[2]), "+v"(af[3]), "+v"(af[4]), "+v"(af[5]), "+v"(af[6]), "+v"(af[7]),
-                       "+v"(ax[0]), "+v"(ax[1]));
+                       "+v"(ax[0]), "+v"(ax[1]), "+v"(lsev));
     };
     auto mfma_slab = [&](f32x4 (&acc)[4]) {
 #pragma unroll
@@ -416,13 +442,40 @@
                 acc[t] = SVOL_MFMA_16x16x32_H16(__builtin_bit_cast(h16x8, wf[t][ks]),
                                                                  __builtin_bit_cast(h16x8, af[ks]), acc[t], 0, 0, 0);
     };
-    auto epilogue = [&](int j, const f32x4 (&acc)[4], const u32x4_t (&axj)[2]) {
+    auto epilogue = [&](int j, const f32x4 (&acc)[4], const u32x4_t (&axj)[2], float lsej) {
         float v[2][8];
 #pragma unroll
         for (int hf = 0; hf < 2; ++hf)
 #pragma unroll
             for (int e = 0; e < 8; ++e) v[hf][e] = acc[2 * hf + (e >> 2)][e & 3];
-        if constexpr (MODE == 0) {
+        if constexpr (DELTA) {
+            h16x8 o[2];
+            float dl[2];
+#pragma unroll
+            for (int hf = 0; hf < 2; ++hf) {
+                const h16x8 a8 = __builtin_bit_cast(h16x8, axj[hf]);
+                float sum = 0.f;
+#pragma unroll
+                for (int e = 0; e < 8; ++e) {
+                    o[hf][e] = (h16_t)(v[hf][e] + bias8[hf][e]);
+                    sum = fmaf((float)o[hf][e], (float)a8[e], sum);
+                }
+                const HalfPair r16 = swap_rows16(__builtin_bit_cast(unsigned, sum));
+                sum = __builtin_bit_cast(float, r16.lo) + __builtin_bit_cast(float, r16.hi);
+                const HalfPair r32 = swap_halves(__builtin_bit_cast(unsigned, sum));
+                dl[hf] = __builtin_bit_cast(float, r32.lo) + __builtin_bit_cast(float, r32.hi);
+            }
+            store_b128_guarded(__builtin_bit_cast(u32x4_t, o[0]), rC, voffC, j * cstep);
+            store_b128_guarded(__builtin_bit_cast(u32x4_t, o[1]), rC, voffC + 64, j * cstep);
+            const float d = fq == 1 ? dl[1] : dl[0];
+            const unsigned vo = (rows_lane && st_m < p.M) ? (unsigned)st_si * 4u : OOB;
+            const unsigned plane = (unsigned)p.rows_total * 4u;
+            __builtin_amdgcn_raw_buffer_store_b32(__builtin_bit_cast(unsigned, d), rR, (int)(vo + ATTN_ROWS_DELTA * plane), 0, 0);
+            __builtin_amdgcn_raw_buffer_store_b32(__builtin_bit_cast(unsigned, -lsej), rR, (int)(vo + ATTN_ROWS_NL * plane), 0, 0);
+            __builtin_amdgcn_raw_buffer_store_b32(__builtin_bit_cast(unsigned, -d), rR, (int)(vo + ATTN_ROWS_ND * plane), 0, 0);
+            st_m += TR; st_q += TR; st_si += TR;
+            if (st_q >= p.Lq) { st_q -= p.Lq; st_si += p.row_wrap; }
+        } else if constexpr (MODE == 0) {
 #pragma unroll
             for (int hf = 0; hf < 2; ++hf)
 #pragma unroll
@@ -489,10 +542,11 @@
         for (int t = 0; t < 4; ++t) accp[t] = acc[t];
         axp[0] = ax[0];
         axp[1] = ax[1];
+        const float lsep = lsev;
         read_frags((j + 1) % STG);
         wait_frags();
         mfma_slab(acc);
-        epilogue(j, accp, axp);
+        epilogue(j, accp, axp, lsep);
 #pragma unroll
         for (int i = 0; i < 32; ++i) {
             __builtin_amdgcn_sched_group_barrier(0x008, 1, 0);
@@ -501,7 +555,7 @@
     }
     {
         u32x4_t axp[2] = {ax[0], ax[1]};
-        epilogue(ntile - 1, acc, axp);
+        epilogue(ntile - 1, acc, axp, lsev);
     }
     if constexpr (MODE == 2) {
         if (p.colsum) {
@@ -532,7 +586,46 @@
 WSP_KERNEL(gemm_wsp_bf16_dmul, 2, SVOL_ACT_GELU_D, false, false, 3)
 WSP_KERNEL(gemm_wsp_bf16_drelu, 2, SVOL_ACT_RELU, false, false, 3)
 #undef WSP_KERNEL
-
+__global__ __launch_bounds__(256, 2) void gemm_wsp_bf16_delta(WsArgs p) { gemm_wsp_body<2, SVOL_ACT_NONE, false, false, 3, true>(p); }
+
+}
+
+static void ws_split(int64_t ntile, int64_t ncg, int64_t& tpw, int64_t& nchunk) {
+    tpw = (ntile * ncg + (ncg <= 2 ? 255 : 511)) / (ncg <= 2 ? 256 : 512);
+    if (tpw < 4) tpw = 4;
+    if (tpw > 64) tpw = 64;
+    nchunk = (ntile + tpw - 1) / tpw;
+    if (ncg > 1 && nchunk > 8 && nchunk % 8) {
+        const int64_t n8 = (nchunk + 7) / 8 * 8;
+        const int64_t t8 = (ntile + n8 - 1) / n8;
+        if (t8 >= 1 && (ntile + t8 - 1) / t8 == n8) { tpw = t8; nchunk = n8; }
+    }
+}
+
+int svol_gemm_ws_delta_bf16(const void* A, int64_t lda, const void* W, int64_t ldw, void* C, int64_t ldc, const float* bias,
+                            const void* O, int64_t ldo, const float* lse2, float* rows, int64_t B, int64_t H, int64_t Lq, int64_t N,
+                            int64_t K, hipStream_t s) {
+    const int64_t M = B * Lq, total = attn_rows_total(B, H, Lq);
+    static_assert(WS_K == 256 && TR == 16, "svol_gemm_nt_delta_shape_ok states these");
+    if (!svol_gemm_nt_delta_shape_ok(B, H, Lq, N, K)) return SVOL_E_UNSUPPORTED;
+    auto al16 = [](const void* p_) { return (reinterpret_cast<uintptr_t>(p_) & 15) == 0; };
+    if (lda % 8 || ldw % 8 || ldc % 8 || ldo % 8 || !al16(A) || !al16(W) || !al16(C) || !al16(O)) return SVOL_E_UNSUPPORTED;
+    if ((reinterpret_cast<uintptr_t>(lse2) | reinterpret_cast<uintptr_t>(rows)) & 3) return SVOL_E_UNSUPPORTED;
+    if (M >= (1ll << 30) || ATTN_ROWS_PLANES * total * 4 >= (1ll << 30)) return SVOL_E_UNSUPPORTED;
+    const int64_t ntile = (M + TR - 1) / TR;
+    int64_t tpw, nchunk;
+    ws_split(ntile, 1, tpw, nchunk);
+    int64_t ldbig = lda > ldo ? lda : ldo;
+    if (ldc > ldbig) ldbig = ldc;
+    if (tpw * TR * ldbig * 2 >= (1ll << 31)) return SVOL_E_UNSUPPORTED;
+    WsArgs p{(const h16_t*)A, (const h16_t*)W, C, bias, nullptr, nullptr, nullptr, (const h16_t*)O, nullptr,
+             lda, ldw, ldc, 0, 0, ldo, (int)M, (int)N, SVOL_ACT_NONE, (int)tpw, (int)nchunk};
+    p.lse = lse2; p.rows = rows; p.Lq = (int)Lq; p.rows_total = (int)total;
+    p.head_step = (int)attn_rows_index(0, 1, 0, H, Lq);
+    p.batch_step = (int)attn_rows_index(1, 0, 0, H, Lq);
+    p.row_wrap = (int)(attn_rows_index(1, 0, 0, H, Lq) - attn_rows_index(0, 0, Lq, H, Lq));
+    hipLaunchKernelGGL(gemm_wsp_bf16_delta, dim3((unsigned)nchunk), dim3(256), 0, s, p);
+    return hipGetLastError() == hipSuccess ? SVOL_OK : SVOL_E_LAUNCH;
 }
 
 int svol_gemm_ws_bf16(const void* A, int64_t lda, const void* W, int64_t ldw, void* C, int64_t ldc, const float* bias, int act,
@@ -558,20 +651,13 @@
     if (mode == 2 && (ldaux % 8 || !al16(aux))) return SVOL_E_UNSUPPORTED;
     const int64_t ntile = (M + TR - 1) / TR;
     const int64_t ncg = (N + 255) / 256;
-    int64_t tpw = (ntile * ncg + (ncg <= 2 ? 255 : 511)) / (ncg <= 2 ? 256 : 512);
-    if (tpw < 4) tpw = 4;
-    if (tpw > 64) tpw = 64;
+    int64_t tpw, nchunk;
+    ws_split(ntile, ncg, tpw, nchunk);
     const int64_t ldmax = lda > ldr * 2 ? lda : ldr * 2;
     int64_t ldbig = ldmax > ldaux ? ldmax : ldaux;
     if (ldc > ldbig) ldbig = ldc;
     if (pre && ldp > ldbig) ldbig = ldp;
     if (tpw * TR * ldbig * 2 >= (1ll << 31)) return SVOL_E_UNSUPPORTED;
-    int64_t nchunk = (ntile + tpw - 1) / tpw;
-    if (ncg > 1 && nchunk > 8 && nchunk % 8) {
-        const int64_t n8 = (nchunk + 7) / 8 * 8;
-        const int64_t t8 = (ntile + n8 - 1) / n8;
-        if (t8 >= 1 && (ntile + t8 - 1) / t8 == n8) { tpw = t8; nchunk = n8; }
-    }
     if (nchunk * ncg > (1ll << 30)) return SVOL_E_UNSUPPORTED;
     WsArgs p{(const h16_t*)A, (const h16_t*)W, C, bias, colscale, (h16_t*)pre, res, (const h16_t*)aux, colsum,
              lda, ldw, ldc, ldp, ldr, ldaux, (int)M, (int)N, act, (int)tpw, (int)nchunk};
diff --git a/svol_amd/csrc/norm.hip b/svol_amd/csrc/norm.hip
--- a/svol_amd/csrc/norm.hip
+++ b/svol_amd/csrc/norm.hip
@@ -311,7 +311,7 @@
                        const float* mean, const float* rstd, float* dx32, void* dx, float* dgamma, float* dbeta,
                        float* dx_colsum, int64_t M, int64_t D, float dropout_p, uint64_t seed, const int64_t* seed_offset_dev,
                        int dtype, void* stream) {
-    if ((!dy32 && !dy && !dy2) || !x || !gamma || !mean || !rstd || (!dx && !dx32) || !dgamma || !dbeta || M < 0 || D <= 0)
+    if ((!dy32 && !dy && !dy2) || !x || !gamma || !mean || !rstd || !dgamma || !dbeta || M < 0 || D <= 0)
         return SVOL_E_INVALID;
     if (D % 4 || D > LN_MAX_PASSES * 256) return SVOL_E_UNSUPPORTED;
     if (dropout_p < 0.f || dropout_p >= 1.f) return SVOL_E_INVALID;
diff --git a/svol_amd/ops.py b/svol_amd/ops.py
--- a/svol_amd/ops.py
+++ b/svol_amd/ops.py
@@ -799,8 +799,8 @@
         x2, gamma, mean, rstd, seed_dev = ctx.saved_tensors
         sg, sb = ctx.sinks
         _, dx, dg, db = layernorm_bwd(None, dy, None, x2, gamma, mean, rstd, x2.dtype, ctx.p, ctx.seed, seed_dev=seed_dev,
-                                      dg_out=sg.view if sg else None, db_out=sb.view if sb else None)
-        return dx.view(ctx.shp), None if sg else dg, None if sb else db, None, None, None
+                                      want_t=ctx.needs_input_grad[0], dg_out=sg.view if sg else None, db_out=sb.view if sb else None)
+        return None if dx is None else dx.view(ctx.shp), None if sg else dg, None if sb else db, None, None, None
 
 
 def layer_norm(x, gamma, beta, p=0.0, seed=0, seed_dev=None):
```

New measurement: 13630. -8.2%, worse.
